# scraed/LanPaint

Measured on AMD Instinct MI355X. Metric: langevin_think_iterations_per_sec, higher is better.
Workload: dtype f32; 1 GPU; c2_sdxl: latent 1x4x128x128 per GPU, 30 sigmas x 5 think iterations, 50% box mask, stub backbone x->(0.9x,0.8x), VE/Karras schedule; rng=torch, graph=auto, mask_format=f32, mask_seen_by_kernels=bits, captured_calls=1, backbone_io=f32, replicas=1, rows_per_gpu=1, global_rows=1, latent_elements_per_gpu=65536

## Files before the change

include/lanpaint_hip.h:

```cpp
#ifndef LANPAINT_HIP_H
#define LANPAINT_HIP_H

#include <stdint.h>

#ifdef __cplusplus
extern "C" {
#endif

#define LP_ABI_VERSION 25

#define LP_API __attribute__((visibility("default")))

#define LP_OK             0
#define LP_E_INVALID     -1
#define LP_E_UNSUPPORTED -2
#define LP_E_LAUNCH      -3
#define LP_E_ALIGN       -4

#define LP_COEF_STRIDE   36
#define LP_C_SCALE        0
#define LP_C_SQRT_ABT     1
#define LP_C_OMA          2
#define LP_C_ABT          3
#define LP_C_RSIGMA       4
#define LP_C_DTX          5
#define LP_C_DTY          6
#define LP_C_AX           7
#define LP_C_AY           8
#define LP_C_DX           9
#define LP_C_DY          10
#define LP_C_VALID       11
#define LP_C_REGION0     12
#define LP_C_REGION1     22
#define LP_R_E_FULL       0
#define LP_R_K_FULL       1
#define LP_R_STD_FULL     2
#define LP_R_E_HALF       3
#define LP_R_K_HALF       4
#define LP_R_STD_HALF     5
#define LP_R_DT           6
#define LP_R_A            7
#define LP_R_CX0          8
#define LP_R_CXT          9
#define LP_C_TMODEL      32
#define LP_C_RSCALE      33

typedef struct lp_hyper {
    float    lambda;
    float    beta;
    float    step_size;
    float    min_step_frac;
    int32_t  is_flow;
    float    one_plus_lambda;
} lp_hyper;

#define LP_PH_REPLACE      (1u << 0)
#define LP_PH_POST_FIRST   (1u << 1)
#define LP_PH_POST_STEADY  (1u << 2)
#define LP_PH_PRE_HALF     (1u << 3)
#define LP_PH_EMIT         (1u << 4)
#define LP_PH_COEFFS       (1u << 5)
#define LP_PH_SIGMA        (1u << 6)

#define LP_FL_FLOW          (1u << 0)
#define LP_FL_MASK_DENOISE  (1u << 1)
#define LP_FL_MASK_U8       (1u << 2)
#define LP_FL_WRITE_X0S     (1u << 3)
#define LP_FL_X0_BF16       (1u << 4)
#define LP_FL_X0_F16        (1u << 5)
#define LP_FL_XIN_BF16      (1u << 6)
#define LP_FL_XIN_F16       (1u << 7)
#define LP_FL_PER_ELEMENT   (1u << 8)
#define LP_FL_CFG_FUSED     (1u << 10)
#define LP_FL_MASK_BITS     (1u << 11)
#define LP_FL_NO_REGION_SKIP (1u << 12)
#define LP_FL_ES            (1u << 13)
#define LP_FL_ES_GATED      (1u << 14)
#define LP_FL_ES_CLOSE      (1u << 15)
#define LP_FL_ES_RING_BITS  (1u << 16)
#define LP_FL_AV            (1u << 17)
#define LP_FL_X0S_GIVEN     (1u << 9)

typedef struct lp_es_state {
    int32_t  stopped;
    int32_t  counter;
    int32_t  n_ran;
    int32_t  cur_slot;
    int32_t  anchor_slot;
    int32_t  write_slot;
    uint32_t reserved0;
    int32_t  enabled;
    int64_t  seq_base;
    int64_t  total_ran;
    double   threshold_eff;
    double   abt_val;
    float*   x0s_buf[3];
} lp_es_state;

#define LP_ES_ACC_SLOTS  64
#define LP_ES_ACC_SETS   3
#define LP_ES_ACC_DOUBLES (LP_ES_ACC_SETS * LP_ES_ACC_SLOTS * 8)
#define LP_ES_SEQ_DONE   0x10000
#define LP_ES_TRACE0     8
#define LP_ES_MAILBOX_DOUBLES(n_steps) (LP_ES_TRACE0 + 8 * (n_steps))

#define LP_RNG_PHILOX 0
#define LP_RNG_TORCH  1

#define LP_REPLACE_KNOWN    0
#define LP_REPLACE_VE       1
#define LP_REPLACE_FLOW     2

typedef struct lp_step_desc {
    int64_t   n_el;
    int64_t   el_per_row;
    int32_t   rows;
    uint32_t  phases;
    uint32_t  flags;
    int32_t   replace_kind;
    float     lambda;
    float     one_plus_lambda;
    float     beta;
    float     step_size;
    float     min_step_frac;
    float     noise_scale;
    float     cfg_scale;
    float     cfg_scale_big;
    const float* coef;
    const float* x;
    const float* known;
    const float* noise;
    const float* y;
    const void*  mask;
    float*       x_t;
    float*       C;
    float*       x0s;
    const void*  x0;
    const void*  x0_big;
    void*        x_in;
    const float* xi_post;
    const float* xi_pre;
    uint64_t     rng_seed;
    uint64_t     rng_offset;
    const uint64_t* rng_offset_ptr;
    const float* abt_el;
    const float* ve_el;
    const float* rsig_el;
    const float* corr_el;
    const float* t_ve;
    const float* t_abt;
    const float* t_rsig;
    const float* t_model;
    float*       coef_out;
    int32_t      t_ve_stride, t_abt_stride, t_rsig_stride, t_model_stride;
    int32_t      rng_kind;
    uint32_t     rng_bg;
    uint32_t     rng_inc;
    uint64_t*    rng_state_out;
    uint64_t     rng_state_val[2];
    uint64_t*    io_table_out;
    uint64_t     io_table_val[2];
    lp_es_state* es;
    float*       es_x0s[3];
    const float* es_ring;
    double*      es_partials;
    double*      es_host;
    double       es_threshold;
    int64_t      es_seq_base;
    int32_t      es_patience_eff;
    int32_t      es_index;
    int32_t      es_n_steps;
    int32_t      es_reset;
    const float* sg_sigma;
    const float* sg_schedule;
    float*       sg_times_out;
    float*       sg_scalars_out;
    int32_t*     sg_seq_out;
    uint64_t*    sg_valid_out;
    double       sg_min_step_frac;
    int32_t      sg_schedule_len, sg_seq, sg_n_steps, sg_early_stop, sg_total_steps, sg_guess;
    double*      clk_out;
    const void*  av_bits;
    float        av_frac;
    uint32_t     reserved2;
    float*       es_xte;
    uint32_t     tune;
    uint32_t     io_valid;
} lp_step_desc;
#define LP_TUNE_VEC1          (1u << 0)
#define LP_TUNE_VEC4          (1u << 1)
#define LP_TUNE_ES_NO_DECIDE  (1u << 2)
#define LP_TUNE_ES_NO_FOLD    (1u << 3)
#define LP_TUNE_ES_NO_ATOMICS (1u << 4)
#define LP_CLK_STAMPS 8

typedef struct lp_final_desc {
    int64_t   n_el;
    uint32_t  flags;
    float     cfg_scale;
    const void*  model_out;
    const void*  uncond;
    const float* y;
    const void*  mask;
    const float* x_src;
    float*       x_dst;
    float*       out;
    uint64_t*    rng_bump_ptr;
    uint64_t     rng_bump;
    const uint64_t* io_table;
} lp_final_desc;

LP_API int lp_abi_version(void);
LP_API const char* lp_strerror(int code);

LP_API int lp_coeffs(const lp_hyper* hyper, const float* ve_sigma, int ve_stride, const float* abt, int abt_stride,
              const float* replace_sigma, int rs_stride, const float* step_override, int step_stride,
              const float* t_model, int t_stride, int rows, float* coef_table, void* stream);

typedef struct lp_call_desc {
    const lp_hyper*      hyper;
    const float*         ve_sigma;      int32_t ve_stride;
    const float*         abt;           int32_t abt_stride;
    const float*         replace_sigma; int32_t rs_stride;
    const float*         t_model;       int32_t t_stride;
    int32_t              rows;
    float*               coef_table;
    const lp_step_desc*  replace;
    void*                graph_exec;
    const lp_final_desc* final;
    const struct lp_graph_binding* replace_binding;
} lp_call_desc;
LP_API int lp_replay_call(const lp_call_desc* call, void* stream);

typedef struct lp_graph_binding {
    void*    node;
    void*    func;
    uint32_t grid[3], block[3];
    uint32_t shared_bytes;
    uint32_t reserved0;
} lp_graph_binding;
LP_API int lp_graph_bind_replace(void* graph, const lp_step_desc* captured_replace, lp_graph_binding* out);
LP_API int lp_graph_clone_tail(void* graph, void** tail_graph_out, void** tail_exec_out);
LP_API int lp_graph_release(void* tail_graph, void* tail_exec);
LP_API int lp_graph_clone_sigma_root(void* graph, const lp_step_desc* with_sigma, void** graph_out, void** exec_out,
                                     lp_graph_binding* binding_out);

LP_API int lp_sigma_times(const float* sigma, int32_t rows, const float* schedule, int32_t schedule_len, int32_t is_flow,
                   float* times_out, float* scalars_out, void* stream);
LP_API int lp_sigma_times_mailbox(const float* sigma, int32_t rows, const float* schedule, int32_t schedule_len, int32_t is_flow,
                           float* times_out, float* scalars_out, int32_t* seq_out, int32_t seq, void* stream);

typedef struct lp_node_call_desc {
    const float*        sigma;
    int32_t             rows;
    int32_t             schedule_len;
    const float*        schedule;
    int32_t             is_flow;
    int32_t             seq;
    float*              times_out;
    float*              scalars_out;
    int32_t*            seq_out;
    const lp_step_desc* replace;
    int32_t             n_steps;
    int32_t             early_stop;
    int32_t             total_steps;
    int32_t             n_counts;
    double              min_step_frac;
    void* const*        exec_by_count;
    int32_t             spin_limit;
    int32_t             guess;
    uint64_t*           valid_word;
    int32_t             fold_sigma;
    int32_t             n_eff;
    int32_t             launched;
    int32_t             speculated;
    int32_t             hit;
    float               step_f, frac;
    void* const*        full_exec_by_count;
    const struct lp_graph_binding* const* full_binding_by_count;
    int32_t             one_launch;
    int32_t             reserved0;
} lp_node_call_desc;
LP_API int lp_node_call(lp_node_call_desc* call, void* stream);
LP_API int32_t lp_effective_inner_steps(int32_t n_steps, double step_f, double frac, int32_t total_steps, int32_t early_stop,
                                 double min_step_frac);

LP_API int lp_step(const lp_step_desc* desc, void* stream);

LP_API int lp_timer_create(void** timer);
LP_API int lp_timer_destroy(void* timer);
LP_API int lp_step_timed(const lp_step_desc* desc, void* stream, void* timer);
LP_API int lp_step_timed_burst(const lp_step_desc* desc, void* stream, void* const* timers, int32_t n);
LP_API int lp_timer_elapsed_ns(void* timer, double* ns);

LP_API int lp_replay_burst(void* const* graph_execs, int32_t n, const lp_step_desc* before, const lp_step_desc* after,
                           int32_t repeats, void* stream);

LP_API int lp_finalize(const lp_final_desc* desc, void* stream);

LP_API int lp_philox_normal(float* out, int64_t n_el, uint64_t seed, uint64_t offset, uint32_t slot, void* stream);
LP_API int lp_torch_normal(float* out, int64_t n_el, uint64_t seed, uint64_t offset, uint32_t bg, void* stream);

LP_API int lp_boundary_ring(const float* mask, float* ring, int64_t planes, int32_t height, int32_t width, void* stream);
LP_API int lp_wmse_pair(const float* a, const float* b, const float* mask, const float* ring, int64_t n_el,
                 double* acc, double* block_scratch, int32_t scratch_blocks, void* stream);

#define LP_MASK_BITS_BYTES(n_el) ((((n_el) + 63) / 64) * 8)

LP_API int lp_pack_mask(const float* mask, int64_t n_el, uint32_t flags, void* bits, int32_t* nonbinary, void* stream);
LP_API int lp_pack_mask_latent(const float* mask, int64_t n_el, uint32_t flags, void* bits, float* latent_out, void* stream);

#define LP_NN_ATEN_SCALAR          0
#define LP_NN_ATEN_CPU_GENERIC_FMA 1
#define LP_NN_ATEN_CPU_GENERIC     2
#define LP_RESHAPE_BINARIZE        1
#define LP_RESHAPE_RULE_SHIFT      8

LP_API int lp_reshape_mask(const float* src, int32_t src_b, int32_t src_c, int32_t src_f, int32_t src_h, int32_t src_w,
                    float* dst, int32_t batch, int32_t channels, int32_t dst_f, int32_t dst_h, int32_t dst_w,
                    int32_t temporal_taps, int32_t flags, void* stream);

typedef struct lp_blend_desc {
    int32_t batch, height, width, channels;
    int32_t k;
    int32_t mask_batch;
    int32_t mask_h, mask_w;
    const float* mask;
    const float* image1;
    const float* image2;
    float*       out;
    float*       smooth_out;
    int32_t nn_rule;
    int32_t reserved0;
} lp_blend_desc;
LP_API int lp_mask_blend(const lp_blend_desc* desc, void* stream);

#define LP_VMASK_MAX_SIDE 16384
#define LP_VMASK_D2_NONE  (-1)
#define LP_VMASK_ZERO     0
#define LP_VMASK_KEY      1
#define LP_VMASK_INNER    2
#define LP_VMASK_OUT_U8   1

typedef struct lp_vmask_edt_desc {
    int32_t n_keys, height, width, reserved0;
    const float* keys;
    int32_t*     d2;
    double*      sdf;
    uint64_t*    csum;
} lp_vmask_edt_desc;
LP_API int lp_vmask_edt(const lp_vmask_edt_desc* desc, void* stream);

typedef struct lp_vmask_frame {
    int32_t kind, key_lo, key_hi, sx1, sy1, sx2, sy2, reserved0;
    double  wf, omw;
} lp_vmask_frame;

typedef struct lp_vmask_morph_desc {
    int32_t n_frames, n_keys, height, width;
    uint32_t flags;
    int32_t  reserved0;
    const lp_vmask_frame* frames;
    const float*  keys;
    const double* sdf;
    void*         out;
} lp_vmask_morph_desc;
LP_API int lp_vmask_morph(const lp_vmask_morph_desc* desc, void* stream);

typedef struct lp_vmask_resize_desc {
    int32_t n_frames, in_h, in_w, out_h, out_w, ksize_x, ksize_y, reserved0;
    const uint8_t* src;
    const int32_t* bounds_x;
    const int32_t* weights_x;
    const int32_t* bounds_y;
    const int32_t* weights_y;
    float*         dst;
} lp_vmask_resize_desc;
LP_API int lp_vmask_resize(const lp_vmask_resize_desc* desc, void* stream);

#define LP_AUDIO_WS_BYTES(mask_len) (12 * ((int64_t)(mask_len) + 1))
typedef struct lp_audio_desc {
    int32_t n;
    int32_t mask_len;
    int32_t batch, channels;
    int32_t cf;
    int32_t nn_rule;
    int64_t orig_sb, orig_sc;
    int64_t inp_sb, inp_sc;
    const float* mask;
    const float* orig;
    const float* inpainted;
    float*       out;
    void*        workspace;
} lp_audio_desc;
// ... 209 lines not shown
```

lanpaint_amd/_cabi.py:

```python
from __future__ import annotations

import ctypes as C
import os

_HERE = os.path.dirname(os.path.abspath(__file__))
LIB_NAME = "liblanpaint_hip.so"
LIB_PATH = os.path.join(_HERE, LIB_NAME)
ABI_VERSION = 25

LP_OK, LP_E_INVALID, LP_E_UNSUPPORTED, LP_E_LAUNCH, LP_E_ALIGN = 0, -1, -2, -3, -4
LP_COEF_STRIDE = 36
(LP_C_SCALE, LP_C_SQRT_ABT, LP_C_OMA, LP_C_ABT, LP_C_RSIGMA, LP_C_DTX, LP_C_DTY, LP_C_AX, LP_C_AY, LP_C_DX, LP_C_DY,
 LP_C_VALID) = range(12)
LP_C_REGION0, LP_C_REGION1, LP_C_TMODEL, LP_C_RSCALE = 12, 22, 32, 33
(LP_R_E_FULL, LP_R_K_FULL, LP_R_STD_FULL, LP_R_E_HALF, LP_R_K_HALF, LP_R_STD_HALF, LP_R_DT, LP_R_A, LP_R_CX0,
 LP_R_CXT) = range(10)

LP_PH_REPLACE, LP_PH_POST_FIRST, LP_PH_POST_STEADY, LP_PH_PRE_HALF, LP_PH_EMIT, LP_PH_COEFFS, LP_PH_SIGMA = 1, 2, 4, 8, 16, 32, 64
LP_FL_FLOW, LP_FL_MASK_DENOISE, LP_FL_MASK_U8, LP_FL_WRITE_X0S = 1, 2, 4, 8
LP_FL_X0_BF16, LP_FL_X0_F16, LP_FL_XIN_BF16, LP_FL_XIN_F16 = 16, 32, 64, 128
LP_FL_PER_ELEMENT, LP_FL_X0S_GIVEN, LP_FL_CFG_FUSED, LP_FL_MASK_BITS, LP_FL_NO_REGION_SKIP = 256, 512, 1024, 2048, 4096
LP_FL_ES, LP_FL_ES_GATED, LP_FL_ES_CLOSE, LP_FL_ES_RING_BITS, LP_FL_AV = 1 << 13, 1 << 14, 1 << 15, 1 << 16, 1 << 17
LP_TUNE_VEC1, LP_TUNE_VEC4, LP_TUNE_ES_NO_DECIDE, LP_TUNE_ES_NO_FOLD, LP_TUNE_ES_NO_ATOMICS = 1, 2, 4, 8, 16


def mask_bits_bytes(n_el: int) -> int:
    return ((int(n_el) + 63) // 64) * 8
LP_REPLACE_KNOWN, LP_REPLACE_VE, LP_REPLACE_FLOW = 0, 1, 2
LP_RNG_PHILOX, LP_RNG_TORCH = 0, 1
LP_NN_ATEN_SCALAR, LP_NN_ATEN_CPU_GENERIC_FMA, LP_NN_ATEN_CPU_GENERIC = 0, 1, 2
LP_RESHAPE_BINARIZE, LP_RESHAPE_RULE_SHIFT = 1, 8


class LpHyper(C.Structure):
    _fields_ = [("lambda_", C.c_float), ("beta", C.c_float), ("step_size", C.c_float), ("min_step_frac", C.c_float),
                ("is_flow", C.c_int32), ("one_plus_lambda", C.c_float)]


class LpStepDesc(C.Structure):
    _fields_ = [
        ("n_el", C.c_int64), ("el_per_row", C.c_int64), ("rows", C.c_int32), ("phases", C.c_uint32),
        ("flags", C.c_uint32), ("replace_kind", C.c_int32),
        ("lambda_", C.c_float), ("one_plus_lambda", C.c_float), ("beta", C.c_float), ("step_size", C.c_float),
        ("min_step_frac", C.c_float), ("noise_scale", C.c_float), ("cfg_scale", C.c_float), ("cfg_scale_big", C.c_float),
        ("coef", C.c_void_p), ("x", C.c_void_p), ("known", C.c_void_p), ("noise", C.c_void_p), ("y", C.c_void_p),
        ("mask", C.c_void_p), ("x_t", C.c_void_p), ("C", C.c_void_p), ("x0s", C.c_void_p), ("x0", C.c_void_p),
        ("x0_big", C.c_void_p), ("x_in", C.c_void_p), ("xi_post", C.c_void_p), ("xi_pre", C.c_void_p),
        ("rng_seed", C.c_uint64), ("rng_offset", C.c_uint64), ("rng_offset_ptr", C.c_void_p),
        ("abt_el", C.c_void_p), ("ve_el", C.c_void_p), ("rsig_el", C.c_void_p), ("corr_el", C.c_void_p),
        ("t_ve", C.c_void_p), ("t_abt", C.c_void_p), ("t_rsig", C.c_void_p), ("t_model", C.c_void_p),
        ("coef_out", C.c_void_p), ("t_ve_stride", C.c_int32), ("t_abt_stride", C.c_int32),
        ("t_rsig_stride", C.c_int32), ("t_model_stride", C.c_int32),
        ("rng_kind", C.c_int32), ("rng_bg", C.c_uint32), ("rng_inc", C.c_uint32),
        ("rng_state_out", C.c_void_p), ("rng_state_val", C.c_uint64 * 2),
        ("io_table_out", C.c_void_p), ("io_table_val", C.c_uint64 * 2),
        ("es", C.c_void_p), ("es_x0s", C.c_void_p * 3), ("es_ring", C.c_void_p), ("es_partials", C.c_void_p), ("es_host", C.c_void_p),
        ("es_threshold", C.c_double), ("es_seq_base", C.c_int64), ("es_patience_eff", C.c_int32), ("es_index", C.c_int32),
        ("es_n_steps", C.c_int32), ("es_reset", C.c_int32),
        ("sg_sigma", C.c_void_p), ("sg_schedule", C.c_void_p), ("sg_times_out", C.c_void_p), ("sg_scalars_out", C.c_void_p),
        ("sg_seq_out", C.c_void_p), ("sg_valid_out", C.c_void_p), ("sg_min_step_frac", C.c_double),
        ("sg_schedule_len", C.c_int32), ("sg_seq", C.c_int32), ("sg_n_steps", C.c_int32), ("sg_early_stop", C.c_int32),
        ("sg_total_steps", C.c_int32), ("sg_guess", C.c_int32), ("clk_out", C.c_void_p), ("av_bits", C.c_void_p), ("av_frac", C.c_float), ("reserved2", C.c_uint32),
        ("es_xte", C.c_void_p),
        ("tune", C.c_uint32), ("io_valid", C.c_uint32),
    ]


class LpEsState(C.Structure):
    _fields_ = [("stopped", C.c_int32), ("counter", C.c_int32), ("n_ran", C.c_int32), ("cur_slot", C.c_int32),
                ("anchor_slot", C.c_int32), ("write_slot", C.c_int32), ("reserved0", C.c_uint32), ("enabled", C.c_int32),
                ("seq_base", C.c_int64), ("total_ran", C.c_int64), ("threshold_eff", C.c_double), ("abt_val", C.c_double), ("x0s_buf", C.c_void_p * 3)]


LP_ES_SEQ_DONE, LP_ES_TRACE0 = 0x10000, 8
LP_ES_ACC_SLOTS, LP_ES_ACC_SETS = 64, 3
LP_ES_ACC_DOUBLES = LP_ES_ACC_SETS * LP_ES_ACC_SLOTS * 8


class LpFinalDesc(C.Structure):
    _fields_ = [
        ("n_el", C.c_int64), ("flags", C.c_uint32), ("cfg_scale", C.c_float),
        ("model_out", C.c_void_p), ("uncond", C.c_void_p), ("y", C.c_void_p), ("mask", C.c_void_p), ("x_src", C.c_void_p),
        ("x_dst", C.c_void_p), ("out", C.c_void_p), ("rng_bump_ptr", C.c_void_p), ("rng_bump", C.c_uint64),
        ("io_table", C.c_void_p),
    ]


class LpGraphBinding(C.Structure):
    _fields_ = [("node", C.c_void_p), ("func", C.c_void_p), ("grid", C.c_uint32 * 3), ("block", C.c_uint32 * 3),
                ("shared_bytes", C.c_uint32), ("reserved0", C.c_uint32)]


class LpCallDesc(C.Structure):
    _fields_ = [
        ("hyper", C.POINTER(LpHyper)),
        ("ve_sigma", C.c_void_p), ("ve_stride", C.c_int32),
        ("abt", C.c_void_p), ("abt_stride", C.c_int32),
        ("replace_sigma", C.c_void_p), ("rs_stride", C.c_int32),
        ("t_model", C.c_void_p), ("t_stride", C.c_int32),
        ("rows", C.c_int32),
        ("coef_table", C.c_void_p),
        ("replace", C.POINTER(LpStepDesc)),
        ("graph_exec", C.c_void_p),
        ("final", C.POINTER(LpFinalDesc)),
        ("replace_binding", C.POINTER(LpGraphBinding)),
    ]


class LpNodeCallDesc(C.Structure):
    _fields_ = [("sigma", C.c_void_p), ("rows", C.c_int32), ("schedule_len", C.c_int32), ("schedule", C.c_void_p),
                ("is_flow", C.c_int32), ("seq", C.c_int32), ("times_out", C.c_void_p), ("scalars_out", C.c_void_p),
                ("seq_out", C.c_void_p), ("replace", C.POINTER(LpStepDesc)), ("n_steps", C.c_int32),
                ("early_stop", C.c_int32), ("total_steps", C.c_int32), ("n_counts", C.c_int32),
                ("min_step_frac", C.c_double), ("exec_by_count", C.POINTER(C.c_void_p)), ("spin_limit", C.c_int32),
                ("guess", C.c_int32), ("valid_word", C.c_void_p), ("fold_sigma", C.c_int32), ("n_eff", C.c_int32), ("launched", C.c_int32),
                ("speculated", C.c_int32), ("hit", C.c_int32), ("step_f", C.c_float), ("frac", C.c_float),
                ("full_exec_by_count", C.POINTER(C.c_void_p)), ("full_binding_by_count", C.POINTER(C.POINTER(LpGraphBinding))),
                ("one_launch", C.c_int32), ("reserved0", C.c_int32)]


class LpBlendDesc(C.Structure):
    _fields_ = [("batch", C.c_int32), ("height", C.c_int32), ("width", C.c_int32), ("channels", C.c_int32),
                ("k", C.c_int32), ("mask_batch", C.c_int32), ("mask_h", C.c_int32), ("mask_w", C.c_int32),
                ("mask", C.c_void_p), ("image1", C.c_void_p), ("image2", C.c_void_p), ("out", C.c_void_p),
                ("smooth_out", C.c_void_p), ("nn_rule", C.c_int32), ("reserved0", C.c_int32)]


LP_VMASK_MAX_SIDE, LP_VMASK_D2_NONE = 16384, -1
LP_VMASK_ZERO, LP_VMASK_KEY, LP_VMASK_INNER, LP_VMASK_OUT_U8 = 0, 1, 2, 1


class LpVmaskEdtDesc(C.Structure):
    _fields_ = [("n_keys", C.c_int32), ("height", C.c_int32), ("width", C.c_int32), ("reserved0", C.c_int32),
                ("keys", C.c_void_p), ("d2", C.c_void_p), ("sdf", C.c_void_p), ("csum", C.c_void_p)]


class LpVmaskFrame(C.Structure):
    _fields_ = [("kind", C.c_int32), ("key_lo", C.c_int32), ("key_hi", C.c_int32), ("sx1", C.c_int32), ("sy1", C.c_int32),
                ("sx2", C.c_int32), ("sy2", C.c_int32), ("reserved0", C.c_int32), ("wf", C.c_double), ("omw", C.c_double)]


class LpVmaskMorphDesc(C.Structure):
    _fields_ = [("n_frames", C.c_int32), ("n_keys", C.c_int32), ("height", C.c_int32), ("width", C.c_int32),
                ("flags", C.c_uint32), ("reserved0", C.c_int32), ("frames", C.c_void_p), ("keys", C.c_void_p),
                ("sdf", C.c_void_p), ("out", C.c_void_p)]


class LpVmaskResizeDesc(C.Structure):
    _fields_ = [("n_frames", C.c_int32), ("in_h", C.c_int32), ("in_w", C.c_int32), ("out_h", C.c_int32),
                ("out_w", C.c_int32), ("ksize_x", C.c_int32), ("ksize_y", C.c_int32), ("reserved0", C.c_int32),
                ("src", C.c_void_p), ("bounds_x", C.c_void_p), ("weights_x", C.c_void_p), ("bounds_y", C.c_void_p),
                ("weights_y", C.c_void_p), ("dst", C.c_void_p)]


class LpAudioDesc(C.Structure):
    _fields_ = [("n", C.c_int32), ("mask_len", C.c_int32), ("batch", C.c_int32), ("channels", C.c_int32), ("cf", C.c_int32),
                ("nn_rule", C.c_int32), ("orig_sb", C.c_int64), ("orig_sc", C.c_int64), ("inp_sb", C.c_int64),
                ("inp_sc", C.c_int64), ("mask", C.c_void_p), ("orig", C.c_void_p), ("inpainted", C.c_void_p),
                ("out", C.c_void_p), ("workspace", C.c_void_p)]


LP_DETAIL_MAX_SIDE, LP_DETAIL_MAX_CHANNELS = 32768, 64


class LpDetailResampleDesc(C.Structure):
    _fields_ = [("batch", C.c_int32), ("src_h", C.c_int32), ("src_w", C.c_int32), ("channels", C.c_int32),
                ("y0", C.c_int32), ("x0", C.c_int32), ("win_h", C.c_int32), ("win_w", C.c_int32),
                ("out_h", C.c_int32), ("out_w", C.c_int32), ("ksize_x", C.c_int32), ("ksize_y", C.c_int32),
                ("src", C.c_void_p), ("bounds_x", C.c_void_p), ("weights_x", C.c_void_p), ("bounds_y", C.c_void_p),
                ("weights_y", C.c_void_p), ("dst", C.c_void_p)]


class LpDetailStitchDesc(C.Structure):
    _fields_ = [("batch", C.c_int32), ("height", C.c_int32), ("width", C.c_int32), ("channels", C.c_int32),
                ("y0", C.c_int32), ("x0", C.c_int32), ("win_h", C.c_int32), ("win_w", C.c_int32),
                ("k", C.c_int32), ("mask_batch", C.c_int32),
                ("mask", C.c_void_p), ("original", C.c_void_p), ("detail", C.c_void_p), ("out", C.c_void_p)]


LP_DETAIL_MAX_COMPONENTS, LP_DETAIL_MAX_REGIONS = 4096, 64


class LpDetailResampleRegionsDesc(C.Structure):
    _fields_ = [("batch", C.c_int32), ("src_h", C.c_int32), ("src_w", C.c_int32), ("channels", C.c_int32),
                ("regions", C.c_int32), ("win_h", C.c_int32), ("win_w", C.c_int32), ("owner_len", C.c_int32),
                ("out_h", C.c_int32), ("out_w", C.c_int32), ("ksize_x", C.c_int32), ("ksize_y", C.c_int32),
                ("origins", C.c_void_p), ("src", C.c_void_p), ("bounds_x", C.c_void_p), ("weights_x", C.c_void_p),
                ("bounds_y", C.c_void_p), ("weights_y", C.c_void_p), ("dst", C.c_void_p), ("labels", C.c_void_p),
                ("owner", C.c_void_p), ("scratch", C.c_void_p)]


class LpDetailStitchRegionsDesc(C.Structure):
    _fields_ = [("batch", C.c_int32), ("height", C.c_int32), ("width", C.c_int32), ("channels", C.c_int32),
                ("regions", C.c_int32), ("win_h", C.c_int32), ("win_w", C.c_int32), ("k", C.c_int32),
                ("mask_batch", C.c_int32), ("owner_len", C.c_int32),
                ("origins", C.c_void_p), ("mask", C.c_void_p), ("original", C.c_void_p), ("detail", C.c_void_p),
                ("out", C.c_void_p), ("labels", C.c_void_p), ("owner", C.c_void_p)]


class LpDetailResampleTrackDesc(C.Structure):
    _fields_ = [("batch", C.c_int32), ("src_h", C.c_int32), ("src_w", C.c_int32), ("channels", C.c_int32),
                ("win_h", C.c_int32), ("win_w", C.c_int32), ("out_h", C.c_int32), ("out_w", C.c_int32),
                ("ksize_x", C.c_int32), ("ksize_y", C.c_int32),
                ("origins", C.c_void_p), ("src", C.c_void_p), ("bounds_x", C.c_void_p), ("weights_x", C.c_void_p),
                ("bounds_y", C.c_void_p), ("weights_y", C.c_void_p), ("dst", C.c_void_p)]


class LpDetailStitchTrackDesc(C.Structure):
    _fields_ = [("batch", C.c_int32), ("height", C.c_int32), ("width", C.c_int32), ("channels", C.c_int32),
                ("win_h", C.c_int32), ("win_w", C.c_int32), ("k", C.c_int32), ("mask_batch", C.c_int32),
                ("origins", C.c_void_p), ("mask", C.c_void_p), ("original", C.c_void_p), ("detail", C.c_void_p),
                ("out", C.c_void_p)]


class LpDetailResampleSubjectsDesc(C.Structure):
    _fields_ = [("batch", C.c_int32), ("src_h", C.c_int32), ("src_w", C.c_int32), ("channels", C.c_int32),
                ("subjects", C.c_int32), ("win_h", C.c_int32), ("win_w", C.c_int32), ("owner_len", C.c_int32),
                ("out_h", C.c_int32), ("out_w", C.c_int32), ("ksize_x", C.c_int32), ("ksize_y", C.c_int32),
                ("origins", C.c_void_p), ("src", C.c_void_p), ("bounds_x", C.c_void_p), ("weights_x", C.c_void_p),
                ("bounds_y", C.c_void_p), ("weights_y", C.c_void_p), ("dst", C.c_void_p), ("labels", C.c_void_p),
                ("owner", C.c_void_p), ("scratch", C.c_void_p)]


class LpDetailStitchSubjectsDesc(C.Structure):
    _fields_ = [("batch", C.c_int32), ("height", C.c_int32), ("width", C.c_int32), ("channels", C.c_int32),
                ("subjects", C.c_int32), ("win_h", C.c_int32), ("win_w", C.c_int32), ("k", C.c_int32),
                ("owner_len", C.c_int32), ("reserved0", C.c_int32),
                ("origins", C.c_void_p), ("mask", C.c_void_p), ("original", C.c_void_p), ("detail", C.c_void_p),
                ("out", C.c_void_p), ("labels", C.c_void_p), ("owner", C.c_void_p)]


LP_COLOR_MIN_COUNT, LP_COLOR_MAX_MARGIN, LP_COLOR_TILE_H, LP_COLOR_TILE_W = 64, 25, 32, 128
LP_COLOR_METHOD_MEAN, LP_COLOR_METHOD_MEAN_STD = 0, 1


class LpColorStatsDesc(C.Structure):
    _fields_ = [("batch", C.c_int32), ("height", C.c_int32), ("width", C.c_int32), ("channels", C.c_int32),
                ("mask_batch", C.c_int32), ("margin", C.c_int32),
                ("detail", C.c_void_p), ("reference", C.c_void_p), ("mask", C.c_void_p), ("stats", C.c_void_p),
                ("workspace", C.c_void_p), ("workspace_bytes", C.c_int64)]


class LpColorFitDesc(C.Structure):
    _fields_ = [("batch", C.c_int32), ("channels", C.c_int32), ("clip_frames", C.c_int32), ("smooth", C.c_int32),
                ("method", C.c_int32), ("reserved0", C.c_int32), ("strength", C.c_double),
                ("stats", C.c_void_p), ("coef", C.c_void_p)]


class LpColorApplyDesc(C.Structure):
    _fields_ = [("batch", C.c_int32), ("height", C.c_int32), ("width", C.c_int32), ("channels", C.c_int32),
                ("detail", C.c_void_p), ("coef", C.c_void_p), ("out", C.c_void_p)]


def lp_color_ws_bytes(batch, height, width, channels):
    tiles = ((int(height) + LP_COLOR_TILE_H - 1) // LP_COLOR_TILE_H) * ((int(width) + LP_COLOR_TILE_W - 1) // LP_COLOR_TILE_W)
    return int(batch) * tiles * (1 + 4 * int(channels)) * 8


LP_FILL_TILE, LP_FILL_SPAN = 32, 5


class LpFillDesc(C.Structure):
    _fields_ = [("batch", C.c_int32), ("height", C.c_int32), ("width", C.c_int32), ("channels", C.c_int32),
                ("mask_batch", C.c_int32), ("reserved0", C.c_int32),
                ("image", C.c_void_p), ("mask", C.c_void_p), ("out", C.c_void_p), ("ws", C.c_void_p), ("ws_bytes", C.c_int64)]


class LpOutpaintDesc(C.Structure):
    _fields_ = [("batch", C.c_int32), ("height", C.c_int32), ("width", C.c_int32), ("channels", C.c_int32),
                ("mask_batch", C.c_int32), ("left", C.c_int32), ("top", C.c_int32), ("right", C.c_int32),
                ("bottom", C.c_int32), ("overlap", C.c_int32), ("reserved0", C.c_int32),
                ("image", C.c_void_p), ("mask", C.c_void_p), ("image_out", C.c_void_p), ("mask_out", C.c_void_p)]


def fill_levels(height, width):
    levels = [(int(height), int(width))]
    while levels[-1] != (1, 1):
        h, w = levels[-1]
        levels.append(((h + 1) // 2, (w + 1) // 2))
    return levels


def fill_ws_bytes(batch, height, width, channels):
    pix = sum(h * w for h, w in fill_levels(height, width)[1:])
    return max(16, (int(batch) * pix * (4 * int(channels) + 1) + 15) // 16 * 16)


def lp_components_ws_bytes(height, width):
    return ((int(height) * int(width) + 1023) // 1024) * 4100


def lp_components_frames_ws_bytes(frames, height, width):
    return ((int(frames) * int(height) * int(width) + 1023) // 1024) * 4100


def lp_audio_ws_bytes(mask_len):
    return 12 * (int(mask_len) + 1)


EXPORTS = {
    "lp_abi_version": (C.c_int, []),
    "lp_strerror": (C.c_char_p, [C.c_int]),
    "lp_coeffs": (C.c_int, [C.POINTER(LpHyper), C.c_void_p, C.c_int, C.c_void_p, C.c_int, C.c_void_p, C.c_int,
                            C.c_void_p, C.c_int, C.c_void_p, C.c_int, C.c_int, C.c_void_p, C.c_void_p]),
    "lp_sigma_times": (C.c_int, [C.c_void_p, C.c_int32, C.c_void_p, C.c_int32, C.c_int32, C.c_void_p, C.c_void_p, C.c_void_p]),
    "lp_sigma_times_mailbox": (C.c_int, [C.c_void_p, C.c_int32, C.c_void_p, C.c_int32, C.c_int32, C.c_void_p, C.c_void_p,
                                         C.c_void_p, C.c_int32, C.c_void_p]),
    "lp_step": (C.c_int, [C.POINTER(LpStepDesc), C.c_void_p]),
    "lp_finalize": (C.c_int, [C.POINTER(LpFinalDesc), C.c_void_p]),
    "lp_mask_blend": (C.c_int, [C.POINTER(LpBlendDesc), C.c_void_p]),
    "lp_timer_create": (C.c_int, [C.POINTER(C.c_void_p)]),
    "lp_timer_destroy": (C.c_int, [C.c_void_p]),
    "lp_step_timed": (C.c_int, [C.POINTER(LpStepDesc), C.c_void_p, C.c_void_p]),
    "lp_step_timed_burst": (C.c_int, [C.POINTER(LpStepDesc), C.c_void_p, C.POINTER(C.c_void_p), C.c_int32]),
    "lp_timer_elapsed_ns": (C.c_int, [C.c_void_p, C.POINTER(C.c_double)]),
    "lp_replay_burst": (C.c_int, [C.POINTER(C.c_void_p), C.c_int32, C.POINTER(LpStepDesc), C.POINTER(LpStepDesc), C.c_int32, C.c_void_p]),
    "lp_torch_normal": (C.c_int, [C.c_void_p, C.c_int64, C.c_uint64, C.c_uint64, C.c_uint32, C.c_void_p]),
    "lp_philox_normal": (C.c_int, [C.c_void_p, C.c_int64, C.c_uint64, C.c_uint64, C.c_uint32, C.c_void_p]),
    "lp_boundary_ring": (C.c_int, [C.c_void_p, C.c_void_p, C.c_int64, C.c_int32, C.c_int32, C.c_void_p]),
    "lp_wmse_pair": (C.c_int, [C.c_void_p, C.c_void_p, C.c_void_p, C.c_void_p, C.c_int64, C.c_void_p, C.c_void_p,
                               C.c_int32, C.c_void_p]),
    "lp_replay_call": (C.c_int, [C.POINTER(LpCallDesc), C.c_void_p]),
    "lp_graph_bind_replace": (C.c_int, [C.c_void_p, C.POINTER(LpStepDesc), C.POINTER(LpGraphBinding)]),
    "lp_graph_clone_tail": (C.c_int, [C.c_void_p, C.POINTER(C.c_void_p), C.POINTER(C.c_void_p)]),
    "lp_graph_release": (C.c_int, [C.c_void_p, C.c_void_p]),
    "lp_graph_clone_sigma_root": (C.c_int, [C.c_void_p, C.POINTER(LpStepDesc), C.POINTER(C.c_void_p), C.POINTER(C.c_void_p),
                                            C.POINTER(LpGraphBinding)]),
    "lp_node_call": (C.c_int, [C.POINTER(LpNodeCallDesc), C.c_void_p]),
    "lp_effective_inner_steps": (C.c_int32, [C.c_int32, C.c_double, C.c_double, C.c_int32, C.c_int32, C.c_double]),
    "lp_pack_mask": (C.c_int, [C.c_void_p, C.c_int64, C.c_uint32, C.c_void_p, C.c_void_p, C.c_void_p]),
    "lp_pack_mask_latent": (C.c_int, [C.c_void_p, C.c_int64, C.c_uint32, C.c_void_p, C.c_void_p, C.c_void_p]),
    "lp_reshape_mask": (C.c_int, [C.c_void_p] + [C.c_int32] * 5 + [C.c_void_p] + [C.c_int32] * 7 + [C.c_void_p]),
    "lp_vmask_edt": (C.c_int, [C.POINTER(LpVmaskEdtDesc), C.c_void_p]),
    "lp_vmask_morph": (C.c_int, [C.POINTER(LpVmaskMorphDesc), C.c_void_p]),
    "lp_vmask_resize": (C.c_int, [C.POINTER(LpVmaskResizeDesc), C.c_void_p]),
    "lp_audio_merge": (C.c_int, [C.POINTER(LpAudioDesc), C.c_void_p]),
    "lp_mask_bbox": (C.c_int, [C.c_void_p, C.c_int32, C.c_int32, C.c_int32, C.c_void_p, C.c_void_p]),
    "lp_detail_resample": (C.c_int, [C.POINTER(LpDetailResampleDesc), C.c_void_p]),
    "lp_detail_stitch": (C.c_int, [C.POINTER(LpDetailStitchDesc), C.c_void_p]),
    "lp_mask_components": (C.c_int, [C.c_void_p, C.c_int32, C.c_int32, C.c_int32, C.c_void_p, C.c_void_p, C.c_void_p, C.c_int64,
                                     C.c_void_p]),
    "lp_detail_resample_regions": (C.c_int, [C.POINTER(LpDetailResampleRegionsDesc), C.c_void_p]),
    "lp_detail_stitch_regions": (C.c_int, [C.POINTER(LpDetailStitchRegionsDesc), C.c_void_p]),
    "lp_mask_bbox_frames": (C.c_int, [C.c_void_p, C.c_int32, C.c_int32, C.c_int32, C.c_void_p, C.c_void_p]),
    "lp_detail_resample_track": (C.c_int, [C.POINTER(LpDetailResampleTrackDesc), C.c_void_p]),
    "lp_detail_stitch_track": (C.c_int, [C.POINTER(LpDetailStitchTrackDesc), C.c_void_p]),
    "lp_mask_components_frames": (C.c_int, [C.c_void_p, C.c_int32, C.c_int32, C.c_int32, C.c_void_p, C.c_void_p, C.c_void_p,
                                            C.c_int64, C.c_void_p]),
    "lp_subject_boxes": (C.c_int, [C.c_void_p, C.c_int32, C.c_int32, C.c_int32, C.c_void_p, C.c_int32, C.c_int32, C.c_void_p,
                                   C.c_void_p]),
    "lp_detail_resample_subjects": (C.c_int, [C.POINTER(LpDetailResampleSubjectsDesc), C.c_void_p]),
    "lp_detail_stitch_subjects": (C.c_int, [C.POINTER(LpDetailStitchSubjectsDesc), C.c_void_p]),
    "lp_color_stats": (C.c_int, [C.POINTER(LpColorStatsDesc), C.c_void_p]),
    "lp_color_fit": (C.c_int, [C.POINTER(LpColorFitDesc), C.c_void_p]),
    "lp_color_apply": (C.c_int, [C.POINTER(LpColorApplyDesc), C.c_void_p]),
    "lp_mask_fill": (C.c_int, [C.POINTER(LpFillDesc), C.c_void_p]),
    "lp_fill_ws_bytes": (C.c_int64, [C.c_int32, C.c_int32, C.c_int32, C.c_int32]),
    "lp_outpaint_pad": (C.c_int, [C.POINTER(LpOutpaintDesc), C.c_void_p]),
}


class LanPaintHipError(RuntimeError):
    """A C-ABI call returned a negative status (the reference raises Python
    exceptions only; C codes are mapped to RuntimeError here)."""


_lib = None


def load(path: str | None = None):
    global _lib
    if _lib is not None and path is None:
        return _lib
    p = path or os.environ.get("LANPAINT_AMD_LIB", LIB_PATH)
    if not os.path.exists(p):
        raise ImportError(
            f"{p} not found: the HIP extension is not built. Run `python -c 'import __graft_entry__ as g; g.build()'` "
            "(or `python -m lanpaint_amd.build`). lanpaint_amd has no CPU / PyTorch fallback for the Langevin path.")
    lib = C.CDLL(p)
    for name, (res, args) in EXPORTS.items():
        fn = getattr(lib, name)
        fn.restype, fn.argtypes = res, args
    v = lib.lp_abi_version()
    if v != ABI_VERSION:
        raise ImportError(f"{p}: ABI version {v}, expected {ABI_VERSION}; rebuild the extension")
    if path is None:
        _lib = lib
    return lib


def check(code: int, what: str = "lanpaint_hip"):
    if code != LP_OK:
        msg = load().lp_strerror(code)
        raise LanPaintHipError(f"{what}: {msg.decode() if msg else code} (code {code})")
```

lanpaint_amd/buffers.py:

```python
from __future__ import annotations

import weakref

import torch

from . import _cabi
from ._util import tensor_version

class _Workspace:

    def __init__(self, like: torch.Tensor, static_io: bool = False, model_dtype=None):
        self.shape, self.device = tuple(like.shape), like.device
        self.x_t = torch.empty_like(like)
        self.C = torch.empty_like(like)
        self.coef = torch.empty((like.shape[0], _cabi.LP_COEF_STRIDE), dtype=torch.float32, device=like.device)
        self.coef_av = None
        self.av_times = None
        self.x0s = []
        self.static_io = static_io
        if static_io:
            self.x_final = torch.empty_like(like)
            self.x_in = self.x_final if model_dtype is None else torch.empty_like(like, dtype=model_dtype)

    def matches(self, like):
        return self.shape == tuple(like.shape) and self.device == like.device


class _DeviceStop:

    def __init__(self, like: torch.Tensor, n_steps: int):
        dev = like.device
        self.shape, self.device, self.n_cap = tuple(like.shape), dev, max(8, int(n_steps))
        self.x0s = [torch.empty_like(like) for _ in range(3)]
        self.x_te = torch.empty_like(like)
        init = _cabi.LpEsState()
        init.cur_slot = init.anchor_slot = -1
        for k in range(3):
            init.x0s_buf[k] = self.x0s[k].data_ptr()
        raw = torch.frombuffer(bytearray(bytes(init) * 2), dtype=torch.uint8)
        self.state = torch.empty(raw.numel(), dtype=torch.uint8, device=dev)
        self.state.copy_(raw)
        self.partials = torch.zeros(_cabi.LP_ES_ACC_DOUBLES, dtype=torch.float64, device=dev)
        self.mailbox = torch.zeros(_cabi.LP_ES_TRACE0 + 8 * self.n_cap, dtype=torch.float64).pin_memory()
        self.f64 = self.mailbox.numpy()
        self.i64 = self.mailbox.view(torch.int64).numpy()
        self.seq_base = 0
        self.seen_total = 0
        self.ring = None

    def matches(self, like, n_steps):
        return self.shape == tuple(like.shape) and self.device == like.device and n_steps <= self.n_cap

    def next_seq(self):
        self.seq_base += 2 * _cabi.LP_ES_SEQ_DONE
        return self.seq_base

    def ring_for(self, key, mask):
        c = self.ring
        ver = (tensor_version(key), key.data_ptr())
        if c is None or c[0]() is not key or c[1] != ver or ver[0] == -1:
            ring = None
            if mask.dim() == 4:
                old = c[2] if c is not None else None
                ring = old if (old is not None and old.shape == mask.shape and old.device == mask.device) else torch.empty_like(mask)
                b, ch, h, w = mask.shape
                with torch.cuda.device(mask.device):
                    _cabi.check(_cabi.load().lp_boundary_ring(mask.data_ptr(), ring.data_ptr(), b * ch, h, w,
                                                              torch.cuda.current_stream(mask.device).cuda_stream),
                                "lp_boundary_ring")
            bits = None
            if ring is not None:
                old_bits = c[3] if c is not None else None
                n_bytes = _cabi.mask_bits_bytes(ring.numel())
                bits = old_bits if (old_bits is not None and old_bits.numel() == n_bytes and old_bits.device == ring.device) \
                    else torch.empty(n_bytes, dtype=torch.uint8, device=ring.device)
                with torch.cuda.device(mask.device):
                    _cabi.check(_cabi.load().lp_pack_mask(ring.data_ptr(), ring.numel(), 0, bits.data_ptr(), None,
                                                          torch.cuda.current_stream(mask.device).cuda_stream), "lp_pack_mask")
            self.ring = c = (weakref.ref(key), ver, ring, bits)
        return c[2]

    def ring_bits(self):
        return self.ring[3] if self.ring is not None else None

    def wait(self, seq, device):
        i64 = self.i64
        for _ in range(20000):
            if i64[0] >= seq:
                return
        torch.cuda.current_stream(device).synchronize()
        if i64[0] < seq:
            raise RuntimeError("early-stop mailbox was not written (expected sequence %d, found %d)" % (seq, int(i64[0])))


class _CallState:
    __slots__ = ("input_x", "xc", "shape", "n_el", "rows", "flow", "ws", "stream", "sigma", "y", "m", "m_c", "m_flag", "abt",
                 "current_times", "base_flags", "keep", "t_model", "sigma_model", "compat", "n_steps", "x_final", "x_in",
                 "xin_flag", "k0_desc", "replace_kind_static", "out", "es")


class _CapturedCall:

    def __init__(self, counter):
        self.graph = torch.cuda.CUDAGraph()
        self.counter = counter
        self.ws = None
        self.final = None
        self.ran = 0
        self.launches = 0
        self.keep = None
        self.fast = False
        self.rows, self.flow, self.hyper, self.k0_desc, self.f_desc = 0, False, None, None, None
        self.call = None
        self.raw_exec = None
        self.ident = None
        self.final_in_graph = False
        self.es = None
        self.n_steps = 0
        self.key = None
        self.tail = None
        self.model_options = None
        self.alive = True
        self.siblings = {}
        self.times_seen = ()
        self.node_table = None
        self.binding = None
        self.tail_handles = None
        self.sigma_root = None

    def __del__(self):
        sr, self.sigma_root = self.sigma_root, None
        if sr:
            try:
                _cabi.load().lp_graph_release(sr[0], sr[1])
            except Exception:
                pass
        h, self.tail_handles = self.tail_handles, None
        if h is not None:
            try:
                _cabi.load().lp_graph_release(h[0], h[1])
            except Exception:
                pass
```

lanpaint_amd/capture.py:

```python
from __future__ import annotations

import ctypes
import os
import weakref

import torch

from . import _cabi
from ._util import _gc_hold, _gc_release
from .buffers import _CapturedCall, _Workspace
from .masks import _compact_mask


class GraphReplay:

    MAX_GRAPHS = 16
    AUTO_MAX_BACKBONE_HOST_US = 100.0

    def begin_call(self, x, latent_image, noise, sigma, latent_mask, current_times, model_options, seed):
        cap = self._last_cap
        if cap is None or cap.tail is None or self.model_dtype is not None or not x.is_cuda:
            return None
        self.img_dim_size = len(x.shape)
        self.latent_image, self.noise = latent_image, noise
# ... 167 lines not shown
                and i[17] == self._hyper_key() and (x.data_ptr() & 15) == 0 and (nz.data_ptr() & 15) == 0
                and not (isinstance(model_options, dict) and "lanpaint_semantic_stop" in model_options))

    @staticmethod
    def _times_ok(cap, current_times):
        i, f32 = cap.ident, torch.float32
        ve, abt, ft = current_times
        for seen in cap.times_seen:
            if seen[0] is ve and seen[1] is abt and seen[2] is ft:
                return True
        ok = (i[13] == ve.numel() and i[14] == abt.numel() and i[15] == ft.numel() and ve.dtype == f32 and abt.dtype == f32
              and ft.dtype == f32 and ve.is_contiguous() and abt.is_contiguous() and ft.is_contiguous())
        if ok:
            cap.times_seen = (cap.times_seen + ((ve, abt, ft),))[-2:]
        return ok

    def _hyper_key(self):
        return (self.chara_lamb, self.chara_beta, self.step_size, self.min_step_frac)

    def _override_state(self):
        d, t, o = self.__dict__, type(self), self._OWN_METHODS
        return ("langevin_dynamics" in d or t.langevin_dynamics is not o[0], "score_model" in d or t.score_model is not o[1],
                "prepare_step_size" in d or t.prepare_step_size is not o[2], self.IS_FLUX, self.IS_FLOW, self.model_dtype)

    def _graph_eligible(self, x, model_options, sigma, current_times):
        if not self.graph or self._graph_blocked or callable(self.rng) or self._noise_regenerated:
            return False
        rows = x.shape[0] if x.ndim else 1
        if any(t.numel() not in (1, rows) for t in (sigma, *current_times)):
            return False
        if self.audio_indicator is not None or self.audio_correction is not None:
            if (self.audio_indicator is None or self.current_times_audio is None
                    or any(t.numel() not in (1, rows) for t in self.current_times_audio)
                    or os.environ.get("LANPAINT_AMD_AV_TABLE", "1") == "0"):
                return False
            packed = self._indicator_pack(self.audio_indicator, x.shape)
            if packed is None or (self._es_opts is not None and not packed[2]):
                return False
        if self._es_opts is not None and (not self._es_opts["device"] or self.rng not in ("torch", "philox")):
            return False
        if self._overridden("langevin_dynamics") or self._overridden("score_model") or \
                self._overridden("prepare_step_size"):
            return False
        return x.dtype == torch.float32 and x.numel() > 0

    def _auto_ready(self, x, latent_mask, model_options):
        a = self._auto
        if a is not None and a[0][0]() is self.latent_image and a[0][1]() is latent_mask and a[0][2] == id(model_options) \
                and a[0][3] == x.shape and a[0][4] == x.device:
            if self._es_opts is not None:
                return False
            return a[1] >= 1 and 1e6 * a[2] < self.AUTO_MAX_BACKBONE_HOST_US
        self._auto = [(weakref.ref(self.latent_image), weakref.ref(latent_mask), id(model_options), x.shape, x.device), 0,
                      float("inf")]
        return False

    def _auto_capture(self, key, x, sigma, latent_mask, current_times, n_steps, model_options, seed, IS_FLUX, IS_FLOW):
        import warnings
        dev = x.device
        saved = (self._iterations_run, torch.cuda.get_rng_state(dev), self._es_opts, self._torch_consumed, self._philox_offset)

        def give_up(why):
            self._capturing = None
            try:
                torch.cuda.synchronize(dev)
            except Exception:
                pass
            self._iterations_run, _, self._es_opts, self._torch_consumed, self._philox_offset = saved
            torch.cuda.set_rng_state(saved[1], dev)
            self._graph_blocked = True
            cap = self._graphs.pop(key, None)
            if cap is not None:
                cap.alive = False
            self._last_cap = None
            warnings.warn("lanpaint_amd: graph='auto' stays with eager launches for this engine: " + why)
            return None

        try:
            cap = self._capture(key, x, sigma, latent_mask, current_times, n_steps, model_options, seed, IS_FLUX, IS_FLOW)
        except Exception as e:
            return give_up("the backbone could not be captured (%s: %s)" % (type(e).__name__, str(e).splitlines()[0] if str(e) else ""))
        if cap is None or self.rng != "torch":
            return cap
        try:
            xa, xb = x.clone(), x.clone()
            out_a = self._run_capture(cap, xa, sigma, latent_mask, current_times, n_steps, model_options, seed, IS_FLUX, IS_FLOW)
            torch.cuda.set_rng_state(saved[1], dev)
            self._last_cap = None
            out_b = self.LanPaint(xb, sigma, latent_mask, current_times, n_steps, model_options, seed, IS_FLUX, IS_FLOW)
            same = bool(torch.equal(out_a, out_b)) and bool(torch.equal(xa, xb))
        except Exception as e:
            return give_up("checking the capture against eager launches failed (%s)" % type(e).__name__)
        if not same:
            return give_up("a replayed sigma call does not reproduce the eager one (the backbone keeps state the graph does not see)")
        self._iterations_run, _, _, self._torch_consumed, self._philox_offset = saved
        torch.cuda.set_rng_state(saved[1], dev)
        return cap

    def _call_graphed(self, x, sigma, latent_mask, current_times, n_steps, model_options, seed, IS_FLUX, IS_FLOW):
        m_c, _ = _compact_mask(latent_mask, x.shape, x.device)
        key = (tuple(x.shape), x.device.index, int(n_steps), bool(IS_FLUX), bool(IS_FLOW), self.latent_image.data_ptr(),
               latent_mask.data_ptr(), m_c.data_ptr() if m_c is not None else 0, int(sigma.numel()),
               tuple(int(t.numel()) for t in current_times), id(model_options), seed, self.rng, self._hyper_key(),
               self.model_dtype, None if self._es_opts is None else (self._es_opts["threshold"], self._es_opts["patience_eff"],
                                                                      self._es_opts["trace"] is not None),
               None if self.audio_indicator is None else (self._indicator_pack(self.audio_indicator, x.shape)[0].data_ptr(),
                                                          self.audio_correction is not None))
        cap = self._graphs.get(key)
        if cap is not None and cap.model_options is not model_options:
            del self._graphs[key]
            cap.alive = False
            cap = None
        if cap is None:
            capture = self._auto_capture if self.graph == "auto" else self._capture
            cap = capture(key, x, sigma, latent_mask, current_times, n_steps, model_options, seed, IS_FLUX, IS_FLOW)
            if cap is None:
                return self.LanPaint(x, sigma, latent_mask, current_times, n_steps, model_options, seed, IS_FLUX, IS_FLOW)
            while len(self._graphs) > self.MAX_GRAPHS:
                self._graphs.popitem(last=False)[1].alive = False
        else:
            self._graphs.move_to_end(key)
        return self._run_capture(cap, x, sigma, latent_mask, current_times, n_steps, model_options, seed, IS_FLUX, IS_FLOW)

    def _run_capture(self, cap, x, sigma, latent_mask, current_times, n_steps, model_options, seed, IS_FLUX, IS_FLOW):
        srcs = (x, sigma, current_times[0], current_times[1], current_times[2], self.noise)
        fast = cap.fast and all(t.dtype == torch.float32 and t.is_contiguous() for t in srcs) and self.noise.shape == x.shape \
            and (x.data_ptr() & 15) == 0 and (self.noise.data_ptr() & 15) == 0
        if not fast and cap.binding is not None:
            self._last_cap = None
            return self.LanPaint(x, sigma, latent_mask, current_times, n_steps, model_options, seed, IS_FLUX, IS_FLOW)
        self._iterations_run += cap.ran
        self.last_inner_steps = cap.ran
        if fast:
            if not isinstance(model_options, dict) or "lanpaint_semantic_stop" not in model_options:
                cap.ident = (self.latent_image, latent_mask, model_options, x.shape, n_steps, seed, self.rng,
                             self.latent_image.data_ptr(), latent_mask.data_ptr(), getattr(latent_mask, "_lp_bits", None),
                             getattr(latent_mask, "_lp_u8", None), x.device, sigma.numel(), current_times[0].numel(),
                             current_times[1].numel(), current_times[2].numel(), self._override_state(), self._hyper_key())
                self._last_cap = cap
            return self._replay_fast(cap, x, sigma, current_times)
        self._last_cap = None
        st = self._prologue(x, sigma, latent_mask, current_times, n_steps, model_options, seed, IS_FLUX, IS_FLOW, ws=cap.ws,
                            ds=cap.es["ds"] if cap.es is not None else None)
        cap.graph.replay()
        if self.rng == "torch":
            gen = self._generator(x.device)
            gen.set_offset(gen.get_offset() + cap.launches)
            self._torch_consumed += cap.launches
        out = self._epilogue(st, cap.final, rng_bump=(cap.counter, cap.launches) if self.rng == "philox" else None,
                             in_graph=cap.final_in_graph)
        if cap.es is not None and st.es is not None:
            self._es_after_replay(cap, st.es["seq"], x.device)
        return out

    def _replay_fast(self, cap, x, sigma, current_times):
        lib, stream = self._lib, self._stream(x.device)
        ve, abt = current_times[0], current_times[1]
        t_src = current_times[2] if cap.flow else ve
        out = torch.empty_like(x)
        k0, f = cap.k0_desc, cap.f_desc
        k0.x, k0.noise = x.data_ptr(), self.noise.data_ptr()
        k0.t_ve, k0.t_abt, k0.t_rsig, k0.t_model = ve.data_ptr(), abt.data_ptr(), sigma.data_ptr(), t_src.data_ptr()
        if cap.final_in_graph:
            k0.io_table_val[0], k0.io_table_val[1] = k0.x, out.data_ptr()
        else:
            f.x_dst, f.out = k0.x, out.data_ptr()
        if self.rng == "torch":
            gen = self._generator(x.device)
            off = gen.get_offset()
            k0.rng_state_val[0], k0.rng_state_val[1] = off, gen.initial_seed()
            gen.set_offset(off + cap.launches)
            self._torch_consumed += cap.launches
        seq = 0
        if cap.es is not None:
            seq = k0.es_seq_base = cap.es["ds"].next_seq()
        if cap.raw_exec is not None:
            _cabi.check(lib.lp_replay_call(ctypes.byref(cap.call), stream), "lp_replay_call")
        else:
            _cabi.check(lib.lp_step(ctypes.byref(k0), stream), "lp_step")
            cap.graph.replay()
            if not cap.final_in_graph:
                _cabi.check(lib.lp_finalize(ctypes.byref(f), stream), "lp_finalize")
        if cap.es is not None:
            self._es_after_replay(cap, seq, x.device)
        return out

    def _es_after_replay(self, cap, seq, dev):
        es = dict(cap.es, trace=self._es_opts["trace"] if self._es_opts is not None else None,
                  tags=self._es_opts["tags"] if self._es_opts is not None else (None, None, None))
        inc = self._randn_policy(dev, cap.ws.x_t.numel())[1] if self.rng == "torch" else 0
        self._es_pending = (cap.es["ds"], seq, cap.n_steps, es, dev, inc)
        if inc or es["trace"] is not None:
            self._es_resolve()

    def _rng_state(self, dev):
        state = self._rng_counters.get(dev)
        if state is None:
            state = self._rng_counters[dev] = torch.zeros(8, dtype=torch.int64, device=dev)
            state[4] = 1
        return state

    _capture_sentinels = {}
    _capture_warned = set()

    @classmethod
    def _warm_capture_state(cls, dev):
        if cls._capture_sentinels.get(dev.index) is not None:
            return
        try:
            with torch.inference_mode(False), torch.no_grad():
                g = torch.cuda.CUDAGraph()
                s = torch.cuda.Stream(device=dev)
                s.wait_stream(torch.cuda.current_stream(dev))
                with torch.cuda.graph(g, stream=s, capture_error_mode="thread_local"):
                    torch.zeros(1, device=dev)
                torch.cuda.current_stream(dev).wait_stream(s)
                cls._capture_sentinels[dev.index] = g
        except Exception as e:
            if dev.index not in cls._capture_warned:
                cls._capture_warned.add(dev.index)
                import warnings
                warnings.warn("lanpaint_amd: the capture warm-up on %s failed (%s: %s); it is retried before the next capture"
                              % (dev, type(e).__name__, str(e).splitlines()[0] if str(e) else ""))

    def _capture(self, key, x, sigma, latent_mask, current_times, n_steps, model_options, seed, IS_FLUX, IS_FLOW,
                 replace_in_graph=None):
        dev = x.device
        self._warm_capture_state(dev)
        if replace_in_graph is None:
            replace_in_graph = os.environ.get("LANPAINT_AMD_REPLACE_IN_GRAPH", "1") != "0"
        raw_ok = self.rng in ("philox", "torch") and os.environ.get("LANPAINT_AMD_RAW_GRAPH", "1") != "0"
        replace_in_graph = bool(replace_in_graph and raw_ok)
        counter = self._rng_state(dev)
        cap = _CapturedCall(counter)
        if replace_in_graph:
            try:
                cap.graph = torch.cuda.CUDAGraph(keep_graph=True)
            except (TypeError, RuntimeError):
                replace_in_graph = False
        ws_key = (tuple(x.shape), dev.index, self.model_dtype)
        cap.ws = self._static_ws.get(ws_key)
        if cap.ws is None:
            if len(self._static_ws) >= self.MAX_GRAPHS:
                self._static_ws.pop(next(iter(self._static_ws)))
            cap.ws = self._static_ws[ws_key] = _Workspace(x.detach().to(torch.float32).contiguous(), static_io=True,
                                                          model_dtype=self.model_dtype)
        side = torch.cuda.Stream(device=dev)
        side.wait_stream(torch.cuda.current_stream(dev))
        it0 = self._iterations_run
        rng_state = torch.cuda.get_rng_state(dev)
        gen = self._generator(dev)
        off0, own0 = gen.get_offset(), self._torch_consumed
        es_user = self._es_opts
        if es_user is not None:
            self._es_opts = dict(es_user, trace=None)
            self._es_close = es_user["trace"] is None
        with torch.cuda.stream(side):
            xw = x.detach().clone()
            st = self._prologue(xw, sigma, latent_mask, current_times, n_steps, model_options, seed, IS_FLUX, IS_FLOW,
                                ws=cap.ws)
            self._epilogue(st, self._think_and_final_model(st, model_options, seed))
            st = self._prologue(xw, sigma, latent_mask, current_times, n_steps, model_options, seed, IS_FLUX, IS_FLOW,
                                ws=cap.ws, defer_launch=replace_in_graph)
            if replace_in_graph and not (st.k0_desc is not None and st.replace_kind_static and st.xc is st.input_x
                                         and (st.xc.data_ptr() & 15) == 0 and (self.noise.data_ptr() & 15) == 0):
                replace_in_graph = False
                self._launch_step_desc(st.k0_desc, st.stream)
        torch.cuda.current_stream(dev).wait_stream(side)
        torch.cuda.synchronize(dev)
        torch_rng_used = (gen.get_offset() - off0) != (self._torch_consumed - own0)
        if torch_rng_used and self.rng == "torch":
            torch.cuda.set_rng_state(rng_state, dev)
            self._iterations_run = it0
            self._graph_blocked = True
            self._es_opts = es_user
            return None
        if torch_rng_used and replace_in_graph:
            torch.cuda.set_rng_state(rng_state, dev)
            self._iterations_run = it0
            self._es_opts = es_user
            return self._capture(key, x, sigma, latent_mask, current_times, n_steps, model_options, seed, IS_FLUX, IS_FLOW,
                                 replace_in_graph=False)
        self._iterations_run = it0
        self._capturing, self._cap_offset = counter, 0
        _gc_hold()
        try:
            f = _cabi.LpFinalDesc()
            with torch.cuda.graph(cap.graph, stream=side, capture_error_mode="thread_local"):
                if replace_in_graph:
                    self._launch_step_desc(st.k0_desc, self._stream(dev))
                cap.final = self._think_and_final_model(st, model_options, seed)
                dense_ok = self._fill_final_desc(f, st, cap.final, st.out)
                if self.rng == "philox":
                    f.rng_bump_ptr, f.rng_bump = counter.data_ptr(), self._cap_offset
                if dense_ok and st.out is not None:
                    f.io_table = counter.data_ptr() + 16
                    _cabi.check(self._lib.lp_finalize(ctypes.byref(f), self._stream(dev)), "lp_finalize")
                    cap.final_in_graph = True
        finally:
            self._capturing = None
            _gc_release()
        cap.launches = self._cap_offset
        self._es_opts = es_user
        torch.cuda.set_rng_state(rng_state, dev)
        cap.ran = self._iterations_run - it0
        self._iterations_run = it0
        cap.keep = st
        cap.rows, cap.flow = st.rows, st.flow
        cap.hyper = _cabi.LpHyper.from_buffer_copy(self._hyper)
        cap.k0_desc = st.k0_desc
        cap.f_desc = f
        cap.model_options = model_options
        cap.es, cap.n_steps = st.es, st.n_steps
        cap.fast = bool(dense_ok and st.k0_desc is not None and st.replace_kind_static and st.xc is st.input_x)
        if replace_in_graph:
            ok = cap.fast and cap.final_in_graph
            if ok:
                try:
                    cap.graph.instantiate()
                    raw_graph = int(cap.graph.raw_cuda_graph())
                    cap.raw_exec = int(cap.graph.raw_cuda_graph_exec()) or None
                    b = _cabi.LpGraphBinding()
                    ok = cap.raw_exec is not None and self._lib.lp_graph_bind_replace(
                        raw_graph, ctypes.byref(cap.k0_desc), ctypes.byref(b)) == _cabi.LP_OK
                    if ok:
                        cap.binding = b
                        tg, te = ctypes.c_void_p(), ctypes.c_void_p()
                        if self._lib.lp_graph_clone_tail(raw_graph, ctypes.byref(tg), ctypes.byref(te)) == _cabi.LP_OK:
                            cap.tail_handles = (tg.value, te.value)
                except Exception:
                    ok = False
            if not ok:
                return self._capture(key, x, sigma, latent_mask, current_times, n_steps, model_options, seed, IS_FLUX,
                                     IS_FLOW, replace_in_graph=False)
        if cap.fast:
            if cap.binding is None and raw_ok and not torch_rng_used:
                try:
                    cap.raw_exec = int(cap.graph.raw_cuda_graph_exec()) or None
                except Exception:
                    cap.raw_exec = None
            c = cap.call = _cabi.LpCallDesc()
            c.replace = ctypes.pointer(cap.k0_desc)
            c.final = None if cap.final_in_graph else ctypes.pointer(f)
            c.rows, c.coef_table, c.graph_exec = st.rows, cap.ws.coef.data_ptr(), cap.raw_exec
            if cap.binding is not None:
                c.replace_binding = ctypes.pointer(cap.binding)
                if cap.tail_handles is not None:
                    t = cap.tail = _cabi.LpCallDesc()
                    t.rows, t.coef_table, t.graph_exec = st.rows, cap.ws.coef.data_ptr(), cap.tail_handles[1]
            elif cap.raw_exec is not None and cap.final_in_graph:
                t = cap.tail = _cabi.LpCallDesc()
                t.rows, t.coef_table, t.graph_exec = st.rows, cap.ws.coef.data_ptr(), cap.raw_exec
        cap.key = key
        self._graphs[key] = cap
        return cap
```

lanpaint_amd/csrc/cabi.hip:

```cpp
#include <cmath>

#include "lp_common.h"

namespace lp {
int step_dispatch(const lp_step_desc* d, hipStream_t stream, void* timer);
int replace_node_update(const lp_step_desc* d, hipGraphExec_t exec, const lp_graph_binding* b);
int timer_create(void** out);
int timer_destroy(void* h);
int timer_elapsed_ns(void* h, double* ns);
int coeffs_dispatch(const lp_hyper* h, const float* ve, int ve_stride, const float* abt, int abt_stride,
                    const float* rs, int rs_stride, const float* step_ov, int step_stride, const float* t_model,
                    int t_stride, int rows, float* table, hipStream_t stream);
int finalize_dispatch(const lp_final_desc* d, hipStream_t stream);
int sigma_times_dispatch(const float* sigma, int rows, const float* schedule, int schedule_len, int is_flow, float* times,
                         float* scalars, int32_t* seq_out, int32_t seq, hipStream_t stream);
int sigma_times_rule_dispatch(const float* sigma, int rows, const float* schedule, int schedule_len, int is_flow,
                              float* times, float* scalars, int32_t* seq_out, int32_t seq, int32_t n_steps, int32_t early_stop,
                              int32_t total_steps, double min_step_frac, int32_t guess, uint64_t* valid_out, hipStream_t stream);
int blend_dispatch(const lp_blend_desc* d, hipStream_t stream);
int philox_dispatch(float* out, int64_t n_el, uint64_t seed, uint64_t offset, uint32_t slot, hipStream_t stream);
int ring_dispatch(const float* mask, float* ring, int64_t planes, int height, int width, hipStream_t stream);
int wmse_dispatch(const float* a, const float* b, const float* mask, const float* ring, int64_t n_el, double* acc,
                  double* scratch, int scratch_blocks, hipStream_t stream);
int torch_normal_dispatch(float* out, int64_t n, uint64_t seed, uint64_t offset, uint32_t bg, hipStream_t stream);
int pack_mask_dispatch(const float* mask, int64_t n_el, uint32_t flags, void* bits, int32_t* nonbinary, float* latent_out,
                       hipStream_t stream);
int vmask_edt_dispatch(const lp_vmask_edt_desc* d, hipStream_t stream);
int vmask_morph_dispatch(const lp_vmask_morph_desc* d, hipStream_t stream);
int vmask_resize_dispatch(const lp_vmask_resize_desc* d, hipStream_t stream);
int audio_merge_dispatch(const lp_audio_desc* d, hipStream_t stream);
int mask_bbox_dispatch(const float* mask, int planes, int H, int W, int32_t* boxes, bool per_plane, hipStream_t stream);
int detail_resample_dispatch(const lp_detail_resample_desc* d, hipStream_t stream);
int detail_stitch_dispatch(const lp_detail_stitch_desc* d, hipStream_t stream);
int mask_components_dispatch(const float* mask, int planes, int H, int W, int32_t* labels, int32_t* table, void* workspace,
                             int64_t workspace_bytes, hipStream_t stream);
int detail_resample_regions_dispatch(const lp_detail_resample_regions_desc* d, hipStream_t stream);
int detail_stitch_regions_dispatch(const lp_detail_stitch_regions_desc* d, hipStream_t stream);
int detail_resample_track_dispatch(const lp_detail_resample_track_desc* d, hipStream_t stream);
int detail_stitch_track_dispatch(const lp_detail_stitch_track_desc* d, hipStream_t stream);
int mask_components_frames_dispatch(const float* mask, int F, int H, int W, int32_t* labels, int32_t* table, void* workspace,
                                    int64_t workspace_bytes, hipStream_t stream);
int subject_boxes_dispatch(const int32_t* labels, int frames, int H, int W, const int32_t* owner, int owner_len, int subjects,
                           int32_t* boxes, hipStream_t stream);
int detail_resample_subjects_dispatch(const lp_detail_resample_subjects_desc* d, hipStream_t stream);
int detail_stitch_subjects_dispatch(const lp_detail_stitch_subjects_desc* d, hipStream_t stream);
int color_stats_dispatch(const lp_color_stats_desc* d, hipStream_t stream);
int color_fit_dispatch(const lp_color_fit_desc* d, hipStream_t stream);
int color_apply_dispatch(const lp_color_apply_desc* d, hipStream_t stream);
int mask_fill_dispatch(const lp_fill_desc* d, hipStream_t stream);
int64_t fill_ws_bytes(int batch, int height, int width, int channels);
int outpaint_pad_dispatch(const lp_outpaint_desc* d, hipStream_t stream);
int reshape_mask_dispatch(const float* src, int sb, int sc, int sf, int sh, int sw, float* dst, int db, int dc, int df,
                          int dh, int dw, int taps, int flags, hipStream_t stream);
}

static inline hipStream_t as_stream(void* s) { return static_cast<hipStream_t>(s); }

extern "C" {

int lp_abi_version(void) { return LP_ABI_VERSION; }

const char* lp_strerror(int code) {
    switch (code) {
        case LP_OK: return "ok";
        case LP_E_INVALID: return "invalid argument (null pointer or inconsistent sizes/phases)";
        case LP_E_UNSUPPORTED: return "unsupported layout or flag combination";
        case LP_E_LAUNCH: return "HIP kernel launch failed";
        case LP_E_ALIGN: return "pointer not aligned for the requested layout";
        default: return "unknown lanpaint_hip error code";
    }
}

int lp_coeffs(const lp_hyper* hyper, const float* ve_sigma, int ve_stride, const float* abt, int abt_stride,
              const float* replace_sigma, int rs_stride, const float* step_override, int step_stride,
              const float* t_model, int t_stride, int rows, float* coef_table, void* stream) {
    return lp::coeffs_dispatch(hyper, ve_sigma, ve_stride, abt, abt_stride, replace_sigma, rs_stride, step_override,
                               step_stride, t_model, t_stride, rows, coef_table, as_stream(stream));
}

int lp_sigma_times(const float* sigma, int32_t rows, const float* schedule, int32_t schedule_len, int32_t is_flow,
                   float* times_out, float* scalars_out, void* stream) {
    return lp::sigma_times_dispatch(sigma, rows, schedule, schedule_len, is_flow, times_out, scalars_out, nullptr, 0,
                                    as_stream(stream));
}

int lp_sigma_times_mailbox(const float* sigma, int32_t rows, const float* schedule, int32_t schedule_len, int32_t is_flow,
                           float* times_out, float* scalars_out, int32_t* seq_out, int32_t seq, void* stream) {
    if (!seq_out) return LP_E_INVALID;
    return lp::sigma_times_dispatch(sigma, rows, schedule, schedule_len, is_flow, times_out, scalars_out, seq_out, seq,
                                    as_stream(stream));
}

int lp_step(const lp_step_desc* desc, void* stream) { return lp::step_dispatch(desc, as_stream(stream), nullptr); }

int lp_timer_create(void** timer) { return lp::timer_create(timer); }
int lp_timer_destroy(void* timer) { return lp::timer_destroy(timer); }
int lp_step_timed(const lp_step_desc* desc, void* stream, void* timer) {
    if (!timer) return LP_E_INVALID;
    return lp::step_dispatch(desc, as_stream(stream), timer);
}
int lp_timer_elapsed_ns(void* timer, double* ns) { return lp::timer_elapsed_ns(timer, ns); }

int lp_mask_blend(const lp_blend_desc* desc, void* stream) { return lp::blend_dispatch(desc, as_stream(stream)); }

int lp_vmask_edt(const lp_vmask_edt_desc* desc, void* stream) { return lp::vmask_edt_dispatch(desc, as_stream(stream)); }

int lp_vmask_morph(const lp_vmask_morph_desc* desc, void* stream) { return lp::vmask_morph_dispatch(desc, as_stream(stream)); }

int lp_vmask_resize(const lp_vmask_resize_desc* desc, void* stream) { return lp::vmask_resize_dispatch(desc, as_stream(stream)); }

int lp_audio_merge(const lp_audio_desc* desc, void* stream) { return lp::audio_merge_dispatch(desc, as_stream(stream)); }

int lp_mask_bbox(const float* mask, int32_t planes, int32_t height, int32_t width, int32_t* bbox, void* stream) {
    return lp::mask_bbox_dispatch(mask, planes, height, width, bbox, false, as_stream(stream));
}

int lp_detail_resample(const lp_detail_resample_desc* desc, void* stream) { return lp::detail_resample_dispatch(desc, as_stream(stream)); }

int lp_detail_stitch(const lp_detail_stitch_desc* desc, void* stream) { return lp::detail_stitch_dispatch(desc, as_stream(stream)); }

int lp_mask_components(const float* mask, int32_t planes, int32_t height, int32_t width, int32_t* labels, int32_t* table,
                       void* workspace, int64_t workspace_bytes, void* stream) {
    return lp::mask_components_dispatch(mask, planes, height, width, labels, table, workspace, workspace_bytes, as_stream(stream));
}

int lp_detail_resample_regions(const lp_detail_resample_regions_desc* desc, void* stream) {
    return lp::detail_resample_regions_dispatch(desc, as_stream(stream));
}

int lp_detail_stitch_regions(const lp_detail_stitch_regions_desc* desc, void* stream) {
    return lp::detail_stitch_regions_dispatch(desc, as_stream(stream));
}

int lp_mask_bbox_frames(const float* mask, int32_t planes, int32_t height, int32_t width, int32_t* boxes, void* stream) {
    return lp::mask_bbox_dispatch(mask, planes, height, width, boxes, true, as_stream(stream));
}

int lp_detail_resample_track(const lp_detail_resample_track_desc* desc, void* stream) {
    return lp::detail_resample_track_dispatch(desc, as_stream(stream));
}

int lp_detail_stitch_track(const lp_detail_stitch_track_desc* desc, void* stream) {
    return lp::detail_stitch_track_dispatch(desc, as_stream(stream));
}

int lp_mask_components_frames(const float* mask, int32_t frames, int32_t height, int32_t width, int32_t* labels, int32_t* table,
                              void* workspace, int64_t workspace_bytes, void* stream) {
    return lp::mask_components_frames_dispatch(mask, frames, height, width, labels, table, workspace, workspace_bytes,
                                               as_stream(stream));
}

int lp_subject_boxes(const int32_t* labels, int32_t frames, int32_t height, int32_t width, const int32_t* owner, int32_t owner_len,
                     int32_t subjects, int32_t* boxes, void* stream) {
    return lp::subject_boxes_dispatch(labels, frames, height, width, owner, owner_len, subjects, boxes, as_stream(stream));
}

int lp_detail_resample_subjects(const lp_detail_resample_subjects_desc* desc, void* stream) {
    return lp::detail_resample_subjects_dispatch(desc, as_stream(stream));
}

int lp_detail_stitch_subjects(const lp_detail_stitch_subjects_desc* desc, void* stream) {
    return lp::detail_stitch_subjects_dispatch(desc, as_stream(stream));
}

int lp_color_stats(const lp_color_stats_desc* desc, void* stream) { return lp::color_stats_dispatch(desc, as_stream(stream)); }

int lp_color_fit(const lp_color_fit_desc* desc, void* stream) { return lp::color_fit_dispatch(desc, as_stream(stream)); }

int lp_color_apply(const lp_color_apply_desc* desc, void* stream) { return lp::color_apply_dispatch(desc, as_stream(stream)); }

int lp_mask_fill(const lp_fill_desc* desc, void* stream) { return lp::mask_fill_dispatch(desc, as_stream(stream)); }

int64_t lp_fill_ws_bytes(int32_t batch, int32_t height, int32_t width, int32_t channels) {
    return lp::fill_ws_bytes(batch, height, width, channels);
}

int lp_outpaint_pad(const lp_outpaint_desc* desc, void* stream) { return lp::outpaint_pad_dispatch(desc, as_stream(stream)); }

int lp_finalize(const lp_final_desc* desc, void* stream) { return lp::finalize_dispatch(desc, as_stream(stream)); }

int lp_philox_normal(float* out, int64_t n_el, uint64_t seed, uint64_t offset, uint32_t slot, void* stream) {
    return lp::philox_dispatch(out, n_el, seed, offset, slot, as_stream(stream));
}

int lp_boundary_ring(const float* mask, float* ring, int64_t planes, int32_t height, int32_t width, void* stream) {
    return lp::ring_dispatch(mask, ring, planes, height, width, as_stream(stream));
}

int lp_wmse_pair(const float* a, const float* b, const float* mask, const float* ring, int64_t n_el, double* acc,
                 double* block_scratch, int32_t scratch_blocks, void* stream) {
    return lp::wmse_dispatch(a, b, mask, ring, n_el, acc, block_scratch, scratch_blocks, as_stream(stream));
}

int lp_replay_call(const lp_call_desc* c, void* stream) {
    if (!c || (!c->replace && !c->graph_exec && !c->final)) return LP_E_INVALID;
    hipStream_t s = as_stream(stream);
    int rc = LP_OK;
    if (c->hyper)
        rc = lp::coeffs_dispatch(c->hyper, c->ve_sigma, c->ve_stride, c->abt, c->abt_stride, c->replace_sigma,
                                 c->rs_stride, nullptr, 0, c->t_model, c->t_stride, c->rows, c->coef_table, s);
    if (rc != LP_OK) return rc;
    if (c->replace && c->replace_binding) {
        if (!c->graph_exec) return LP_E_INVALID;
        rc = lp::replace_node_update(c->replace, static_cast<hipGraphExec_t>(c->graph_exec), c->replace_binding);
    } else if (c->replace) {
        rc = lp::step_dispatch(c->replace, s, nullptr);
    }
    if (rc != LP_OK) return rc;
    if (c->graph_exec && hipGraphLaunch(static_cast<hipGraphExec_t>(c->graph_exec), s) != hipSuccess) return LP_E_LAUNCH;
    return c->final ? lp::finalize_dispatch(c->final, s) : LP_OK;
}

int lp_graph_bind_replace(void* graph, const lp_step_desc* captured, lp_graph_binding* out) {
    if (!graph || !captured || !out) return LP_E_INVALID;
    hipGraph_t g = static_cast<hipGraph_t>(graph);
    size_t n_root = 0;
    if (hipGraphGetRootNodes(g, nullptr, &n_root) != hipSuccess || n_root != 1) return LP_E_UNSUPPORTED;
    hipGraphNode_t root = nullptr;
    if (hipGraphGetRootNodes(g, &root, &n_root) != hipSuccess || !root) return LP_E_UNSUPPORTED;
    hipGraphNodeType ty;
    if (hipGraphNodeGetType(root, &ty) != hipSuccess || ty != hipGraphNodeTypeKernel) return LP_E_UNSUPPORTED;
    hipKernelNodeParams p{};
    if (hipGraphKernelNodeGetParams(root, &p) != hipSuccess || !p.func || !p.kernelParams) return LP_E_UNSUPPORTED;
    void* const* kp = p.kernelParams;
    const lp_step_desc* dn = static_cast<const lp_step_desc*>(kp[8]);
    if (*static_cast<void* const*>(kp[0]) != captured->x_t || *static_cast<const void* const*>(kp[2]) != captured->x ||
        !dn || dn->phases != captured->phases || !(dn->phases & LP_PH_REPLACE) || dn->n_el != captured->n_el)
        return LP_E_UNSUPPORTED;
    lp::StepPlan plan;
    const int rc = lp::plan_step(*captured, &plan);
    if (rc != LP_OK) return rc;
    if (!lp::plan_is_node(plan, p.func, p.gridDim, p.blockDim)) return LP_E_UNSUPPORTED;
    out->node = root; out->func = p.func;
    out->grid[0] = p.gridDim.x; out->grid[1] = p.gridDim.y; out->grid[2] = p.gridDim.z;
    out->block[0] = p.blockDim.x; out->block[1] = p.blockDim.y; out->block[2] = p.blockDim.z;
    out->shared_bytes = p.sharedMemBytes; out->reserved0 = 0;
    return LP_OK;
}

int lp_graph_clone_tail(void* graph, void** tail_graph_out, void** tail_exec_out) {
    if (!graph || !tail_graph_out || !tail_exec_out) return LP_E_INVALID;
    hipGraph_t clone = nullptr;
    if (hipGraphClone(&clone, static_cast<hipGraph_t>(graph)) != hipSuccess) return LP_E_LAUNCH;
    size_t n_root = 0;
    hipGraphNode_t root = nullptr;
    hipGraphExec_t exec = nullptr;
    if (hipGraphGetRootNodes(clone, nullptr, &n_root) == hipSuccess && n_root == 1 &&
        hipGraphGetRootNodes(clone, &root, &n_root) == hipSuccess && root && hipGraphDestroyNode(root) == hipSuccess &&
        hipGraphInstantiate(&exec, clone, nullptr, nullptr, 0) == hipSuccess) {
        *tail_graph_out = clone; *tail_exec_out = exec;
        return LP_OK;
    }
    (void)hipGraphDestroy(clone);
    return LP_E_UNSUPPORTED;
}

int lp_graph_clone_sigma_root(void* graph, const lp_step_desc* with_sigma, void** graph_out, void** exec_out,
                              lp_graph_binding* binding_out) {
    if (!graph || !with_sigma || !graph_out || !exec_out || !binding_out) return LP_E_INVALID;
    if (with_sigma->phases != (LP_PH_REPLACE | LP_PH_EMIT | LP_PH_COEFFS | LP_PH_SIGMA)) return LP_E_INVALID;
    lp::StepPlan sig, plain;
    int rc = lp::plan_step(*with_sigma, &sig);
    if (rc != LP_OK) return rc;
    lp_step_desc without = *with_sigma;
    without.phases &= ~LP_PH_SIGMA;
    rc = lp::plan_step(without, &plain);
    if (rc != LP_OK) return rc;
    rc = LP_E_UNSUPPORTED;
    hipGraph_t clone = nullptr;
    hipGraphExec_t exec = nullptr;
    do {
        if (hipGraphClone(&clone, static_cast<hipGraph_t>(graph)) != hipSuccess) { clone = nullptr; break; }
        hipGraphNode_t root = nullptr;
        size_t n_root = 0;
        if (hipGraphGetRootNodes(clone, nullptr, &n_root) != hipSuccess || n_root != 1 ||
            hipGraphGetRootNodes(clone, &root, &n_root) != hipSuccess || !root) break;
        hipGraphNodeType ty;
        if (hipGraphNodeGetType(root, &ty) != hipSuccess || ty != hipGraphNodeTypeKernel) break;
        hipKernelNodeParams p{};
        if (hipGraphKernelNodeGetParams(root, &p) != hipSuccess || !lp::plan_is_node(plain, p.func, p.gridDim, p.blockDim)) break;
        lp::StepArgs a;
        lp::pack_step_args(sig, *with_sigma, &a);
        p.func = const_cast<void*>(sig.kernel);
        p.gridDim = sig.grid;
        p.kernelParams = a.ptr;
        p.extra = nullptr;
        if (hipGraphKernelNodeSetParams(root, &p) != hipSuccess) break;
        if (hipGraphInstantiate(&exec, clone, nullptr, nullptr, 0) != hipSuccess) { exec = nullptr; break; }
        binding_out->node = root; binding_out->func = p.func;
        binding_out->grid[0] = p.gridDim.x; binding_out->grid[1] = p.gridDim.y; binding_out->grid[2] = p.gridDim.z;
        binding_out->block[0] = p.blockDim.x; binding_out->block[1] = p.blockDim.y; binding_out->block[2] = p.blockDim.z;
        binding_out->shared_bytes = p.sharedMemBytes; binding_out->reserved0 = 0;
        *graph_out = clone; *exec_out = exec;
        rc = LP_OK;
    } while (false);
    if (rc != LP_OK) {
        if (exec) (void)hipGraphExecDestroy(exec);
        if (clone) (void)hipGraphDestroy(clone);
    }
    return rc;
}

int lp_graph_release(void* tail_graph, void* tail_exec) {
    if (tail_exec) (void)hipGraphExecDestroy(static_cast<hipGraphExec_t>(tail_exec));
    if (tail_graph) (void)hipGraphDestroy(static_cast<hipGraph_t>(tail_graph));
    return LP_OK;
}

int32_t lp_effective_inner_steps(int32_t n_steps, double step_f, double frac, int32_t total_steps, int32_t early_stop,
                                 double min_step_frac) {
    return lp::effective_inner_steps(n_steps, step_f, frac, total_steps, early_stop, min_step_frac);
}

static int node_wait(const lp_node_call_desc* c, int32_t want, hipStream_t s) {
    for (int32_t k = 0; k < c->spin_limit; ++k)
        if (__atomic_load_n(c->seq_out, __ATOMIC_ACQUIRE) == want) return LP_OK;
    if (hipStreamSynchronize(s) != hipSuccess) return LP_E_LAUNCH;
    return __atomic_load_n(c->seq_out, __ATOMIC_ACQUIRE) == want ? LP_OK : LP_E_LAUNCH;
}

static int node_call_body(lp_node_call_desc* c, hipStream_t s, bool* queued_spec) {
    const auto exec_for = [&](int32_t n) -> hipGraphExec_t {
        return (c->exec_by_count && n >= 0 && n < c->n_counts) ? static_cast<hipGraphExec_t>(c->exec_by_count[n]) : nullptr;
    };
    const bool speculate = c->guess >= 0 && c->valid_word && exec_for(c->guess) != nullptr && c->replace && !c->replace->es_reset;
    c->speculated = speculate ? 1 : 0;
    c->hit = 0;
    c->launched = 0;
    int rc = LP_OK;
    lp_step_desc rep;
    if (c->replace) {
        rep = *c->replace;
        rep.io_valid = 0;
    }
    lp_step_desc d;
    bool fold_sigma = speculate && c->fold_sigma && c->is_flow == ((c->replace->flags & LP_FL_FLOW) ? 1 : 0) &&
                      c->rows == c->replace->rows;
    if (fold_sigma) {
        d = rep;
        d.phases |= LP_PH_SIGMA;
        d.sg_sigma = c->sigma; d.sg_schedule = c->schedule; d.sg_schedule_len = c->schedule_len; d.sg_times_out = c->times_out;
        d.sg_scalars_out = c->scalars_out; d.sg_seq_out = c->seq_out; d.sg_seq = c->seq; d.sg_valid_out = c->valid_word;
        d.sg_n_steps = c->n_steps; d.sg_early_stop = c->early_stop; d.sg_total_steps = c->total_steps; d.sg_guess = c->guess;
        d.sg_min_step_frac = c->min_step_frac;
        lp::StepPlan plan;
        fold_sigma = lp::plan_step(d, &plan) == LP_OK;
    }
    c->one_launch = 0;
    if (fold_sigma) {
        hipGraphExec_t full = (c->full_exec_by_count && c->full_binding_by_count && c->guess < c->n_counts)
                                  ? static_cast<hipGraphExec_t>(c->full_exec_by_count[c->guess]) : nullptr;
        const lp_graph_binding* fb = full ? c->full_binding_by_count[c->guess] : nullptr;
        if (full && fb) {
            rc = lp::replace_node_update(&d, full, fb);
            if (rc != LP_OK) return rc;
            if (hipGraphLaunch(full, s) != hipSuccess) return LP_E_LAUNCH;
            *queued_spec = true;
            c->one_launch = 1;
        } else {
            rc = lp::step_dispatch(&d, s, nullptr);
            if (rc != LP_OK) return rc;
            *queued_spec = true;
        }
    } else {
        rc = lp::sigma_times_rule_dispatch(c->sigma, c->rows, c->schedule, c->schedule_len, c->is_flow, c->times_out,
                                           c->scalars_out, c->seq_out, c->seq, c->n_steps, c->early_stop, c->total_steps,
                                           c->min_step_frac, speculate ? c->guess : -1, c->valid_word, s);
        if (rc != LP_OK) return rc;
        *queued_spec = speculate;
        if (c->replace) {
            rc = lp::step_dispatch(&rep, s, nullptr);
            if (rc != LP_OK) return rc;
        }
    }
    if (speculate && !c->one_launch && hipGraphLaunch(exec_for(c->guess), s) != hipSuccess) return LP_E_LAUNCH;
    rc = node_wait(c, c->seq, s);
    if (rc != LP_OK) return rc;
    c->step_f = c->scalars_out[0];
    c->frac = c->scalars_out[1];
    c->n_eff = lp::effective_inner_steps(c->n_steps, static_cast<double>(c->step_f), static_cast<double>(c->frac),
                                         c->total_steps, c->early_stop, c->min_step_frac);
    if (c->valid_word && static_cast<int32_t>(c->scalars_out[3]) != c->n_eff) return LP_E_UNSUPPORTED;
    if (speculate) {
        if (c->n_eff == c->guess) {
            c->hit = 1;
            c->launched = 1;
            *queued_spec = false;
            return LP_OK;
        }
        rc = lp::sigma_times_rule_dispatch(c->sigma, c->rows, c->schedule, c->schedule_len, c->is_flow, c->times_out,
                                           c->scalars_out, c->seq_out, c->seq ^ 0x40000000, c->n_steps, c->early_stop,
                                           c->total_steps, c->min_step_frac, -1, c->valid_word, s);
        if (rc != LP_OK) return rc;
        *queued_spec = false;
        rc = lp::step_dispatch(&rep, s, nullptr);
        if (rc != LP_OK) return rc;
    }
    if (hipGraphExec_t e = exec_for(c->n_eff)) {
        if (hipGraphLaunch(e, s) != hipSuccess) return LP_E_LAUNCH;
        c->launched = 1;
    }
    return LP_OK;
}

int lp_node_call(lp_node_call_desc* c, void* stream) {
    if (!c || !c->sigma || !c->schedule || !c->times_out || !c->scalars_out || !c->seq_out || c->rows <= 0) return LP_E_INVALID;
    hipStream_t s = as_stream(stream);
    bool queued_spec = false;
    const int rc = node_call_body(c, s, &queued_spec);
    if (rc != LP_OK && queued_spec && c->valid_word) {
        (void)lp::sigma_times_rule_dispatch(c->sigma, c->rows, c->schedule, c->schedule_len, c->is_flow, c->times_out,
                                            c->scalars_out, c->seq_out, c->seq ^ 0x20000000, c->n_steps, c->early_stop,
                                            c->total_steps, c->min_step_frac, -1, c->valid_word, s);
    }
    return rc;
}

int lp_step_timed_burst(const lp_step_desc* desc, void* stream, void* const* timers, int32_t n) {
    if (!desc || !timers || n <= 0) return LP_E_INVALID;
    lp_step_desc d = *desc;
    for (int32_t i = 0; i < n; ++i) {
        d.rng_offset = desc->rng_offset + static_cast<uint64_t>(i);
        const int rc = lp::step_dispatch(&d, as_stream(stream), timers[i]);
        if (rc != LP_OK) return rc;
    }
    return LP_OK;
}

int lp_replay_burst(void* const* graph_execs, int32_t n, const lp_step_desc* before, const lp_step_desc* after,
                    int32_t repeats, void* stream) {
    if (!graph_execs || n <= 0 || repeats <= 0) return LP_E_INVALID;
    hipStream_t s = as_stream(stream);
    for (int32_t r = 0; r < repeats; ++r) {
        for (int32_t i = 0; i < n; ++i) {
            if (before) {
                const int rc = lp::step_dispatch(before, s, nullptr);
                if (rc != LP_OK) return rc;
            }
            if (graph_execs[i] && hipGraphLaunch(static_cast<hipGraphExec_t>(graph_execs[i]), s) != hipSuccess) return LP_E_LAUNCH;
            if (after) {
                const int rc = lp::step_dispatch(after, s, nullptr);
                if (rc != LP_OK) return rc;
            }
        }
    }
    return LP_OK;
}

int lp_torch_normal(float* out, int64_t n_el, uint64_t seed, uint64_t offset, uint32_t bg, void* stream) {
    return lp::torch_normal_dispatch(out, n_el, seed, offset, bg, as_stream(stream));
}

int lp_pack_mask(const float* mask, int64_t n_el, uint32_t flags, void* bits, int32_t* nonbinary, void* stream) {
    return lp::pack_mask_dispatch(mask, n_el, flags, bits, nonbinary, nullptr, as_stream(stream));
}

int lp_pack_mask_latent(const float* mask, int64_t n_el, uint32_t flags, void* bits, float* latent_out, void* stream) {
    if (!latent_out) return LP_E_INVALID;
    return lp::pack_mask_dispatch(mask, n_el, flags, bits, nullptr, latent_out, as_stream(stream));
}

int lp_reshape_mask(const float* src, int32_t src_b, int32_t src_c, int32_t src_f, int32_t src_h, int32_t src_w,
                    float* dst, int32_t batch, int32_t channels, int32_t dst_f, int32_t dst_h, int32_t dst_w,
                    int32_t temporal_taps, int32_t flags, void* stream) {
    return lp::reshape_mask_dispatch(src, src_b, src_c, src_f, src_h, src_w, dst, batch, channels, dst_f, dst_h, dst_w,
                                     temporal_taps, flags, as_stream(stream));
}

}
```

lanpaint_amd/csrc/step_kernel.hip:

```cpp
#include <cstddef>

#include "lp_common.h"

#pragma clang fp contract(off)

namespace lp {

struct RegionCoef {
    float e_full, k_full, std_full, e_half, k_half, std_half, dt, a, cx0, cxt;
};

struct RowCoef {
    float scale, sqrt_abt, oma, abt, rsigma, dtx, dty, ax, ay, dx, dy, valid;
    RegionCoef reg[2];
    float rscale;
};

__device__ __forceinline__ RowCoef load_row(const float* __restrict__ coef, int row) {
    const float* c = coef + static_cast<int64_t>(row) * LP_COEF_STRIDE;
    RowCoef r;
    r.scale = c[LP_C_SCALE]; r.sqrt_abt = c[LP_C_SQRT_ABT]; r.oma = c[LP_C_OMA]; r.abt = c[LP_C_ABT];
    r.rsigma = c[LP_C_RSIGMA]; r.dtx = c[LP_C_DTX]; r.dty = c[LP_C_DTY]; r.ax = c[LP_C_AX]; r.ay = c[LP_C_AY];
    r.dx = c[LP_C_DX]; r.dy = c[LP_C_DY]; r.valid = c[LP_C_VALID];
    r.rscale = c[LP_C_RSCALE];
// ... 73 lines not shown
__device__ __forceinline__ float ou_general(float x, float tau, float a, float c, float d, float xi) {
    const float adt = a * tau;
    const float e = expf(-adt);
    float k, k2;
    if (fabsf(a) < 1e-8f) {
        k = tau;
        k2 = tau;
    } else {
        k = (-expm1f(-adt)) / a;
        k2 = (-expm1f(-2.0f * adt)) / (2.0f * a);
    }
    const float mean = e * x + k * c;
    const float var = (d * d) * k2;
    return mean + xi * sqrtf(fmaxf(var, 0.0f));
}

constexpr int kEsSums = 6;

constexpr int kEsSlots = LP_ES_ACC_SLOTS, kEsSets = LP_ES_ACC_SETS;
static_assert(kEsSlots == kWave, "one accumulator slot per lane of the reducing wave");

__device__ __forceinline__ double* es_acc_set(const lp_step_desc& d, int iteration) {
    return d.es_partials + static_cast<size_t>(((iteration % kEsSets) + kEsSets) % kEsSets) * kEsSlots * 8;
}

__device__ __forceinline__ void es_slot_total(const double (&v)[kEsSums], float (&tot)[kEsSums]) {
    float f[kEsSums];
#pragma unroll
    for (int k = 0; k < kEsSums; ++k) f[k] = static_cast<float>(v[k]);
    wave_sum_dpp(f);
#pragma unroll
    for (int k = 0; k < kEsSums; ++k)
        tot[k] = __builtin_bit_cast(float, __builtin_amdgcn_readlane(__builtin_bit_cast(int, f[k]), kWave - 1));
}

__device__ __forceinline__ double clamp01(double v) { return v <= 0.0 ? 0.0 : (v >= 1.0 ? 1.0 : v); }

__device__ __forceinline__ void es_reset_state(const lp_step_desc& d, bool fold) {
    lp_es_state* es = d.es;
    const int n = fold ? (d.t_abt_stride ? d.rows : 1) : d.rows;
    const bool av = (d.flags & LP_FL_AV) != 0;
    float sum = 0.0f;
    for (int r = 0; r < n; ++r) {
        if (av) {
            const float v = d.coef[static_cast<int64_t>(2 * r) * LP_COEF_STRIDE + LP_C_ABT];
            const float a = d.coef[static_cast<int64_t>(2 * r + 1) * LP_COEF_STRIDE + LP_C_ABT];
            sum = sum + (v * (1.0f - d.av_frac) + a * d.av_frac);
        } else {
            sum = sum + (fold ? d.t_abt[static_cast<int64_t>(r) * d.t_abt_stride]
                              : d.coef[static_cast<int64_t>(r) * LP_COEF_STRIDE + LP_C_ABT]);
        }
    }
    const double abt_val = static_cast<double>(sum / static_cast<float>(n));
    const double a = clamp01(abt_val);
    const double thr_eff = d.es_threshold * clamp01(4.0 * a * (1.0 - a));
    const int64_t total = es[0].total_ran > es[1].total_ran ? es[0].total_ran : es[1].total_ran;
    es->total_ran = total;
    es->stopped = 0; es->counter = 0; es->n_ran = 0;
    es->cur_slot = -1; es->anchor_slot = -1; es->write_slot = 0;
    es->enabled = thr_eff > 0.0 ? 1 : 0;
    es->seq_base = d.es_seq_base;
    es->threshold_eff = thr_eff;
    es->abt_val = abt_val;
    es[1] = es[0];
}

__device__ __forceinline__ void es_post_seq(double* host, int64_t seq) {
    __threadfence_system();
    __hip_atomic_store(reinterpret_cast<int64_t*>(host), seq, __ATOMIC_RELEASE, __HIP_MEMORY_SCOPE_SYSTEM);
}

__device__ __forceinline__ void es_decide(const lp_step_desc& d, lp_es_state& st, const float (&sf)[kEsSums], bool have_prev,
                                          bool have_anchor, int i, bool post) {
    double* host = post ? d.es_host : nullptr;
    const bool has_ring = d.es_ring != nullptr;
    const float* s = sf;
    const double nan = __builtin_nan("");
    double dist_in = static_cast<double>(s[0] / (s[1] + 1e-12f)), dist_ring = nan, dist_drift = nan;
    double dist = dist_in;
    if (have_prev && has_ring) {
        dist_ring = static_cast<double>(s[2] / (s[3] + 1e-12f));
        dist = dist_in > dist_ring ? dist_in : dist_ring;
    }
    const bool enabled = st.enabled != 0 && s[1] >= 1e-6f;
    int counter = st.counter, anchor = st.anchor_slot, stopped = 0;
    const int cur = st.write_slot;
    if (enabled) {
        const double thr = st.threshold_eff;
        if (dist <= thr) {
            if (anchor < 0) {
                anchor = cur;
            } else if (have_anchor) {
                const double di = static_cast<double>(s[4] / (s[1] + 1e-12f));
                const double dr = has_ring ? static_cast<double>(s[5] / (s[3] + 1e-12f)) : nan;
                dist_drift = has_ring ? (di > dr ? di : dr) : di;
                dist = dist > dist_drift ? dist : dist_drift;
            }
        } else {
            anchor = -1;
        }
        if (dist <= thr) {
            counter += 1;
        } else {
            counter = 0;
            anchor = -1;
        }
        stopped = counter >= d.es_patience_eff ? 1 : 0;
    }
    st.counter = counter;
    st.anchor_slot = anchor;
    st.cur_slot = cur;
    int w = 0;
    while (w == cur || w == anchor) ++w;
    st.write_slot = w;
    st.n_ran = i + 1;
    st.total_ran += 1;
    st.stopped = stopped;
    if (host) {
        double* rec = host + LP_ES_TRACE0 + 8 * i;
        rec[0] = dist; rec[1] = dist_in; rec[2] = dist_ring; rec[3] = dist_drift;
        rec[4] = static_cast<double>(counter); rec[5] = static_cast<double>(stopped); rec[6] = 0.0; rec[7] = 0.0;
        host[1] = static_cast<double>(i + 1); host[2] = static_cast<double>(stopped);
        host[3] = enabled ? 1.0 : 0.0; host[4] = st.threshold_eff; host[5] = st.abt_val;
        host[6] = static_cast<double>(st.total_ran);
        const bool gated = (d.flags & LP_FL_ES_GATED) != 0;
        if (!gated) es_post_seq(host, st.seq_base + i + 1);
        else if (i + 1 == d.es_n_steps) es_post_seq(host, st.seq_base + LP_ES_SEQ_DONE);
    }
}

__device__ __forceinline__ void es_store_dynamic(lp_es_state* dst, const lp_es_state& st) {
    dst->stopped = st.stopped; dst->counter = st.counter; dst->n_ran = st.n_ran; dst->cur_slot = st.cur_slot;
    dst->anchor_slot = st.anchor_slot; dst->write_slot = st.write_slot; dst->total_ran = st.total_ran;
}

#ifdef LP_SHADER_CLOCK
__device__ __forceinline__ uint64_t clk_now() {
    uint64_t t;
    asm volatile("s_memtime %0\n s_waitcnt lgkmcnt(0)" : "=s"(t)::"memory");
    return t;
}
__device__ __forceinline__ uint64_t clk_after_loads() {
    uint64_t t;
    asm volatile("s_waitcnt vmcnt(0)\n s_memtime %0\n s_waitcnt lgkmcnt(0)" : "=s"(t)::"memory");
    return t;
}
__device__ __forceinline__ uint64_t clk_real() {
    uint64_t t;
    asm volatile("s_memrealtime %0\n s_waitcnt lgkmcnt(0)" : "=s"(t)::"memory");
    return t;
}
#define LP_CLK_DECL                                                                                                  \
    uint64_t clk_t[LP_CLK_STAMPS] = {}, clk_r0 = 0;                                                                  \
    const bool clk_on = d_arg.clk_out && threadIdx.x == 0 && blockIdx.y == 0 && (blockIdx.x == 0 || blockIdx.x == gridDim.x - 1); \
    if (clk_on) { clk_t[0] = clk_now(); clk_r0 = clk_real(); }
#define LP_CLK(k) if (clk_on) clk_t[k] = clk_now();
#define LP_CLK_LOADS(k) if (clk_on) clk_t[k] = clk_after_loads();
#define LP_CLK_FLUSH                                                                                                 \
    if (clk_on) {                                                                                                    \
        double* clk_o = d_arg.clk_out + (blockIdx.x == 0 ? 0 : 16);                                                  \
        for (int k = 0; k < LP_CLK_STAMPS; ++k) clk_o[k] = clk_t[k] ? static_cast<double>(clk_t[k] - clk_t[0]) : 0.0; \
        clk_o[15] = static_cast<double>(clk_real() - clk_r0);                                                        \
        clk_o[14] = static_cast<double>(clk_r0 & 0xffffffffffffull);       \
    }
#else
#define LP_CLK_DECL
#define LP_CLK(k)
#define LP_CLK_LOADS(k)
#define LP_CLK_FLUSH
#endif

constexpr int kBlock = 256;

constexpr uint32_t kPost = LP_PH_POST_FIRST | LP_PH_POST_STEADY;
constexpr uint32_t kTouchXt = LP_PH_REPLACE | kPost | LP_PH_PRE_HALF;

enum : int { MODE_ROW = 0, MODE_PER_EL = 1, MODE_HARD = 2 };

template <int VEC, int MODE, uint32_t PH, int X0W, int RNG, bool ST = false, int ES = 0>
__global__ __launch_bounds__(256) __attribute__((amdgpu_waves_per_eu((ES == 2 && VEC == 4 && PH != 0) ? 8 : 1))) void lp_step_kernel(void* a0, void* a1, const void* a2, const void* a3, const void* a4,
                                                       const void* a5, int32_t a_el_per_row, uint32_t a_flags,
                                                       const lp_step_desc d_arg) {
    constexpr bool PER_EL = MODE == MODE_PER_EL;
    constexpr bool HARD = MODE == MODE_HARD;
    constexpr bool SMALL = VEC == 1;
    constexpr bool PAIR = X0W == 2 && VEC == 4 && !ST;
    static_assert(!PAIR || ES == 0, "pair accesses: every lane that has not left the kernel is active");
    constexpr bool TBL = (PH & LP_PH_COEFFS) != 0 && VEC == 1;
    const unsigned el_bx = blockIdx.x - (TBL ? 1u : 0u);
    static_assert(!TBL || (!ST && !ES && (PH & LP_PH_REPLACE) != 0), "table block: the fused replace launches only");
    LP_CLK_DECL
    lp_step_desc d = d_arg;
    d.x_t = static_cast<float*>(a0); d.C = static_cast<float*>(a1);
    if constexpr ((PH & LP_PH_REPLACE) != 0) {
        d.x = static_cast<const float*>(a2);
        d.known = d.noise = static_cast<const float*>(a3);
        d.y = static_cast<const float*>(a4); d.mask = a5;
    } else {
        d.x0 = a2; d.x0_big = a3;
        if constexpr (SMALL) {
            d.coef = static_cast<const float*>(a4); d.rng_offset_ptr = static_cast<const uint64_t*>(a5);
        } else {
            d.y = static_cast<const float*>(a4); d.mask = a5;
        }
    }
    d.el_per_row = a_el_per_row; d.flags = a_flags;
    static_assert(!ES || (!ST && !PER_EL && (PH & LP_PH_REPLACE) == 0), "early stop: think-step launches of the row-table modes");
    constexpr bool es_fold = ES == 2;
    int row = blockIdx.y;
    int64_t st_base = 0, st_lo = 0, st_hi = 0;
    uint32_t st_round = 0;
    if constexpr (ST) {
        const int64_t span = 4 * static_cast<int64_t>(d.rng_bg), epr = d.el_per_row;
        const uint32_t rounds = d.rng_inc >> 2, per_round = gridDim.y / rounds;
        st_round = blockIdx.y / per_round;
        st_base = static_cast<int64_t>(st_round) * span;
        row = static_cast<int>(st_base / epr) + static_cast<int>(blockIdx.y - st_round * per_round);
        const int64_t row_lo = static_cast<int64_t>(row) * epr, row_hi = row_lo + epr;
        st_lo = row_lo > st_base ? row_lo : st_base;
        st_hi = row_hi < st_base + span ? row_hi : st_base + span;
        if (row >= d.rows || st_lo >= st_hi) return;
        const int64_t i0 = st_base + static_cast<int64_t>(blockIdx.x) * kBlock, i1 = i0 + kBlock;
        bool any = false;
#pragma unroll
        for (int k = 0; k < 4; ++k) {
            const int64_t s0 = i0 + k * static_cast<int64_t>(d.rng_bg), s1 = i1 + k * static_cast<int64_t>(d.rng_bg);
            any = any || (s0 < st_hi && s1 > st_lo);
        }
        if (!any) return;
    }
    const uint32_t fl = d.flags;
    bool es_gated = false, es_idle = false;
    int es_prev = -1, es_anchor = -1, es_write = 0;
    bool es_keeper = false;
    lp_es_state es_lite;
    uint2 es_words[8];
    double es_fv[kEsSums];
    if constexpr (ES) {
        es_gated = (fl & LP_FL_ES_GATED) != 0;
        if constexpr (es_fold) {
            const int rd = (d.es_index + 1) & 1;
            const lp_es_state* sp = d.es + rd;
            if constexpr (VEC == 4) {
                const uint2* sv = reinterpret_cast<const uint2*>(sp);
#pragma unroll
                for (int k = 0; k < 8; ++k) es_words[k] = sv[k];
            } else {
                uint32_t lane_zero;
                asm volatile("v_mov_b32 %0, 0" : "=v"(lane_zero));
                const uint2* sv = reinterpret_cast<const uint2*>(sp) + lane_zero;
#pragma unroll
                for (int k = 0; k < 8; ++k) es_words[k] = sv[k];
            }
            es_keeper = blockIdx.x == 0 && blockIdx.y == 0 && threadIdx.x == 0;
            if constexpr (VEC != 4) {
                if (threadIdx.x < kWave) {
                    const double* src = es_acc_set(d, d.es_index - 1) + static_cast<size_t>(threadIdx.x) * 8;
#pragma unroll
                    for (int k = 0; k < kEsSums; ++k) es_fv[k] = src[k];
                }
            }
        } else {
            es_prev = d.es->cur_slot; es_anchor = d.es->anchor_slot; es_write = d.es->write_slot;
            if (es_gated && d.es->stopped != 0) {
                const int64_t g = static_cast<int64_t>(blockIdx.x) * kBlock + threadIdx.x;
                if (g >= d.el_per_row / VEC) return;
                const int64_t i = static_cast<int64_t>(row) * d.el_per_row + g * VEC;
                float xt[VEC], xo[VEC];
                load_f32<VEC>(d.x_t, i, xt);
                if constexpr (PH == 0 && MODE == MODE_ROW && !ST) {
                    if (fl & LP_FL_AV) {
                        const uint32_t word = static_cast<const uint32_t*>(d.av_bits)[i >> 5];
                        const uint32_t nib = word >> (static_cast<uint32_t>(i) & 31u);
#pragma unroll
                        for (int k = 0; k < VEC; ++k) {
                            const float sc = d.coef[static_cast<int64_t>(2 * row + static_cast<int>((nib >> k) & 1u)) * LP_COEF_STRIDE + LP_C_SCALE];
                            xo[k] = (fl & LP_FL_FLOW) ? xt[k] / sc : xt[k] * sc;
                        }
                        store_any<VEC>(d.x_in, xin_dtype(fl), i, xo);
                        return;
                    }
                }
                const float sc = load_row(d.coef, row).scale;
#pragma unroll
                for (int k = 0; k < VEC; ++k) xo[k] = (fl & LP_FL_FLOW) ? xt[k] / sc : xt[k] * sc;
                store_any<VEC>(d.x_in, xin_dtype(fl), i, xo);
                return;
            }
        }
    }
    const uint32_t ph = PH ? PH : d.phases;
    const bool flow = fl & LP_FL_FLOW;
    const bool post = ph & kPost;
    constexpr bool HOT = PH != 0 && ES == 0 && RNG == 0;
    const bool given = HOT ? false : (fl & LP_FL_X0S_GIVEN) != 0;
    const int x0dt = X0W == 4 ? static_cast<int>(DT_F32) : x0_dtype(fl), xindt = xin_dtype(fl);
    const int64_t groups = ST ? static_cast<int64_t>(d.rng_bg) : d.el_per_row / VEC;
    const int64_t row_base = static_cast<int64_t>(row) * d.el_per_row;
    const float lam = d.lambda, opl = d.one_plus_lambda;

    RowCoef rc;
    bool av_mixed = false;
    uint32_t av_nib = 0u;
    const bool fold_coeffs = (ph & LP_PH_COEFFS) != 0;
    constexpr bool fold_sigma = (PH & LP_PH_SIGMA) != 0;
    static_assert(!fold_sigma || PH != 0, "LP_PH_SIGMA: the phase-specialised kernels only");
    auto row_times = [&](float& abt_f, float& ve_f, float& rs_f, float& tm_f) __attribute__((always_inline)) {
        if constexpr (fold_sigma) {
            float ft;
            rs_f = d.sg_sigma[row];
            sigma_to_times(rs_f, flow, ve_f, abt_f, ft);
            tm_f = flow ? ft : ve_f;
        } else {
            abt_f = d.t_abt[static_cast<int64_t>(row) * d.t_abt_stride];
            ve_f = d.t_ve ? d.t_ve[static_cast<int64_t>(row) * d.t_ve_stride] : 0.0f;
            rs_f = d.t_rsig ? d.t_rsig[static_cast<int64_t>(row) * d.t_rsig_stride] : 0.0f;
            tm_f = 0.0f;
        }
    };
    if (fold_coeffs) {
        auto build_table = [&](float abt_f, float ve_f, float rs_f, float tm_sig) __attribute__((always_inline)) {
            if (threadIdx.x < 4) {
                lp_hyper h;
                h.lambda = d.lambda; h.beta = d.beta; h.step_size = d.step_size; h.min_step_frac = d.min_step_frac;
                h.is_flow = flow ? 1 : 0; h.one_plus_lambda = d.one_plus_lambda;
                const float tm_f = fold_sigma ? tm_sig : (d.t_model ? d.t_model[static_cast<int64_t>(row) * d.t_model_stride] : 0.0f);
                const float step = d.step_size * fmaxf(1.0f - abt_f, d.min_step_frac);
                coeffs_lane(h, abt_f, ve_f, rs_f, tm_f, step, (threadIdx.x >> 1) & 1, threadIdx.x & 1,
                            d.coef_out + static_cast<int64_t>(row) * LP_COEF_STRIDE);
                if (row == 0 && threadIdx.x == 0 && d.rng_state_out) {
                    d.rng_state_out[0] = d.rng_state_val[0];
                    d.rng_state_out[1] = d.rng_state_val[1];
                }
            }
        };
        auto sigma_rule = [&]() __attribute__((always_inline)) {
            const SigmaRule rule{d.sg_n_steps, d.sg_early_stop, d.sg_total_steps, d.sg_guess, d.sg_min_step_frac, d.sg_valid_out};
            sigma_rows_and_rule(d.sg_sigma, d.rows, d.sg_schedule, d.sg_schedule_len, flow, d.sg_times_out,
                                d.sg_scalars_out, d.sg_seq_out, d.sg_seq, rule);
        };
        if constexpr (TBL) {
            if (blockIdx.x == 0) {
                if (threadIdx.x < kWave) {
                    float abt_f, ve_f, rs_f, tm_f;
                    row_times(abt_f, ve_f, rs_f, tm_f);
                    build_table(abt_f, ve_f, rs_f, tm_f);
                    LP_CLK(5)
                } else if (fold_sigma && blockIdx.y == 0 && threadIdx.x < 2 * kWave) {
                    sigma_rule();
                }
                LP_CLK(6)
                LP_CLK_FLUSH
                return;
            }
        } else {
            float abt_f, ve_f, rs_f, tm_f;
            row_times(abt_f, ve_f, rs_f, tm_f);
            if constexpr (fold_sigma) {
                if (blockIdx.x == 0 && blockIdx.y == 0 && threadIdx.x < kWave) sigma_rule();
            }
            if (blockIdx.x == 0) build_table(abt_f, ve_f, rs_f, tm_f);
            rc.scale = row_scale(flow, abt_f, ve_f);
            rc.rscale = 1.0f / rc.scale;
            rc.rsigma = rs_f;
        }
    } else {
        if constexpr (PH == 0) {
            if ((ph & LP_PH_REPLACE) && d.rng_state_out && blockIdx.x == 0 && blockIdx.y == 0 && threadIdx.x == 0) {
                d.rng_state_out[0] = d.rng_state_val[0];
                d.rng_state_out[1] = d.rng_state_val[1];
            }
        }
        if constexpr (!PER_EL) {
            if constexpr (SMALL && PH != 0) {
                static_assert(VEC == 1, "load_row_early leaves rc.rscale poisoned: the div_shared paths (VEC == 4) must use load_row");
                rc = load_row_early(d.coef, row);
            } else {
                int crow = row;
                if constexpr (PH == 0 && MODE == MODE_ROW && !ST) {
                    if (fl & LP_FL_AV) {
                        const int64_t g0 = static_cast<int64_t>(blockIdx.x) * kBlock + threadIdx.x;
                        const bool in_row = g0 < groups;
                        const int64_t i0 = row_base + (in_row ? g0 : groups - 1) * VEC;
                        const uint32_t word = static_cast<const uint32_t*>(d.av_bits)[i0 >> 5];
                        av_nib = (word >> (static_cast<uint32_t>(i0) & 31u)) & ((1u << VEC) - 1u);
                        const bool any_audio = __ballot(in_row && av_nib != 0u) != 0ull;
                        const bool any_video = __ballot(in_row && av_nib != ((1u << VEC) - 1u)) != 0ull;
                        av_mixed = any_audio && any_video;
                        crow = 2 * row + ((any_audio && !any_video) ? 1 : 0);
                    }
                }
                rc = load_row(d.coef, crow);
            }
        }
    }

    uint64_t rng_w0 = 0, rng_w1 = 0;
    bool rng_have = false;
    if constexpr (SMALL) {
        if (d.rng_offset_ptr) {
            rng_w0 = d.rng_offset_ptr[0];
            rng_w1 = d.rng_offset_ptr[1];
            rng_have = true;
        }
    }

    const int64_t g_raw = static_cast<int64_t>(el_bx) * kBlock + threadIdx.x;
    int64_t st_i = 0;
    if constexpr (ST) st_i = st_base + static_cast<int64_t>(threadIdx.x >> 6) * static_cast<int64_t>(d.rng_bg) +
                             static_cast<int64_t>(blockIdx.x) * kBlock + static_cast<int64_t>(threadIdx.x & 63) * VEC;
    const bool active = ST ? (st_i >= st_lo && st_i < st_hi) : (g_raw < groups);
    if constexpr (!ES && !ST) {
        if (!active) return;
    }
    const int64_t g = active ? g_raw : groups - 1;
    float es_p[kEsSums] = {0.f, 0.f, 0.f, 0.f, 0.f, 0.f};
    bool es_zero_wave = false;
    {
        const int64_t i = ST ? (active ? st_i : st_lo) : row_base + g * VEC;

        constexpr bool AVK = PH == 0 && MODE == MODE_ROW && !ST;
        auto av_row = [&](int k) __attribute__((always_inline)) -> const float* {
            return d.coef + static_cast<int64_t>(2 * row + static_cast<int>((av_nib >> k) & 1u)) * LP_COEF_STRIDE;
        };
        auto av_ld = [&](const float* c, int f) __attribute__((always_inline)) -> float {
            return __hip_atomic_load(c + f, __ATOMIC_RELAXED, __HIP_MEMORY_SCOPE_WAVEFRONT);
        };
        auto row_scale_of = [&](int k) __attribute__((always_inline)) -> float {
            if constexpr (AVK) {
                if (av_mixed) return av_ld(av_row(k), LP_C_SCALE);
            }
            return rc.scale;
        };
        auto row_rsigma_of = [&](int k) __attribute__((always_inline)) -> float {
            if constexpr (AVK) {
                if (av_mixed) return av_ld(av_row(k), LP_C_RSIGMA);
            }
            return rc.rsigma;
        };
        auto elem_of = [&](int k, float mk) __attribute__((always_inline)) -> ElemCoef {
            float ax = rc.ax, ay = rc.ay, dx = rc.dx, dy = rc.dy, dtx = rc.dtx, dty = rc.dty, sq = rc.sqrt_abt, oma = rc.oma,
                  sc = rc.scale, valid = rc.valid;
            if constexpr (AVK) {
                if (av_mixed) {
                    const float* c = av_row(k);
                    ax = av_ld(c, LP_C_AX); ay = av_ld(c, LP_C_AY); dx = av_ld(c, LP_C_DX); dy = av_ld(c, LP_C_DY);
                    dtx = av_ld(c, LP_C_DTX); dty = av_ld(c, LP_C_DTY); sq = av_ld(c, LP_C_SQRT_ABT); oma = av_ld(c, LP_C_OMA);
                    sc = av_ld(c, LP_C_SCALE); valid = av_ld(c, LP_C_VALID);
                }
            }
            const float om = 1.0f - mk;
            ElemCoef e;
            e.a = ax * om + ay * mk;
            e.d = dx * om + dy * mk;
            e.dt = dtx * om + dty * mk;
            e.sqrt_abt = sq;
            e.oma = oma;
            e.scale = sc;
            e.valid = valid != 0.0f;
            return e;
        };

        auto form_verdict = [&]() __attribute__((always_inline)) {
                const int it = d.es_index;
                {
                    const auto u = [&](int w) { return __builtin_amdgcn_readfirstlane(static_cast<int>((w & 1) ? es_words[w >> 1].y : es_words[w >> 1].x)); };
                    const auto u64 = [&](int w) { return (static_cast<uint64_t>(static_cast<uint32_t>(u(w + 1))) << 32) | static_cast<uint32_t>(u(w)); };
                    static_assert(offsetof(lp_es_state, enabled) == 28 && offsetof(lp_es_state, seq_base) == 32 &&
                                  offsetof(lp_es_state, abt_val) == 56, "lp_es_state layout");
                    es_lite.stopped = u(0); es_lite.counter = u(1); es_lite.n_ran = u(2); es_lite.cur_slot = u(3);
                    es_lite.anchor_slot = u(4); es_lite.write_slot = u(5); es_lite.enabled = u(7);
                    es_lite.seq_base = static_cast<int64_t>(u64(8)); es_lite.total_ran = static_cast<int64_t>(u64(10));
                    es_lite.threshold_eff = __longlong_as_double(static_cast<long long>(u64(12)));
                    es_lite.abt_val = __longlong_as_double(static_cast<long long>(u64(14)));
                }
                int v_stopped = 0, v_cur = -1, v_anchor = -1, v_write = 0;
                bool v_have = false;
                if (it > 0 && es_lite.stopped == 0) {
                    __shared__ int fold_out[4];
                    if (threadIdx.x < kWave) {
                        float tot[kEsSums];
                        if constexpr (VEC == 4) {
                            const double* src = es_acc_set(d, d.es_index - 1) + static_cast<size_t>(threadIdx.x) * 8;
#pragma unroll
                            for (int k = 0; k < kEsSums; ++k) es_fv[k] = src[k];
                        }
                        if constexpr (VEC != 4) {
#pragma unroll
                            for (int k = 0; k < kEsSums; ++k) asm volatile("" : "+v"(es_fv[k]));
                        }
                        es_slot_total(es_fv, tot);
                        const bool hp = es_lite.cur_slot >= 0, ha = es_lite.anchor_slot >= 0;
                        es_decide(d, es_lite, tot, hp, ha, it - 1, es_keeper);
                        if (threadIdx.x == 0) {
                            fold_out[0] = es_lite.stopped; fold_out[1] = es_lite.cur_slot;
                            fold_out[2] = es_lite.anchor_slot; fold_out[3] = es_lite.write_slot;
                        }
                    }
                    __syncthreads();
                    v_stopped = fold_out[0]; v_cur = fold_out[1]; v_anchor = fold_out[2]; v_write = fold_out[3];
                    v_have = true;
                }
                if ((fl & LP_FL_ES_CLOSE) && it + 1 == d.es_n_steps) {
                    if (es_lite.stopped == 0) {
                        es_lite.n_ran = it + 1;
                        es_lite.total_ran += 1;
                    }
                    if (es_keeper) {
                        es_store_dynamic(d.es + (it & 1), es_lite);
                        if (double* host = d.es_host) {
                            host[1] = static_cast<double>(es_lite.n_ran); host[2] = static_cast<double>(es_lite.stopped);
                            host[3] = es_lite.enabled ? 1.0 : 0.0; host[4] = es_lite.threshold_eff; host[5] = es_lite.abt_val;
                            host[6] = static_cast<double>(es_lite.total_ran);
                            es_post_seq(host, es_lite.seq_base + LP_ES_SEQ_DONE);
                        }
                    }
                } else if (es_keeper) {
                    es_store_dynamic(d.es + (it & 1), es_lite);
                }
                es_prev = v_have ? v_cur : es_lite.cur_slot; es_anchor = v_have ? v_anchor : es_lite.anchor_slot;
                es_write = v_have ? v_write : es_lite.write_slot;
                es_idle = (v_have ? v_stopped : es_lite.stopped) != 0;
        };
        if constexpr (ES == 2 && VEC == 4) form_verdict();
        float m[VEC], xt[VEC], yv[VEC], cv[VEC], x0[VEC], x0b[VEC], xi_a[VEC], xi_b[VEC], corr[VEC];
        float xv[VEC], kn[VEC], nv[VEC], rs[VEC], abt_e[VEC], ve_e[VEC];
        Raw<VEC> m_raw, x0_raw, x0b_raw;
        const uint32_t mfl = HARD ? static_cast<uint32_t>(LP_FL_MASK_BITS) : (PH != 0 ? (fl & ~LP_FL_MASK_U8) : fl);
        if constexpr (!SMALL) load_mask_raw<VEC>(d.mask, mfl, i, m_raw);
        constexpr bool RA = HARD && VEC == 4 && (PH & kPost) != 0;
        constexpr bool UNI = HARD && VEC == 4 && (PH & (kPost | LP_PH_PRE_HALF)) != 0 && (PH & LP_PH_REPLACE) == 0;
        constexpr bool MIXSEL = UNI && ES == 0;
        int uni = -1;
        bool need_x0 = true, need_known = true;
        bool lane_x0 = true, lane_known = true;
        bool pair_x0 = true, pair_known = true;
        if constexpr (PER_EL) {
            load_f32<VEC>(d.abt_el, i, abt_e);
            if (!flow) load_f32<VEC>(d.ve_el, i, ve_e);
        }
        if (ph & LP_PH_REPLACE) {
            load_f32<VEC>(d.x, i, xv);
            bool need_kn = true;
            if constexpr (HARD && VEC == 4 && (PH & LP_PH_REPLACE) != 0) {
                if (!(fl & LP_FL_NO_REGION_SKIP)) {
                    const uint32_t nib = (m_raw.w[0] >> (static_cast<uint32_t>(i) & 31u)) & 0xFu;
                    need_kn = __ballot(nib != 0u) != 0ull;
                }
            }
            if (!need_kn) {
#pragma unroll
                for (int k = 0; k < VEC; ++k) kn[k] = 0.0f, nv[k] = 0.0f, yv[k] = 0.0f;
            } else if (d.replace_kind == LP_REPLACE_KNOWN) {
                load_f32<VEC>(d.known, i, kn);
            } else {
                load_f32<VEC>(d.noise, i, nv);
                load_f32<VEC>(d.y, i, yv);
                if constexpr (PER_EL) load_f32<VEC>(d.rsig_el, i, rs);
            }
        } else {
            load_f32<VEC>((ES && es_gated && (ph & LP_PH_POST_STEADY)) ? d.es_xte : d.x_t, i, xt);
        }
        if ((ph & LP_PH_POST_STEADY) || ((ph & LP_PH_PRE_HALF) && !post)) load_f32<VEC>(d.C, i, cv);
        if constexpr (UNI) {
            const uint32_t nib = (m_raw.w[0] >> (static_cast<uint32_t>(i) & 31u)) & 0xFu;
            const bool any_known = __ballot(nib != 0u) != 0ull, any_inpaint = __ballot(nib != 0xFu) != 0ull;
            uni = !any_known ? 0 : (!any_inpaint ? 1 : -1);
        }
        if constexpr (RA) {
            if (!given && d.x0_big != d.x0 && !(fl & (LP_FL_CFG_FUSED | LP_FL_NO_REGION_SKIP))) {
                const uint32_t nib = (m_raw.w[0] >> (static_cast<uint32_t>(i) & 31u)) & 0xFu;
                need_known = uni != 0;
                need_x0 = uni != 1;
                lane_known = nib != 0u;
                lane_x0 = nib != 0xFu;
                if constexpr (PAIR) {
                    const uint32_t nib8 = (m_raw.w[0] >> (static_cast<uint32_t>(i) & 24u)) & 0xFFu;
                    pair_known = nib8 != 0u;
                    pair_x0 = nib8 != 0xFFu;
                }
            }
        }
        const int64_t i_x0 = i, i_kn = i;
        if (post) {
            if constexpr (PAIR) {
                if (need_x0) load_raw_pair(d.x0, i, pair_x0, x0_raw);
                if (!(d.x0_big == d.x0 || given) && need_known) load_raw_pair(d.x0_big, i, pair_known, x0b_raw);
            } else {
                if (need_x0 && lane_x0) load_raw_w<VEC, X0W>(d.x0, x0dt, i_x0, x0_raw);
                if (!(d.x0_big == d.x0 || given) && need_known && lane_known) load_raw_w<VEC, X0W>(d.x0_big, x0dt, i_kn, x0b_raw);
            }
        }
        if constexpr (SMALL) load_mask_raw<VEC>(d.mask, mfl, i, m_raw);
        const bool has_corr = d.corr_el != nullptr && !given;
        const bool host_post = HOT ? false : d.xi_post != nullptr, host_pre = HOT ? false : d.xi_pre != nullptr;
        const bool need_rng = (post && !host_post) || ((ph & LP_PH_PRE_HALF) && !host_pre);
        if (post) {
            if (!given && need_known && lane_known) load_f32<VEC>(d.y, i_kn, yv);
            if (host_post) load_f32<VEC>(d.xi_post, i, xi_a);
            if (has_corr) load_f32<VEC>(d.corr_el, i, corr);
        }
        if ((ph & LP_PH_PRE_HALF) && host_pre) load_f32<VEC>(d.xi_pre, i, xi_b);
        float x0p[VEC], anc[VEC], rg[VEC], es_b0[VEC], es_b1[VEC], es_b2[VEC];
        constexpr bool RING_BITS_ONLY = ES != 0 && HARD && PH != 0;
        const bool ring_bits = RING_BITS_ONLY || (fl & LP_FL_ES_RING_BITS) != 0;
        uint32_t rg_raw = 0u;
        auto load_ring = [&]() __attribute__((always_inline)) {
            if (!d.es_ring) return;
            if (ring_bits) {
                if constexpr (!ST) rg_raw = reinterpret_cast<const uint32_t*>(d.es_ring)[i >> 5];
            } else {
                if constexpr (!RING_BITS_ONLY) load_f32<VEC>(d.es_ring, i, rg);
            }
        };
        auto ring_weight = [&](int k) __attribute__((always_inline)) -> float {
            if (!d.es_ring) return 0.0f;
            if (ring_bits) {
                if constexpr (!ST) return static_cast<float>((rg_raw >> ((static_cast<uint32_t>(i) & 31u) + k)) & 1u);
                else return 0.0f;
            }
            if constexpr (!RING_BITS_ONLY) return rg[k];
            else return 0.0f;
        };
        if constexpr (ES) {
            if (post) {
                if constexpr (es_fold && VEC == 4) {
                } else if constexpr (es_fold) {
                    load_f32<VEC>(d.es_x0s[0], i, es_b0);
                    load_f32<VEC>(d.es_x0s[1], i, es_b1);
                    load_f32<VEC>(d.es_x0s[2], i, es_b2);
                } else {
                    if (es_prev >= 0) load_f32<VEC>(es_prev == 0 ? d.es_x0s[0] : es_prev == 1 ? d.es_x0s[1] : d.es_x0s[2], i, x0p);
                    if (es_anchor >= 0) load_f32<VEC>(es_anchor == 0 ? d.es_x0s[0] : es_anchor == 1 ? d.es_x0s[1] : d.es_x0s[2], i, anc);
                }
                if constexpr (!(es_fold && VEC == 4)) {
                    load_ring();
                }
            }
        }

        if constexpr (!SMALL) {
            if (need_rng && d.rng_offset_ptr) {
                rng_w0 = d.rng_offset_ptr[0];
                rng_w1 = d.rng_offset_ptr[1];
                rng_have = true;
            }
        }
        if (d.io_table_out && el_bx == 0 && blockIdx.y == 0 && threadIdx.x == 0) {
            d.io_table_out[0] = d.io_table_val[0];
            d.io_table_out[1] = d.io_table_val[1];
            if (d.io_valid) d.io_table_out[2] = 1ull;
        }
        if constexpr (PH == 0 || (PH & LP_PH_REPLACE) != 0) {
            if (d.es_reset && d.es && el_bx == 0 && blockIdx.y == 0) {
                if (d.es_partials) {
                    for (int k = threadIdx.x; k < kEsSets * kEsSlots * 8; k += kBlock) d.es_partials[k] = 0.0;
                }
                if (threadIdx.x == 0) es_reset_state(d, fold_coeffs);
            }
        }
        if constexpr (TBL) {
            float abt_f, ve_f, rs_f, tm_f;
            row_times(abt_f, ve_f, rs_f, tm_f);
            rc.scale = row_scale(flow, abt_f, ve_f);
            rc.rscale = 1.0f / rc.scale;
            rc.rsigma = rs_f;
        }

        LP_CLK(1)
        if (need_rng) {
            const bool torch_kind = RNG == 2 ? (d.rng_kind == LP_RNG_TORCH) : (RNG == 1);
            uint64_t seq = d.rng_offset, seed = d.rng_seed;
            if (rng_have) {
                seq += rng_w0;
                if (torch_kind) seed = rng_w1;
            }
            if (torch_kind) {
                const bool draw_post = post && !host_post, draw_pre = (ph & LP_PH_PRE_HALF) && !host_pre;
                const uint64_t off_pre = seq + (draw_post ? d.rng_inc : 0u);
                if constexpr (ST) {
                    static_assert(!ST || VEC == 4, "the ATen layout is four elements per lane");
                    __shared__ __attribute__((aligned(16))) float st_xi[2][4][kBlock];
                    const uint32_t aten_thread = static_cast<uint32_t>(g_raw);
                    if (draw_post) {
                        float z[4];
                        torch_normal4(aten_thread, seed, seq + 4ull * st_round, z);
#pragma unroll
                        for (int k = 0; k < 4; ++k) st_xi[0][k][threadIdx.x] = z[k];
                    }
                    if (draw_pre) {
                        float z[4];
                        torch_normal4(aten_thread, seed, off_pre + 4ull * st_round, z);
#pragma unroll
                        for (int k = 0; k < 4; ++k) st_xi[1][k][threadIdx.x] = z[k];
                    }
                    __syncthreads();
                    const int w = threadIdx.x >> 6, l4 = (threadIdx.x & 63) * 4;
                    if (draw_post) {
                        const float4 q = *reinterpret_cast<const float4*>(&st_xi[0][w][l4]);
                        xi_a[0] = q.x; xi_a[1] = q.y; xi_a[2] = q.z; xi_a[3] = q.w;
                    }
                    if (draw_pre) {
                        const float4 q = *reinterpret_cast<const float4*>(&st_xi[1][w][l4]);
                        xi_b[0] = q.x; xi_b[1] = q.y; xi_b[2] = q.z; xi_b[3] = q.w;
                    }
                } else {
                    const bool small = d.n_el <= static_cast<int64_t>(d.rng_bg);
#pragma unroll
                    for (int k = 0; k < VEC; ++k) {
                        const uint64_t li = static_cast<uint64_t>(elem_index(i, k));
                        if (draw_post) xi_a[k] = torch_normal<PH != 0>(li, seed, seq, d.rng_bg, small);
                        if (draw_pre) xi_b[k] = torch_normal<PH != 0>(li, seed, off_pre, d.rng_bg, small);
                    }
                }
            } else {
                const bool key_uniform = !SMALL && d.n_el <= 0xffffffffll;
                const uint32_t key0 = philox_key(seed, seq, 0);
                if constexpr (VEC == 4 && HOT) {
                    if (key_uniform) {
                        uint32_t e4[4];
#pragma unroll
                        for (int k = 0; k < 4; ++k) e4[k] = static_cast<uint32_t>(elem_index(i, k));
                        normal_pairs4_key<true>(e4, static_cast<uint32_t>(seq), key0, xi_a, xi_b);
                    } else {
#pragma unroll
                        for (int k = 0; k < VEC; ++k) normal_pair(static_cast<uint64_t>(elem_index(i, k)), seq, seed, xi_a[k], xi_b[k]);
                    }
                } else {
#pragma unroll
                for (int k = 0; k < VEC; ++k) {
                    float za, zb;
                    const uint64_t e = static_cast<uint64_t>(elem_index(i, k));
                    if (key_uniform) normal_pair_key<PH != 0>(static_cast<uint32_t>(e), static_cast<uint32_t>(seq), key0, za, zb);
                    else normal_pair(e, seq, seed, za, zb);
                    if (!host_post) xi_a[k] = za;
                    if (!host_pre) xi_b[k] = zb;
                }
                }
            }
        }

        if constexpr (ES == 2 && VEC == 4) {
            if (post) {
                if (es_prev >= 0) load_f32<VEC>(es_prev == 0 ? d.es_x0s[0] : es_prev == 1 ? d.es_x0s[1] : d.es_x0s[2], i, x0p);
                load_ring();
            }
        }
        LP_CLK(2)
        LP_CLK_LOADS(3)
        if constexpr (ES) {
            if constexpr (es_fold) {
                if constexpr (VEC != 4) form_verdict();
                if constexpr (VEC != 4) {
                    if (post) {
#pragma unroll
                        for (int k = 0; k < VEC; ++k) {
                            x0p[k] = es_prev == 0 ? es_b0[k] : es_prev == 1 ? es_b1[k] : es_b2[k];
                            anc[k] = es_anchor == 0 ? es_b0[k] : es_anchor == 1 ? es_b1[k] : es_b2[k];
                        }
                    }
                }
            }
        }
        LP_CLK(4)
        const bool live = active && !es_idle;

        if (UNI && uni >= 0) {
#pragma unroll
            for (int k = 0; k < VEC; ++k) m[k] = static_cast<float>(uni);
        } else {
            cvt_mask<VEC>(mfl, i, m_raw, m);
        }
        if (post) {
            if constexpr (PAIR) {
                cvt_raw_pair(x0dt, x0_raw, x0);
                if (!(d.x0_big == d.x0 || given)) cvt_raw_pair(x0dt, x0b_raw, x0b);
            } else {
                cvt_raw<VEC>(x0dt, x0_raw, x0, i);
                if (!(d.x0_big == d.x0 || given)) cvt_raw<VEC>(x0dt, x0b_raw, x0b, i);
            }
        }

        if (ph & LP_PH_REPLACE) {
            if (d.replace_kind != LP_REPLACE_KNOWN) {
#pragma unroll
                for (int k = 0; k < VEC; ++k) {
                    const float r = PER_EL ? rs[k] : row_rsigma_of(k);
                    kn[k] = (d.replace_kind == LP_REPLACE_VE) ? fmaf(nv[k], r, yv[k])
                                                              : (r * (d.noise_scale * nv[k]) + (1.0f - r) * yv[k]);
                }
            }
#pragma unroll
            for (int k = 0; k < VEC; ++k) {
                const float xr = fmaf(kn[k], m[k], xv[k] * (1.0f - m[k]));
                float sc;
                if constexpr (PER_EL) {
                    sc = flow ? (sqrtf(abt_e[k]) + sqrtf(1.0f - abt_e[k])) : sqrtf(1.0f + ve_e[k] * ve_e[k]);
                } else {
                    sc = row_scale_of(k);
                }
                if constexpr (VEC == 4 && !PER_EL && PH != 0) {
                    xt[k] = flow ? xr * sc : div_shared(xr, sc, rc.rscale);
                } else {
                    xt[k] = flow ? xr * sc : xr / sc;
                }
            }
        }

        auto half_valid = [&](float x, float c, float xi, const RegionCoef& q) __attribute__((always_inline)) -> float {
            return fmaf(q.e_half, x, fmaf(q.k_half, c, q.std_half * xi));
        };
        auto half_table = [&](float x, float c, float xi, const RegionCoef& q) __attribute__((always_inline)) -> float {
            return rc.valid != 0.0f ? half_valid(x, c, xi, q) : x;
        };
        auto half_step = [&](float x, float c, float xi, int k) __attribute__((always_inline)) -> float {
            const float mk = m[k];
            const bool table = HARD || (!PER_EL && !av_mixed && ((mk == 0.0f) || (mk == 1.0f)));
            if (table) {
                if constexpr (SMALL) return half_table(x, c, xi, rc.reg[mk == 1.0f ? 1 : 0]);
                if (mk == 1.0f) return half_table(x, c, xi, rc.reg[1]);
                return half_table(x, c, xi, rc.reg[0]);
            }
            if constexpr (!HARD) {
                ElemCoef e;
                if constexpr (PER_EL) {
                    e = elem_from_times(abt_e[k], flow ? 0.0f : ve_e[k], mk, flow, opl, d.beta, d.step_size, d.min_step_frac);
                } else {
                    e = elem_of(k, mk);
                }
                if (e.valid) return ou_general(x, e.dt / 2.0f, e.a, c, e.d, xi);
            }
            return x;
        };

        float x0s[VEC], xb[VEC];
        if constexpr (ES) {
            if (ph & LP_PH_POST_FIRST) {
#pragma unroll
                for (int k = 0; k < VEC; ++k) xb[k] = xt[k];
            }
        }

        if (post) {
            if (d.x0_big == d.x0 || given) {
#pragma unroll
                for (int k = 0; k < VEC; ++k) x0b[k] = x0[k];
            } else if (fl & LP_FL_CFG_FUSED) {
#pragma unroll
                for (int k = 0; k < VEC; ++k) {
                    const float c = x0[k], u = x0b[k], diff = c - u;
                    x0[k] = fmaf(diff, d.cfg_scale, u);
                    x0b[k] = fmaf(diff, d.cfg_scale_big, u);
                }
            }
            if (given) {
#pragma unroll
                for (int k = 0; k < VEC; ++k) yv[k] = 0.0f;
            }
            if constexpr (!HARD) {
                if (has_corr) {
#pragma unroll
                    for (int k = 0; k < VEC; ++k) {
                        float sc;
                        if constexpr (PER_EL) sc = flow ? (sqrtf(abt_e[k]) + sqrtf(1.0f - abt_e[k])) : sqrtf(1.0f + ve_e[k] * ve_e[k]);
                        else sc = row_scale_of(k);
                        const float xm = flow ? xt[k] / sc : xt[k] * sc;
                        x0[k] = xm + corr[k] * (x0[k] - xm);
                        x0b[k] = xm + corr[k] * (x0b[k] - xm);
                    }
                }
            }
            auto post_vals = [&](int k, const RegionCoef& q, bool known_el, float& s0, float& cn, float& xn) __attribute__((always_inline)) {
                s0 = (given || !known_el) ? x0[k] : fmaf(-lam, x0b[k], opl * yv[k]);
                cn = fmaf(q.cx0, s0, q.cxt * xt[k]);
                if (ph & LP_PH_POST_FIRST) {
                    xn = fmaf(q.e_full, xt[k], fmaf(q.k_full, cn, q.std_full * xi_a[k]));
                } else {
                    const float xd = fmaf(cn - cv[k], q.dt, xt[k]);
                    xn = fmaf(q.e_half, xd, fmaf(q.k_half, cv[k], q.std_half * xi_a[k]));
                }
            };
            auto post_valid = [&](int k, const RegionCoef& q, bool known_el) __attribute__((always_inline)) {
                float s0, cn, xn;
                post_vals(k, q, known_el, s0, cn, xn);
                x0s[k] = s0;
                xt[k] = xn;
                cv[k] = cn;
            };
            auto post_skipped = [&](int k) __attribute__((always_inline)) {
                x0s[k] = x0[k];
                if (ph & LP_PH_POST_FIRST) cv[k] = 0.0f;
            };
            auto post_table = [&](int k, const RegionCoef& q, bool known_el) __attribute__((always_inline)) {
                if (rc.valid != 0.0f) post_valid(k, q, known_el);
// ... 64 lines not shown
                    }
                }
            }
            }
            if ((fl & LP_FL_WRITE_X0S) && live) store_f32<VEC>(d.x0s, i, x0s);
            if constexpr (ES) {
                if (live) {
                    store_f32<VEC>(es_write == 0 ? d.es_x0s[0] : es_write == 1 ? d.es_x0s[1] : d.es_x0s[2], i, x0s);
                    if constexpr (ES == 2 && VEC == 4) {
                        if (es_anchor >= 0 && !(UNI && uni == 1))
                            load_f32<VEC>(es_anchor == 0 ? d.es_x0s[0] : es_anchor == 1 ? d.es_x0s[1] : d.es_x0s[2], i, anc);
                    }
                    if (UNI && uni == 1) {
                        es_zero_wave = true;
                    } else if (UNI && uni == 0 && !d.es_ring) {
#pragma unroll
                        for (int k = 0; k < VEC; ++k) {
                            const float da = es_prev >= 0 ? x0s[k] - x0p[k] : xt[k] - xb[k];
                            es_p[0] += da * da;
                            es_p[1] += 1.0f;
                            if (es_anchor >= 0) {
                                const float db = x0s[k] - anc[k];
                                es_p[4] += db * db;
                            }
                        }
                    } else {
#pragma unroll
                        for (int k = 0; k < VEC; ++k) {
                            const float w1 = 1.0f - m[k];
                            const float w2 = ring_weight(k);
                            const float da = es_prev >= 0 ? x0s[k] - x0p[k] : xt[k] - xb[k];
                            const float da2 = da * da;
                            es_p[0] += da2 * w1;
                            es_p[1] += w1;
                            es_p[2] += da2 * w2;
                            es_p[3] += w2;
                            if (es_anchor >= 0) {
                                const float db = x0s[k] - anc[k];
                                const float db2 = db * db;
                                es_p[4] += db2 * w1;
                                es_p[5] += db2 * w2;
                            }
                        }
                    }
                }
            }
        }

        float xe[VEC];
#pragma unroll
        for (int k = 0; k < VEC; ++k) xe[k] = xt[k];
        if (ph & LP_PH_PRE_HALF) {
            if (UNI && uni >= 0 && rc.valid == 0.0f) {
            } else if (UNI && uni == 0) {
#pragma unroll
                for (int k = 0; k < VEC; ++k) xe[k] = half_valid(xt[k], cv[k], xi_b[k], rc.reg[0]);
            } else if (UNI && uni == 1) {
#pragma unroll
                for (int k = 0; k < VEC; ++k) xe[k] = half_valid(xt[k], cv[k], xi_b[k], rc.reg[1]);
            } else if (MIXSEL && rc.valid != 0.0f) {
#pragma unroll
                for (int k = 0; k < VEC; ++k) {
                    const float ha = half_valid(xt[k], cv[k], xi_b[k], rc.reg[0]), hb = half_valid(xt[k], cv[k], xi_b[k], rc.reg[1]);
                    xe[k] = m[k] == 1.0f ? hb : ha;
                }
            } else {
#pragma unroll
                for (int k = 0; k < VEC; ++k) xe[k] = half_step(xt[k], cv[k], xi_b[k], k);
            }
            if (!(ES && es_gated)) {
#pragma unroll
                for (int k = 0; k < VEC; ++k) xt[k] = xe[k];
            }
        }

        LP_CLK(5)
        if (post && live) store_f32<VEC>(d.C, i, cv);
        if ((ph & kTouchXt) && live) store_f32<VEC>(d.x_t, i, xt);
        if constexpr (ES) {
            if (es_gated && (ph & LP_PH_PRE_HALF) && live) store_f32<VEC>(d.es_xte, i, xe);
            if (es_fold && es_idle) load_f32<VEC>(d.x_t, i, xe);
        }

        if (ph & LP_PH_EMIT) {
            float xo[VEC];
            if constexpr (VEC == 4 && !PER_EL && PH != 0) {
                const float sc = rc.scale;
                if (flow) {
                    float y;
                    if constexpr (ES != 0 || (RNG == 1 && !ST)) {
                        y = 1.0f / sc;
                        asm volatile("" : "+v"(y));
                    } else {
                        y = rc.rscale;
                    }
#pragma unroll
                    for (int k = 0; k < VEC; ++k) xo[k] = div_shared(xe[k], sc, y);
                } else {
#pragma unroll
                    for (int k = 0; k < VEC; ++k) xo[k] = xe[k] * sc;
                }
            } else {
#pragma unroll
                for (int k = 0; k < VEC; ++k) {
                    float sc;
                    if constexpr (PER_EL) {
                        sc = flow ? (sqrtf(abt_e[k]) + sqrtf(1.0f - abt_e[k])) : sqrtf(1.0f + ve_e[k] * ve_e[k]);
                    } else {
                        sc = row_scale_of(k);
                    }
                    xo[k] = flow ? xe[k] / sc : xe[k] * sc;
                }
            }
            if constexpr (PAIR) {
                if (xindt != DT_F32) store_half_pair(d.x_in, xindt, i, xo);
                else store_any<VEC>(d.x_in, xindt, i, xo);
            } else {
                if (active) store_any<VEC>(d.x_in, xindt, i, xo);
            }
        }
    }

    LP_CLK(6)
    if constexpr (!ES) {
        LP_CLK_FLUSH
    }
    if constexpr (ES) {
        if (es_idle || !post) return;
        __shared__ float es_part[4][kEsSums];
        const int lane = threadIdx.x & (kWave - 1), wave = threadIdx.x / kWave;
        if (!es_zero_wave) wave_sum_dpp(es_p);
        if (lane == kWave - 1) {
#pragma unroll
            for (int k = 0; k < kEsSums; ++k) es_part[wave][k] = es_p[k];
        }
        __syncthreads();
        const unsigned blk = blockIdx.y * gridDim.x + blockIdx.x;
        if (threadIdx.x < kEsSums && !(d.tune & LP_TUNE_ES_NO_ATOMICS)) {
            const float p0 = es_part[0][threadIdx.x], p1 = es_part[1][threadIdx.x], p2 = es_part[2][threadIdx.x],
                        p3 = es_part[3][threadIdx.x];
            const float v = ((p0 + p1) + p2) + p3;
            double* acc = es_acc_set(d, d.es_index) + static_cast<size_t>(blk % kEsSlots) * 8 + threadIdx.x;
            (void)unsafeAtomicAdd(acc, static_cast<double>(v));
        }
        if (blk == 0 && threadIdx.x >= kWave) {
            double* nxt = es_acc_set(d, d.es_index + 1);
            for (int k = threadIdx.x - kWave; k < kEsSlots * 8; k += kBlock - kWave) nxt[k] = 0.0;
        }
        LP_CLK(7)
        LP_CLK_FLUSH
    }
}

__global__ __launch_bounds__(64) void lp_es_decide_kernel(const lp_step_desc d, int slot) {
    const double* src = es_acc_set(d, d.es_index) + static_cast<size_t>(threadIdx.x) * 8;
    double v[kEsSums];
#pragma unroll
    for (int k = 0; k < kEsSums; ++k) v[k] = __builtin_nontemporal_load(src + k);
    lp_es_state st;
    if (threadIdx.x == 0) st = d.es[slot];
    const bool gated = (d.flags & LP_FL_ES_GATED) != 0;
    float tot[kEsSums];
    es_slot_total(v, tot);
    if (threadIdx.x != 0) return;
    if (gated && st.stopped != 0) {
        if (d.es_index + 1 == d.es_n_steps) {
            d.es[0] = st;
            d.es[1] = st;
            if (d.es_host) es_post_seq(d.es_host, st.seq_base + LP_ES_SEQ_DONE);
        }
        return;
    }
    es_decide(d, st, tot, st.cur_slot >= 0, st.anchor_slot >= 0, d.es_index, true);
    d.es[0] = st;
    d.es[1] = st;
}

struct Timer {
    hipEvent_t start, stop;
};

static unsigned st_segments(const lp_step_desc& d) {
    const int64_t span = 4 * static_cast<int64_t>(d.rng_bg);
    const int64_t rounds = (d.n_el + span - 1) / span;
    int64_t per_round = (span + d.el_per_row - 1) / d.el_per_row + 1;
    if (per_round > d.rows) per_round = d.rows;
    const int64_t gy = rounds * per_round;
    return (gy > 0 && gy <= 65535 && static_cast<int64_t>(d.rng_inc) == 4 * rounds) ? static_cast<unsigned>(gy) : 0u;
}


template <int VEC, int MODE, uint32_t PH, int X0W = 0, int RNG = 2, bool ST = false, int ES = 0>
static void plan_kernel(const lp_step_desc& d, StepPlan* p) {
    const int64_t groups = ST ? static_cast<int64_t>(d.rng_bg) : d.el_per_row / VEC;
    int64_t bx = (groups + kBlock - 1) / kBlock;
    if (bx < 1) bx = 1;
    if constexpr ((PH & LP_PH_COEFFS) != 0 && VEC == 1) bx += 1;
    const unsigned gy = ST ? st_segments(d) : static_cast<unsigned>(d.rows);
    *p = StepPlan{reinterpret_cast<const void*>(&lp_step_kernel<VEC, MODE, PH, X0W, RNG, ST, ES>), dim3(static_cast<unsigned>(bx), gy),
                  PH, VEC, false, 0, MODE, X0W, RNG, ES, ST};
}

template <int VEC, int MODE, uint32_t PH, int X0W = 0, int RNG = 2>
static void plan_es(const lp_step_desc& d, StepPlan* p) {
    const bool fold = (d.flags & LP_FL_ES_GATED) && !(d.tune & LP_TUNE_ES_NO_FOLD);
    if constexpr (PH != 0) {
        if (!fold) return plan_es<VEC, MODE, 0>(d, p);
        plan_kernel<VEC, MODE, PH, X0W, RNG, false, 2>(d, p);
    } else {
        if (fold) plan_kernel<VEC, MODE, PH, X0W, RNG, false, 2>(d, p);
        else plan_kernel<VEC, MODE, PH, X0W, RNG, false, 1>(d, p);
    }
    const bool close = fold && (d.flags & LP_FL_ES_CLOSE) && d.es_index + 1 == d.es_n_steps;
    p->decide = (d.phases & kPost) && !(d.tune & LP_TUNE_ES_NO_DECIDE) && !close && (!fold || d.es_index + 1 == d.es_n_steps);
    p->decide_slot = fold ? (d.es_index & 1) : 0;
}

template <int VEC, int MODE, uint32_t PH>
static void plan_hot(const lp_step_desc& d, bool strided, bool x0_half, bool rng_torch, StepPlan* p) {
    if (strided) return x0_half ? plan_kernel<4, MODE, PH, 2, 1, true>(d, p) : plan_kernel<4, MODE, PH, 4, 1, true>(d, p);
    if (x0_half) return rng_torch ? plan_kernel<VEC, MODE, PH, 2, 1>(d, p) : plan_kernel<VEC, MODE, PH, 2, 0>(d, p);
    return rng_torch ? plan_kernel<VEC, MODE, PH, 4, 1>(d, p) : plan_kernel<VEC, MODE, PH, 4, 0>(d, p);
}

static bool aligned(const void* p, size_t a) { return p == nullptr || (reinterpret_cast<uintptr_t>(p) % a) == 0; }

template <int VEC>
static void plan_phase(const lp_step_desc& d, StepPlan* p) {
    if (d.flags & LP_FL_PER_ELEMENT) return plan_kernel<VEC, MODE_PER_EL, 0>(d, p);
    constexpr uint32_t R = LP_PH_REPLACE, F = LP_PH_POST_FIRST, S = LP_PH_POST_STEADY, P = LP_PH_PRE_HALF,
                       E = LP_PH_EMIT;
    const bool hard = (d.flags & LP_FL_MASK_BITS) && d.corr_el == nullptr;
    if (d.flags & LP_FL_AV)
        return (d.flags & LP_FL_ES) ? plan_es<VEC, MODE_ROW, 0>(d, p) : plan_kernel<VEC, MODE_ROW, 0>(d, p);
    const bool rare = (d.flags & LP_FL_X0S_GIVEN) || d.xi_post || d.xi_pre;
    const bool x0_half = x0_dtype(d.flags) != DT_F32;
    const bool pair_ok = VEC != 4 || !x0_half ||
                         (aligned(d.x0, 16) && aligned(d.x0_big, 16) && (xin_dtype(d.flags) == DT_F32 || aligned(d.x_in, 16)) &&
                          d.el_per_row % 8 == 0);
    if (d.flags & LP_FL_ES) {
        if (hard && !x0_half && !rare && (!d.es_ring || (d.flags & LP_FL_ES_RING_BITS))) {
            const bool rt = d.rng_kind == LP_RNG_TORCH;
            if (d.phases == (S | P | E))
                return rt ? plan_es<VEC, MODE_HARD, S | P | E, 4, 1>(d, p) : plan_es<VEC, MODE_HARD, S | P | E, 4, 0>(d, p);
            if (d.phases == (F | P | E))
                return rt ? plan_es<VEC, MODE_HARD, F | P | E, 4, 1>(d, p) : plan_es<VEC, MODE_HARD, F | P | E, 4, 0>(d, p);
        }
        return hard ? plan_es<VEC, MODE_HARD, 0>(d, p) : plan_es<VEC, MODE_ROW, 0>(d, p);
    }
    if (d.flags & LP_FL_MASK_U8) return plan_kernel<VEC, MODE_ROW, 0>(d, p);
    if (d.phases == (R | E | LP_PH_COEFFS))
        return hard ? plan_kernel<VEC, MODE_HARD, R | E | LP_PH_COEFFS>(d, p) : plan_kernel<VEC, MODE_ROW, R | E | LP_PH_COEFFS>(d, p);
    if (d.phases == (R | E | LP_PH_COEFFS | LP_PH_SIGMA))
        return plan_kernel<VEC, MODE_HARD, R | E | LP_PH_COEFFS | LP_PH_SIGMA>(d, p);
    const bool rng_torch = d.rng_kind == LP_RNG_TORCH;
    const bool strided = VEC == 4 && rng_torch && !d.xi_post && !d.xi_pre && d.n_el > static_cast<int64_t>(d.rng_bg) &&
                         (d.rng_bg % kBlock) == 0 &&
                         (d.rows == 1 || d.el_per_row >= 2 * static_cast<int64_t>(d.rng_bg)) && st_segments(d) != 0;
    if (!pair_ok || rare) return hard ? plan_kernel<VEC, MODE_HARD, 0>(d, p) : plan_kernel<VEC, MODE_ROW, 0>(d, p);
    if (hard) {
        switch (d.phases) {
            case S | P | E: return plan_hot<VEC, MODE_HARD, S | P | E>(d, strided, x0_half, rng_torch, p);
            case F | P | E: return plan_hot<VEC, MODE_HARD, F | P | E>(d, strided, x0_half, rng_torch, p);
            case S | E: return plan_hot<VEC, MODE_HARD, S | E>(d, strided, x0_half, rng_torch, p);
            default: return plan_kernel<VEC, MODE_HARD, 0>(d, p);
        }
    }
    switch (d.phases) {
        case S | P | E: return plan_hot<VEC, MODE_ROW, S | P | E>(d, strided, x0_half, rng_torch, p);
        case F | P | E: return plan_hot<VEC, MODE_ROW, F | P | E>(d, strided, x0_half, rng_torch, p);
        case S | E: return plan_hot<VEC, MODE_ROW, S | E>(d, strided, x0_half, rng_torch, p);
        default: return plan_kernel<VEC, MODE_ROW, 0>(d, p);
    }
}

int plan_step(const lp_step_desc& d, StepPlan* out, bool timed) {
    if (d.n_el <= 0 || d.rows <= 0 || d.el_per_row <= 0 || d.n_el != d.el_per_row * d.rows) return LP_E_INVALID;
    if (d.rows > 65535 || d.el_per_row > 0x7fffffff) return LP_E_UNSUPPORTED;
    if (!d.mask || !d.x_t) return LP_E_INVALID;
    if ((d.flags & LP_FL_MASK_BITS) && ((d.flags & (LP_FL_MASK_U8 | LP_FL_MASK_DENOISE)) || !aligned(d.mask, 4)))
        return LP_E_INVALID;
    const uint32_t ph = d.phases;
    if (ph == 0 || (ph & ~0x7fu)) return LP_E_INVALID;
    if (ph & LP_PH_SIGMA) {
        if (ph != (LP_PH_REPLACE | LP_PH_EMIT | LP_PH_COEFFS | LP_PH_SIGMA) || !(d.flags & LP_FL_MASK_BITS) || d.corr_el ||
            d.replace_kind == LP_REPLACE_KNOWN)
            return LP_E_INVALID;
        if (!d.sg_sigma || !d.sg_schedule || d.sg_schedule_len <= 0 || !d.sg_scalars_out) return LP_E_INVALID;
        if (d.es_reset) return LP_E_UNSUPPORTED;
    }
    if (d.flags & LP_FL_AV) {
        if (!d.av_bits || !aligned(d.av_bits, 4) || !d.coef || (d.flags & LP_FL_PER_ELEMENT) || (ph & (LP_PH_COEFFS | LP_PH_SIGMA)) ||
            !(d.av_frac >= 0.0f && d.av_frac <= 1.0f))
            return LP_E_INVALID;
    }
    if (d.rng_kind != LP_RNG_PHILOX && d.rng_kind != LP_RNG_TORCH) return LP_E_INVALID;
    if (d.rng_kind == LP_RNG_TORCH && (d.rng_bg == 0 || (d.rng_inc & 3u) || d.rng_inc == 0)) return LP_E_INVALID;
    if (ph & LP_PH_COEFFS) {
        if ((ph & ~LP_PH_SIGMA) != (LP_PH_REPLACE | LP_PH_EMIT | LP_PH_COEFFS) || (d.flags & LP_FL_PER_ELEMENT)) return LP_E_INVALID;
        if (!d.coef_out) return LP_E_INVALID;
        if (!(ph & LP_PH_SIGMA)) {
            if (!d.t_abt || (!(d.flags & LP_FL_FLOW) && !d.t_ve)) return LP_E_INVALID;
            if (d.replace_kind != LP_REPLACE_KNOWN && !d.t_rsig) return LP_E_INVALID;
        }
    }
    if ((ph & LP_PH_POST_FIRST) && (ph & LP_PH_POST_STEADY)) return LP_E_INVALID;
    if ((ph & LP_PH_REPLACE) && (ph & (kPost | LP_PH_PRE_HALF))) return LP_E_INVALID;
    const bool per_el = d.flags & LP_FL_PER_ELEMENT;
    if (!per_el && !d.coef && !(ph & LP_PH_COEFFS)) return LP_E_INVALID;
    if (per_el && (!d.abt_el || (!(d.flags & LP_FL_FLOW) && !d.ve_el))) return LP_E_INVALID;
    if (ph & LP_PH_REPLACE) {
        if (!d.x) return LP_E_INVALID;
        if (d.replace_kind == LP_REPLACE_KNOWN) {
            if (!d.known) return LP_E_INVALID;
        } else if (d.replace_kind == LP_REPLACE_VE || d.replace_kind == LP_REPLACE_FLOW) {
            if (!d.noise || !d.y) return LP_E_INVALID;
            if (per_el && !d.rsig_el) return LP_E_INVALID;
        } else {
            return LP_E_INVALID;
        }
    }
    if (ph & kPost) {
        const bool given = d.flags & LP_FL_X0S_GIVEN;
        if (!d.x0 || !d.C || (!given && (!d.x0_big || !d.y))) return LP_E_INVALID;
        if ((d.flags & LP_FL_WRITE_X0S) && !d.x0s) return LP_E_INVALID;
    }
    if ((ph & LP_PH_PRE_HALF) && !d.C) return LP_E_INVALID;
    if ((ph & LP_PH_EMIT) && !d.x_in) return LP_E_INVALID;
    if (d.es_reset && !d.es) return LP_E_INVALID;
    if (d.flags & LP_FL_ES) {
        if (timed) return LP_E_UNSUPPORTED;
        if (per_el || !d.es || !d.es_partials || d.es_index < 0 || d.es_n_steps <= d.es_index) return LP_E_INVALID;
        if (!d.es_x0s[0] || !d.es_x0s[1] || !d.es_x0s[2]) return LP_E_INVALID;
        if ((d.flags & LP_FL_ES_GATED) && !d.es_xte) return LP_E_INVALID;
        if ((d.flags & LP_FL_ES_CLOSE) && !(d.flags & LP_FL_ES_GATED)) return LP_E_INVALID;
        if ((d.flags & LP_FL_ES_RING_BITS) && (!(d.flags & LP_FL_MASK_BITS) || !aligned(d.es_ring, 4))) return LP_E_INVALID;
    } else if (d.flags & (LP_FL_ES_GATED | LP_FL_ES_CLOSE | LP_FL_ES_RING_BITS)) {
        return LP_E_INVALID;
    }

    const size_t half_al = 8, f_al = 16;
    const bool x0_half = x0_dtype(d.flags) != DT_F32, xin_half = xin_dtype(d.flags) != DT_F32;
    const bool can_vec4 = (d.el_per_row % 4 == 0) && aligned(d.x, f_al) && aligned(d.known, f_al) &&
                          aligned(d.noise, f_al) && aligned(d.y, f_al) &&
                          aligned(d.mask, (d.flags & (LP_FL_MASK_U8 | LP_FL_MASK_BITS)) ? 4 : f_al) && aligned(d.x_t, f_al) &&
                          aligned(d.C, f_al) && aligned(d.x0s, f_al) && aligned(d.x0, x0_half ? half_al : f_al) &&
                          aligned(d.x0_big, x0_half ? half_al : f_al) && aligned(d.x_in, xin_half ? half_al : f_al) &&
                          aligned(d.xi_post, f_al) && aligned(d.xi_pre, f_al) && aligned(d.abt_el, f_al) &&
                          aligned(d.ve_el, f_al) && aligned(d.rsig_el, f_al) && aligned(d.corr_el, f_al);
    bool vec4 = can_vec4 && d.n_el > 512 * 1024;
    if (d.tune & LP_TUNE_VEC4) vec4 = can_vec4;
    if (d.tune & LP_TUNE_VEC1) vec4 = false;
    if (vec4) plan_phase<4>(d, out);
    else plan_phase<1>(d, out);
    return LP_OK;
}

void pack_step_args(const StepPlan& p, const lp_step_desc& d, StepArgs* a) {
    const bool rep = (p.ph_ct & LP_PH_REPLACE) != 0, lead_y = rep || p.vec != 1;
    a->x_t = d.x_t;
    a->C = d.C;
    a->a2 = rep ? static_cast<const void*>(d.x) : d.x0;
    a->a3 = rep ? static_cast<const void*>(d.replace_kind == LP_REPLACE_KNOWN ? d.known : d.noise) : d.x0_big;
    a->a4 = lead_y ? static_cast<const void*>(d.y) : static_cast<const void*>(d.coef);
    a->a5 = lead_y ? d.mask : static_cast<const void*>(d.rng_offset_ptr);
    a->el_per_row = static_cast<int32_t>(d.el_per_row);
    a->flags = d.flags;
    void* const ptr[9] = {&a->x_t, &a->C, &a->a2, &a->a3, &a->a4, &a->a5, &a->el_per_row, &a->flags, const_cast<lp_step_desc*>(&d)};
    for (int k = 0; k < 9; ++k) a->ptr[k] = ptr[k];
}

bool plan_is_node(const StepPlan& p, const void* func, const dim3& grid, const dim3& block) {
    return !p.decide && func == p.kernel && grid.x == p.grid.x && grid.y == p.grid.y && grid.z == p.grid.z &&
           block.x == static_cast<unsigned>(kBlock) && block.y == 1 && block.z == 1;
}

#ifdef LP_TRACE_INSTANTIATIONS
}
#include <cstdio>
#include <cstdlib>
#include <mutex>
#include <set>
#include <string>
namespace lp {
struct TraceSet {
    std::mutex mu;
    std::set<std::string> seen;
    ~TraceSet() {
        const char* path = std::getenv("LANPAINT_AMD_TRACE_FILE");
        if (!path || seen.empty()) return;
        if (FILE* f = std::fopen(path, "a")) {
            for (const auto& s : seen) std::fprintf(f, "%s\n", s.c_str());
            std::fclose(f);
        }
    }
};
static TraceSet& trace_set() {
    static TraceSet t;
    return t;
}
static void trace_note(const StepPlan& p) {
    char buf[96];
    std::snprintf(buf, sizeof buf, "%d, %d, %uu, %d, %d, %s, %d", p.vec, p.mode, p.ph_ct, p.x0w, p.rng, p.st ? "true" : "false", p.es);
    TraceSet& t = trace_set();
    std::lock_guard<std::mutex> lock(t.mu);
    t.seen.insert(buf);
}
#define LP_TRACE(p) trace_note(p)
#else
#define LP_TRACE(p)
#endif

static int enqueue(const StepPlan& p, const lp_step_desc& d, hipStream_t stream, Timer* timer) {
    LP_TRACE(p);
    StepArgs a;
    pack_step_args(p, d, &a);
    if (timer) (void)hipExtLaunchKernel(p.kernel, p.grid, dim3(kBlock), a.ptr, 0, stream, timer->start, timer->stop, 0);
    else (void)hipLaunchKernel(p.kernel, p.grid, dim3(kBlock), a.ptr, 0, stream);
    if (hipGetLastError() != hipSuccess) return LP_E_LAUNCH;
    if (p.decide) {
        hipLaunchKernelGGL(lp_es_decide_kernel, dim3(1), dim3(kWave), 0, stream, d, p.decide_slot);
        if (hipGetLastError() != hipSuccess) return LP_E_LAUNCH;
    }
    return LP_OK;
}

int step_dispatch(const lp_step_desc* dp, hipStream_t stream, void* timer_handle) {
    if (!dp) return LP_E_INVALID;
    Timer* timer = static_cast<Timer*>(timer_handle);
    StepPlan p;
    const int rc = plan_step(*dp, &p, timer != nullptr);
    return rc == LP_OK ? enqueue(p, *dp, stream, timer) : rc;
}

int replace_node_update(const lp_step_desc* dp, hipGraphExec_t exec, const lp_graph_binding* b) {
    if (!dp || !exec || !b || !b->node || !b->func) return LP_E_INVALID;
    const lp_step_desc& d = *dp;
    if (!(d.phases & LP_PH_REPLACE) || d.xi_post || d.xi_pre || (d.flags & LP_FL_X0S_GIVEN)) return LP_E_INVALID;
    StepPlan p;
    const int rc = plan_step(d, &p);
    if (rc != LP_OK) return rc;
    if (!plan_is_node(p, b->func, dim3(b->grid[0], b->grid[1], b->grid[2]), dim3(b->block[0], b->block[1], b->block[2])))
        return LP_E_INVALID;
    StepArgs a;
    pack_step_args(p, d, &a);
    hipKernelNodeParams np{};
    np.func = const_cast<void*>(p.kernel);
    np.gridDim = p.grid;
    np.blockDim = dim3(kBlock);
    np.sharedMemBytes = b->shared_bytes;
    np.kernelParams = a.ptr;
    np.extra = nullptr;
    return hipGraphExecKernelNodeSetParams(exec, static_cast<hipGraphNode_t>(b->node), &np) == hipSuccess ? LP_OK : LP_E_LAUNCH;
}

int timer_create(void** out) {
    if (!out) return LP_E_INVALID;
    Timer* t = new Timer();
    if (hipEventCreate(&t->start) != hipSuccess || hipEventCreate(&t->stop) != hipSuccess) {
        delete t;
        return LP_E_LAUNCH;
    }
    *out = t;
    return LP_OK;
}

int timer_destroy(void* h) {
    if (!h) return LP_E_INVALID;
    Timer* t = static_cast<Timer*>(h);
    (void)hipEventDestroy(t->start);
    (void)hipEventDestroy(t->stop);
    delete t;
    return LP_OK;
}

int timer_elapsed_ns(void* h, double* ns) {
    if (!h || !ns) return LP_E_INVALID;
    Timer* t = static_cast<Timer*>(h);
    if (hipEventSynchronize(t->stop) != hipSuccess) return LP_E_LAUNCH;
    float ms = 0.f;
    if (hipEventElapsedTime(&ms, t->start, t->stop) != hipSuccess) return LP_E_LAUNCH;
    *ns = static_cast<double>(ms) * 1e6;
    return LP_OK;
}

}
```

lanpaint_amd/engine.py:

```python
from __future__ import annotations

import ctypes
import os
import weakref
from collections import OrderedDict
from time import perf_counter

import torch

from . import _cabi
from ._cabi import (LP_FL_ES, LP_FL_ES_GATED, LP_FL_ES_CLOSE, LP_FL_CFG_FUSED, LP_FL_FLOW, LP_FL_MASK_BITS, LP_FL_MASK_U8, LP_FL_XIN_BF16,
                    LP_FL_XIN_F16, LP_FL_PER_ELEMENT, LP_FL_WRITE_X0S, LP_FL_X0_BF16, LP_FL_X0_F16, LP_FL_X0S_GIVEN, LP_PH_EMIT,
                    LP_PH_POST_FIRST, LP_PH_POST_STEADY, LP_PH_PRE_HALF, LP_PH_REPLACE, LP_REPLACE_FLOW, LP_REPLACE_KNOWN,
                    LP_REPLACE_VE)
from ._util import _as_f32c, _noise_scaling_kind, aten_randn_policy, raw_stream, tensor_version
from .buffers import _CallState, _Workspace
from .earlystop import HostStopper, StopOptions
from .masks import _compact_mask, pack_indicator, pack_mask, refresh_packed_mask
from .types import FusedCFGHeads


class EngineCore:

    def __init__(self, Model, NSteps, Friction, Lambda, Beta, StepSize, IS_FLUX=False, IS_FLOW=False,
                 EarlyStopThreshold=0.0, EarlyStopPatience=1, EarlyStopHook=None, MinStepFrac=0.0,
                 *, rng=None, philox_seed=None, graph=None, model_dtype=None, early_stop_group=None):
        self.n_steps = NSteps
        self.chara_lamb = Lambda
        self.IS_FLUX = IS_FLUX
        self.IS_FLOW = IS_FLOW
        self.step_size = StepSize
        self.inner_model = Model
        self.friction = Friction
        self.chara_beta = Beta
        self.min_step_frac = MinStepFrac
        self.img_dim_size = None
        self.early_stop_threshold = EarlyStopThreshold
        self.early_stop_patience = EarlyStopPatience
        self.early_stop_hook = EarlyStopHook

        self.rng = rng if rng is not None else os.environ.get("LANPAINT_AMD_RNG", "torch")
        if not callable(self.rng) and self.rng not in ("torch", "torch-eager", "philox"):
            raise ValueError(f"rng must be 'torch', 'torch-eager', 'philox' or a callable, got {self.rng!r}")
        self._torch_consumed = 0
        self._graph_blocked = False
        self.philox_seed = philox_seed
        self._philox_offset = 0
        if graph is None:
            graph = {"1": True, "0": False}.get(os.environ.get("LANPAINT_AMD_GRAPH", "auto"), "auto")
        self.graph = "auto" if graph == "auto" else bool(graph)
        self._auto = None
        if model_dtype not in (None, torch.float32, torch.bfloat16, torch.float16):
            raise ValueError(f"model_dtype must be None, float32, bfloat16 or float16, got {model_dtype}")
        self.model_dtype = None if model_dtype == torch.float32 else model_dtype
        self._graphs = OrderedDict()
        self._static_ws = {}
        self._last_cap = None
        self._es_close = False
        self._rng_counters = {}
        self._capturing = None
        self._cap_offset = 0
        self._lib = _cabi.load()
        self._ws = None
        self._desc = _cabi.LpStepDesc()
        self._fdesc = _cabi.LpFinalDesc()
        self._hyper = _cabi.LpHyper()
        self._noise_check = None
        self.assume_static_noise = False
        self.auto_pack_mask = os.environ.get("LANPAINT_AMD_AUTO_PACK", "1") != "0"
        self._mask_seen = None
        self._noise_regenerated = False
        self._iterations_run = 0
        self.last_inner_steps = 0
        self.early_stop_group = early_stop_group
        self._ds = None
        self._es_opts = None
        self._es_pending = None

    @property
    def iterations_run(self):
        self._es_resolve()
        return self._iterations_run

    @iterations_run.setter
    def iterations_run(self, v):
        self._iterations_run = v

    def _indicator_pack(self, indicator, shape):
        c = getattr(self, "_av_pack", None)
        if c is None or c[0] is not indicator or c[1] != tuple(shape):
            c = self._av_pack = (indicator, tuple(shape), pack_indicator(indicator, shape))
        return c[2]

    def _auto_pack(self, latent_mask, x):
        if not self.auto_pack_mask or self.graph is True or not latent_mask.is_cuda or latent_mask.dtype != torch.float32 \
                or not latent_mask.is_contiguous() or latent_mask.shape != x.shape or latent_mask.numel() == 0 \
                or getattr(latent_mask, "_lp_u8", None) is not None:
            return
        ver = (tensor_version(latent_mask), latent_mask.data_ptr())
        if ver[0] == -1:
            return
        seen = self._mask_seen
        if seen is None or seen[0]() is not latent_mask or seen[1] != ver:
            self._mask_seen = (weakref.ref(latent_mask), ver, False)
            return
        if seen[2]:
            return
        try:
            pack_mask(latent_mask, check=True)
            latent_mask._lp_auto = True
        except ValueError:
            self._mask_seen = (seen[0], seen[1], True)
        except Exception:
            self.auto_pack_mask = False

    def rng_position(self, device):
        if self.rng == "philox":
            st = self._rng_counters.get(device)
            return (int(st[0].item()) if st is not None else 0, int(self._philox_offset))
        gen = self._generator(device)
        return (int(gen.get_offset()), int(gen.initial_seed()))

    def _es_options(self, model_options):
        o = StopOptions.parse(model_options, self.early_stop_threshold, self.early_stop_patience, self.early_stop_hook)
        if o is None:
            return None
        return {"threshold": o.threshold, "patience_eff": o.patience_eff, "distance_fn": o.distance_fn, "trace": o.trace,
                "tags": o.tags, "device": not callable(o.distance_fn) and self.early_stop_group is None, "parsed": o}

    def add_none_dims(self, array):
        while array.ndim < self.img_dim_size:
            array = array.unsqueeze(array.ndim)
        return array

    def remove_none_dims(self, array):
        return array[(slice(None),) + (0,) * (self.img_dim_size - 1)]

    def unpack_model_output(self, output):
        if isinstance(output, FusedCFGHeads):
            return output.materialize()
        if isinstance(output, (tuple, list)):
            if len(output) >= 2:
                return output[0], output[1]
            if len(output) == 1:
                return output[0], output[0]
            raise ValueError("Model output is empty")
        return output, output

    def sigma_x(self, abt):
        return abt ** 0

    def sigma_y(self, abt):
        return self.chara_beta * abt ** 0

    def prepare_step_size(self, current_times, step_size, sigma_x, sigma_y):
        sigma, abt, _flow_t = current_times
        sigma, abt = self.add_none_dims(sigma), self.add_none_dims(abt)
        dtx, dty = 2 * step_size * sigma_x, 2 * step_size * sigma_y
        gam_x = self.friction ** 2 * self.step_size * sigma_x / 0.1 * sigma ** 0 / 2.0
        gam_y = self.friction ** 2 * self.step_size * sigma_y / 0.1 * sigma ** 0 / 2.0
        a_t_x = 1 / (1 - abt) * dtx / 2
        a_t_y = (1 + self.chara_lamb) / (1 - abt) * dty / 2
        a_x, a_y = a_t_x / (dtx / 2), a_t_y / (dty / 2)
        d = (2 * abt ** 0) ** 0.5
        return sigma, abt, dtx / 2, dty / 2, gam_x / (dtx / 2), gam_y / (dty / 2), a_x, a_y, d, d

    def score_model(self, x_t, y, mask, abt, sigma, tflow, model_options, seed):
        lamb = self.chara_lamb
        if self.IS_FLUX or self.IS_FLOW:
            x = x_t / (abt ** 0.5 + (1 - abt) ** 0.5)
            t = self.remove_none_dims(tflow)
        else:
            x = x_t * (1 + sigma ** 2) ** 0.5
            t = self.remove_none_dims(sigma)
        x_0, x_0_big = self.unpack_model_output(self.inner_model(x, t, model_options=model_options, seed=seed))
        corr = getattr(self, "audio_correction", None)
        if corr is not None:
            x_0 = x + corr * (x_0 - x)
            x_0_big = x + corr * (x_0_big - x)
        score_x = -(x_t - x_0)
        score_y = -(1 + lamb) * (x_t - y) + lamb * (x_t - x_0_big)
        return score_x * (1 - mask) + score_y * mask

    def _overridden(self, name):
        return name in self.__dict__ or getattr(type(self), name) is not self._OWN_METHODS[self._OWN_NAMES.index(name)]

    def _stream(self, device):
        return raw_stream(device)

    def _noise_is_zero(self, noise):
        c = self._noise_check
        ver = (tensor_version(noise), noise.data_ptr())
        stale = ver[0] == -1 and not self.assume_static_noise
        if c is None or c[0]() is not noise or c[1] != ver or stale:
            self._noise_check = c = (weakref.ref(noise), ver, bool(torch.mean(torch.abs(noise)) < 1e-8))
        return c[2]

    def _draw(self, like):
        if self.rng == "philox":
            return None
        xi = self.rng(like) if callable(self.rng) else torch.randn_like(like)
        return _as_f32c(xi)

    @staticmethod
    def _generator(device):
        torch.cuda.init()
        return torch.cuda.default_generators[device.index if device.index is not None else torch.cuda.current_device()]

    _policy_cache = {}

    @classmethod
    def _randn_policy(cls, device, numel):
        key = (device.index, numel)
        hit = cls._policy_cache.get(key)
# ... 207 lines not shown
        corr = self.audio_correction
        if per_el:
            st.base_flags = base_flags = base_flags | LP_FL_PER_ELEMENT
            abt_el = _as_f32c(self.add_none_dims(abt).expand(shape))
            ve_el = _as_f32c(self.add_none_dims(VE_Sigma).expand(shape))
            rs_el = _as_f32c(self.add_none_dims(replace_sigma).expand(shape))
            keep += [abt_el, ve_el, rs_el]
            d.abt_el, d.ve_el, d.rsig_el = abt_el.data_ptr(), ve_el.data_ptr(), rs_el.data_ptr()
            d.coef = None
        elif av is not None:
            st.base_flags = base_flags = base_flags | _cabi.LP_FL_AV
            tv = ws.av_times
            _cabi.check(lib.lp_coeffs(ctypes.byref(hyp), tv[0].data_ptr(), 1, tv[1].data_ptr(), 1, tv[2].data_ptr(), 1, None, 0,
                                      tv[3].data_ptr(), 1, 2 * rows, ws.coef_av.data_ptr(), stream), "lp_coeffs")
            d.coef, d.coef_out = ws.coef_av.data_ptr(), None
            d.av_bits, d.av_frac = av[0].data_ptr(), float(av[1])
            keep.append(av[0])
        else:
            flat = lambda t: _as_f32c(t if t.ndim == 1 else t.reshape(-1))
            ve_r, abt_r, rs_r, tm_r = flat(VE_Sigma), flat(abt), flat(replace_sigma), flat(t_model)
            keep += [ve_r, abt_r, rs_r, tm_r]
            d.t_ve, d.t_abt, d.t_rsig, d.t_model = ve_r.data_ptr(), abt_r.data_ptr(), rs_r.data_ptr(), tm_r.data_ptr()
            d.t_ve_stride, d.t_abt_stride = ve_r.numel() > 1, abt_r.numel() > 1
            d.t_rsig_stride, d.t_model_stride = rs_r.numel() > 1, tm_r.numel() > 1
            d.coef = d.coef_out = ws.coef.data_ptr()
        if corr is not None:
            corr_el = _as_f32c(corr if corr.shape == shape else corr.expand(shape))
            if ws.static_io:
                if getattr(ws, "corr", None) is None:
                    ws.corr = torch.empty_like(ws.x_t)
                ws.corr.copy_(corr_el)
                corr_el = ws.corr
            keep.append(corr_el)
            d.corr_el = corr_el.data_ptr()
        if ws.static_io and not per_el:
            n_t, n_s = (rows if t_model.numel() > 1 else 1), (rows if sigma.numel() > 1 else 1)
            table = ws.coef if av is None else ws.coef_av.view(rows, 2 * _cabi.LP_COEF_STRIDE)
            st.t_model, st.sigma_model = table[:n_t, _cabi.LP_C_TMODEL], table[:n_s, _cabi.LP_C_RSIGMA]
        else:
            st.t_model, st.sigma_model = t_model, sigma

        ms = self.inner_model.inner_model.model_sampling
        d.noise_scale = 1.0
        d.known = None
        d.noise = nz.data_ptr()
        if replace_sigma.numel() == 1 and av is None:
            kind, ns = _noise_scaling_kind(ms)
            if kind == "callback":
                known = _as_f32c(ms.noise_scaling(self.add_none_dims(replace_sigma), nz, y))
                keep.append(known)
                d.replace_kind, d.known = LP_REPLACE_KNOWN, known.data_ptr()
            elif kind == "ve":
                d.replace_kind = LP_REPLACE_VE
            else:
                d.replace_kind, d.noise_scale = LP_REPLACE_FLOW, ns
        else:
            d.replace_kind, d.noise_scale = LP_REPLACE_FLOW, float(getattr(ms, "noise_scale", 1.0))

        st.compat = self._overridden("langevin_dynamics") or self._overridden("score_model") or \
            self._overridden("prepare_step_size")
        if n_steps > 0 and float(self.step_size) <= 0.0 and not st.compat:
            n_steps = 0
        st.n_steps = n_steps

        if ws.static_io:
            st.x_final, st.x_in = ws.x_final, ws.x_in
        else:
            st.x_final = torch.empty_like(xc)
            st.x_in = st.x_final if self.model_dtype is None else torch.empty_like(xc, dtype=self.model_dtype)
        st.xin_flag = 0 if self.model_dtype is None else (LP_FL_XIN_BF16 if self.model_dtype == torch.bfloat16 else LP_FL_XIN_F16)

        d.x = xc.data_ptr()
        d.xi_post = d.xi_pre = None
        d.rng_offset_ptr = None
        d.rng_seed = int(self.philox_seed if self.philox_seed is not None else (seed or 0)) & 0xFFFFFFFFFFFFFFFF
        d.rng_state_out = None
        if ws.static_io and self.rng == "torch" and not per_el:
            gen = self._generator(xc.device)
            d.rng_state_out = self._rng_state(xc.device).data_ptr()
            d.rng_state_val[0], d.rng_state_val[1] = gen.get_offset(), gen.initial_seed()
        d.flags = base_flags | self._emit(st, n_steps == 0)
        d.phases = LP_PH_REPLACE | LP_PH_EMIT | (0 if (per_el or av is not None) else _cabi.LP_PH_COEFFS)
        st.out = None
        if ws.static_io and not per_el:
            st.out = out if out is not None else torch.empty_like(xc)
            d.io_table_out, d.io_valid = self._rng_state(xc.device).data_ptr() + 16, 1
            d.io_table_val[0], d.io_table_val[1] = xc.data_ptr(), st.out.data_ptr()
        st.es = None
        es = self._es_opts
        d.es, d.es_reset = None, 0
        if es is not None and es["device"] and not per_el and not st.compat and (corr is None or av is not None) and n_steps > 0:
            ds = ds if ds is not None else self._device_stop(xc, n_steps)
            ring = ds.ring_for(latent_mask if latent_mask.shape == shape else m, m)
            ring_bits = ds.ring_bits() if (ring is not None and m_flag == LP_FL_MASK_BITS) else None
            st.es = dict(es, ds=ds, seq=ds.next_seq(), ring=ring, ring_flag=_cabi.LP_FL_ES_RING_BITS if ring_bits is not None else 0)
            d.es, d.es_reset, d.es_seq_base = ds.state.data_ptr(), 1, st.es["seq"]
            d.es_threshold, d.es_patience_eff, d.es_n_steps = es["threshold"], es["patience_eff"], n_steps
            d.es_host, d.es_partials = ds.mailbox.data_ptr(), ds.partials.data_ptr()
            for k in range(3):
                d.es_x0s[k] = ds.x0s[k].data_ptr()
            d.es_ring = ring_bits.data_ptr() if ring_bits is not None else (ring.data_ptr() if ring is not None else None)
            d.es_xte = ds.x_te.data_ptr()
        if not defer_launch:
            self._launch_step(stream)
        st.replace_kind_static = d.replace_kind != LP_REPLACE_KNOWN and not per_el and av is None
        st.k0_desc = _cabi.LpStepDesc.from_buffer_copy(d) if ws.static_io else None
        d.io_table_out, d.io_valid = None, 0
        d.es_reset = 0
        return st

    def _emit(self, st, final):
        d = self._desc
        if final:
            d.x_in = st.x_final.data_ptr()
            return 0
        d.x_in = st.x_in.data_ptr()
        return st.xin_flag

    def _think_and_final_model(self, st, model_options, seed):
        d, ws, shape, base_flags, n_steps, stream = self._desc, st.ws, st.shape, st.base_flags, st.n_steps, st.stream
        d.n_el, d.el_per_row, d.rows = st.n_el, st.n_el // st.rows, st.rows
        stopper = None
        if self._capturing is None and st.es is None:
            stopper = HostStopper.from_options(
                StopOptions.parse(model_options, self.early_stop_threshold, self.early_stop_patience, self.early_stop_hook),
                st.m, st.abt)
            if stopper is not None and self.early_stop_group is not None:
                stopper.sums.reduce_group = self.early_stop_group
        ran = 0
        if st.compat:
            ran = self._loop_compat(ws, shape, st.m, st.y, st.abt, st.current_times, n_steps, model_options, seed, stopper)
            d.phases = LP_PH_EMIT
            d.flags = base_flags | self._emit(st, True)
            self._launch_step(stream)
        elif st.es is not None:
            ran = self._loop_es(st, n_steps, model_options, seed)
        elif stopper is not None:
            ran = self._loop_unfused(st, n_steps, model_options, seed, stopper)
        else:
            auto = self._auto if (self.graph == "auto" and self._capturing is None) else None
            bb_s = 0.0
            for i in range(n_steps):
                last = i == n_steps - 1
                if auto is not None:
                    t_bb = perf_counter()
                    output = self.inner_model(st.x_in, st.t_model, model_options=model_options, seed=seed)
                    bb_s += perf_counter() - t_bb
                else:
                    output = self.inner_model(st.x_in, st.t_model, model_options=model_options, seed=seed)
                alive = self._set_model_output(d, output, base_flags | self._emit(st, last), shape)
                d.phases = (LP_PH_POST_FIRST if i == 0 else LP_PH_POST_STEADY) | (0 if last else LP_PH_PRE_HALF) | LP_PH_EMIT
                self._set_xi(d, ws.x_t, want_pre=not last)
                self._launch_step(stream)
                del alive
            ran = n_steps
            if auto is not None and n_steps > 0:
                auto[1] += 1
                auto[2] = min(auto[2], bb_s / n_steps)
        self._iterations_run += ran
        self.last_inner_steps = ran
        x_model = st.x_final if self.model_dtype is None else st.x_final.to(self.model_dtype)
        return self.inner_model(x_model, st.sigma_model, model_options=model_options, seed=seed)

    def _fill_final_desc(self, f, st, final, out):
        shape = st.shape
        converted = []

        def dense(t):
            t0 = t
            if t.shape != shape:
                t = t.expand(shape)
            if t.dtype not in (torch.float32, torch.bfloat16, torch.float16):
                t = t.float()
            t = t if t.is_contiguous() else t.contiguous()
            if t is not t0:
                converted.append(t)
            return t

        uncond = None
        if isinstance(final, FusedCFGHeads) and final._heads is None and final.cond.dtype == final.uncond.dtype:
            out_model, uncond = dense(final.cond), dense(final.uncond)
            f.cfg_scale = final.scale
        else:
            out_model = dense(self.unpack_model_output(final)[0])
        f.n_el = st.n_el
        f.flags = (LP_FL_X0_BF16 if out_model.dtype == torch.bfloat16 else
                   LP_FL_X0_F16 if out_model.dtype == torch.float16 else 0) | (LP_FL_CFG_FUSED if uncond is not None else 0) \
            | st.m_flag
        f.uncond = uncond.data_ptr() if uncond is not None else None
        f.model_out, f.y = out_model.data_ptr(), st.y.data_ptr()
        f.mask = st.m_c.data_ptr() if st.m_c is not None else st.m.data_ptr()
        f.x_src, f.x_dst, f.out = st.x_final.data_ptr(), st.xc.data_ptr(), out.data_ptr()
        f.rng_bump_ptr, f.rng_bump, f.io_table = None, 0, None
        self._final_alive = (out_model, uncond)
        return not converted

    def _epilogue(self, st, final, rng_bump=None, in_graph=False):
        f, xc = self._fdesc, st.xc
        out = st.out if st.out is not None else torch.empty_like(xc)
        if not in_graph:
            self._fill_final_desc(f, st, final, out)
            if rng_bump is not None:
                f.rng_bump_ptr, f.rng_bump = rng_bump[0].data_ptr(), int(rng_bump[1])
            _cabi.check(self._lib.lp_finalize(ctypes.byref(f), st.stream), "lp_finalize")
        if xc is not st.input_x:
            st.input_x.copy_(xc)
        return out if out.dtype == st.input_x.dtype else out.to(st.input_x.dtype)

    def _set_xi(self, d, like, want_pre, want_post=True):
        if self.rng == "philox":
            d.xi_post = d.xi_pre = None
            d.rng_kind = _cabi.LP_RNG_PHILOX
            if self._capturing is not None:
                d.rng_offset, d.rng_offset_ptr = self._cap_offset, self._capturing.data_ptr()
                self._cap_offset += 1
            else:
                d.rng_offset, d.rng_offset_ptr = (1 << 48) + self._philox_offset, None
                self._philox_offset += 1
            self._xi_alive = None
            return
        if self.rng == "torch":
            d.xi_post = d.xi_pre = None
            d.rng_kind = _cabi.LP_RNG_TORCH
            d.rng_bg, d.rng_inc = self._randn_policy(like.device, like.numel())
            used = (int(bool(want_post)) + int(bool(want_pre))) * d.rng_inc
            if self._capturing is not None:
                d.rng_offset, d.rng_offset_ptr = self._cap_offset, self._capturing.data_ptr()
                self._cap_offset += used
            else:
                gen = self._generator(like.device)
                off = gen.get_offset()
                d.rng_seed, d.rng_offset, d.rng_offset_ptr = gen.initial_seed(), off, None
                gen.set_offset(off + used)
                self._torch_consumed += used
            self._xi_alive = None
            return
        xa = self._draw(like) if want_post else None
        xb = self._draw(like) if want_pre else None
        d.xi_post = xa.data_ptr() if xa is not None else None
        d.xi_pre = xb.data_ptr() if xb is not None else None
        self._xi_alive = (xa, xb)
```

Measured before the change: 117,600 think-iterations/s.

## Pass think-step RNG state by value through graph node parameter updates

At replay, each captured think-step kernel node is now bound and updated with the RNG seed and offset passed directly as kernel arguments, instead of reading the offset through a device pointer. This removes the dependent load of the RNG state at kernel start. When a single draw per lane suffices, the kernel can start generating the Philox normal before its other loads. The cost is one graph node parameter update per step on every replay, plus a more complex binding and validation path.

```diff
diff --git a/include/lanpaint_hip.h b/include/lanpaint_hip.h
--- a/include/lanpaint_hip.h
+++ b/include/lanpaint_hip.h
@@ -80,6 +80,8 @@
 #define LP_FL_ES_RING_BITS  (1u << 16)
 #define LP_FL_AV            (1u << 17)
 #define LP_FL_X0S_GIVEN     (1u << 9)
+#define LP_FL_STATE_ARGS       (1u << 30)
+#define LP_FL_STATE_ONE_THREAD (1u << 31)
 
 typedef struct lp_es_state {
     int32_t  stopped;
@@ -229,6 +231,10 @@
     void*                graph_exec;
     const lp_final_desc* final;
     const struct lp_graph_binding* replace_binding;
+    const lp_step_desc*  steps;
+    const struct lp_graph_binding* step_bindings;
+    int32_t              n_steps;
+    int32_t              reserved_steps;
 } lp_call_desc;
 LP_API int lp_replay_call(const lp_call_desc* call, void* stream);
 
@@ -240,6 +246,7 @@
     uint32_t reserved0;
 } lp_graph_binding;
 LP_API int lp_graph_bind_replace(void* graph, const lp_step_desc* captured_replace, lp_graph_binding* out);
+LP_API int lp_graph_bind_steps(void* graph, const lp_step_desc* captured, int32_t n, lp_graph_binding* out);
 LP_API int lp_graph_clone_tail(void* graph, void** tail_graph_out, void** tail_exec_out);
 LP_API int lp_graph_release(void* tail_graph, void* tail_exec);
 LP_API int lp_graph_clone_sigma_root(void* graph, const lp_step_desc* with_sigma, void** graph_out, void** exec_out,
diff --git a/lanpaint_amd/_cabi.py b/lanpaint_amd/_cabi.py
--- a/lanpaint_amd/_cabi.py
+++ b/lanpaint_amd/_cabi.py
@@ -21,6 +21,7 @@
 LP_FL_X0_BF16, LP_FL_X0_F16, LP_FL_XIN_BF16, LP_FL_XIN_F16 = 16, 32, 64, 128
 LP_FL_PER_ELEMENT, LP_FL_X0S_GIVEN, LP_FL_CFG_FUSED, LP_FL_MASK_BITS, LP_FL_NO_REGION_SKIP = 256, 512, 1024, 2048, 4096
 LP_FL_ES, LP_FL_ES_GATED, LP_FL_ES_CLOSE, LP_FL_ES_RING_BITS, LP_FL_AV = 1 << 13, 1 << 14, 1 << 15, 1 << 16, 1 << 17
+LP_FL_STATE_ARGS, LP_FL_STATE_ONE_THREAD = 1 << 30, 1 << 31
 LP_TUNE_VEC1, LP_TUNE_VEC4, LP_TUNE_ES_NO_DECIDE, LP_TUNE_ES_NO_FOLD, LP_TUNE_ES_NO_ATOMICS = 1, 2, 4, 8, 16
 
 
@@ -104,6 +105,8 @@
         ("graph_exec", C.c_void_p),
         ("final", C.POINTER(LpFinalDesc)),
         ("replace_binding", C.POINTER(LpGraphBinding)),
+        ("steps", C.POINTER(LpStepDesc)), ("step_bindings", C.POINTER(LpGraphBinding)),
+        ("n_steps", C.c_int32), ("reserved_steps", C.c_int32),
     ]
 
 
@@ -322,6 +325,7 @@
                                C.c_int32, C.c_void_p]),
     "lp_replay_call": (C.c_int, [C.POINTER(LpCallDesc), C.c_void_p]),
     "lp_graph_bind_replace": (C.c_int, [C.c_void_p, C.POINTER(LpStepDesc), C.POINTER(LpGraphBinding)]),
+    "lp_graph_bind_steps": (C.c_int, [C.c_void_p, C.POINTER(LpStepDesc), C.c_int32, C.POINTER(LpGraphBinding)]),
     "lp_graph_clone_tail": (C.c_int, [C.c_void_p, C.POINTER(C.c_void_p), C.POINTER(C.c_void_p)]),
     "lp_graph_release": (C.c_int, [C.c_void_p, C.c_void_p]),
     "lp_graph_clone_sigma_root": (C.c_int, [C.c_void_p, C.POINTER(LpStepDesc), C.POINTER(C.c_void_p), C.POINTER(C.c_void_p),
diff --git a/lanpaint_amd/buffers.py b/lanpaint_amd/buffers.py
--- a/lanpaint_amd/buffers.py
+++ b/lanpaint_amd/buffers.py
@@ -125,6 +125,8 @@
         self.times_seen = ()
         self.node_table = None
         self.binding = None
+        self.step_descs = None
+        self.step_bindings = None
         self.tail_handles = None
         self.sigma_root = None
 
diff --git a/lanpaint_amd/capture.py b/lanpaint_amd/capture.py
--- a/lanpaint_amd/capture.py
+++ b/lanpaint_amd/capture.py
@@ -343,6 +343,14 @@
         if cap.es is not None and st.es is not None:
             self._es_after_replay(cap, st.es["seq"], x.device)
         return out
+
+    def _bind_steps(self, cap, raw_graph, steps, n_steps):
+        if not steps or len(steps) != n_steps or os.environ.get("LANPAINT_AMD_STEP_STATE_ARGS", "1") == "0":
+            return
+        descs = (_cabi.LpStepDesc * len(steps))(*steps)
+        binds = (_cabi.LpGraphBinding * len(steps))()
+        if self._lib.lp_graph_bind_steps(raw_graph, descs, len(steps), binds) == _cabi.LP_OK:
+            cap.step_descs, cap.step_bindings = descs, binds
 
     def _replay_fast(self, cap, x, sigma, current_times):
         lib, stream = self._lib, self._stream(x.device)
@@ -474,6 +482,7 @@
                                  replace_in_graph=False)
         self._iterations_run = it0
         self._capturing, self._cap_offset = counter, 0
+        self._cap_steps = [] if replace_in_graph and self.rng == "torch" else None
         _gc_hold()
         try:
             f = _cabi.LpFinalDesc()
@@ -490,6 +499,7 @@
                     cap.final_in_graph = True
         finally:
             self._capturing = None
+            cap_steps, self._cap_steps = self._cap_steps, None
             _gc_release()
         cap.launches = self._cap_offset
         self._es_opts = es_user
@@ -516,6 +526,7 @@
                         raw_graph, ctypes.byref(cap.k0_desc), ctypes.byref(b)) == _cabi.LP_OK
                     if ok:
                         cap.binding = b
+                        self._bind_steps(cap, raw_graph, cap_steps, st.n_steps)
                         tg, te = ctypes.c_void_p(), ctypes.c_void_p()
                         if self._lib.lp_graph_clone_tail(raw_graph, ctypes.byref(tg), ctypes.byref(te)) == _cabi.LP_OK:
                             cap.tail_handles = (tg.value, te.value)
@@ -536,6 +547,8 @@
             c.rows, c.coef_table, c.graph_exec = st.rows, cap.ws.coef.data_ptr(), cap.raw_exec
             if cap.binding is not None:
                 c.replace_binding = ctypes.pointer(cap.binding)
+                if cap.step_bindings is not None:
+                    c.steps, c.step_bindings, c.n_steps = cap.step_descs, cap.step_bindings, len(cap.step_descs)
                 if cap.tail_handles is not None:
                     t = cap.tail = _cabi.LpCallDesc()
                     t.rows, t.coef_table, t.graph_exec = st.rows, cap.ws.coef.data_ptr(), cap.tail_handles[1]
diff --git a/lanpaint_amd/csrc/cabi.hip b/lanpaint_amd/csrc/cabi.hip
--- a/lanpaint_amd/csrc/cabi.hip
+++ b/lanpaint_amd/csrc/cabi.hip
@@ -1,10 +1,12 @@
+#include <algorithm>
 #include <cmath>
+#include <vector>
 
 #include "lp_common.h"
 
 namespace lp {
 int step_dispatch(const lp_step_desc* d, hipStream_t stream, void* timer);
-int replace_node_update(const lp_step_desc* d, hipGraphExec_t exec, const lp_graph_binding* b);
+int step_node_update(const lp_step_desc* d, hipGraphExec_t exec, const lp_graph_binding* b, bool replace);
 int timer_create(void** out);
 int timer_destroy(void* h);
 int timer_elapsed_ns(void* h, double* ns);
@@ -192,8 +194,19 @@
     return lp::wmse_dispatch(a, b, mask, ring, n_el, acc, block_scratch, scratch_blocks, as_stream(stream));
 }
 
+static bool bindable_step(const lp_step_desc& d) {
+    return !(d.phases & LP_PH_REPLACE) && !(d.flags & (LP_FL_ES | LP_FL_X0S_GIVEN)) && !d.xi_post && !d.xi_pre &&
+           d.rng_kind == LP_RNG_TORCH && d.rng_offset_ptr != nullptr;
+}
+
 int lp_replay_call(const lp_call_desc* c, void* stream) {
     if (!c || (!c->replace && !c->graph_exec && !c->final)) return LP_E_INVALID;
+    if (c->n_steps < 0) return LP_E_INVALID;
+    if (c->n_steps > 0) {
+        if (!c->steps || !c->step_bindings || !c->graph_exec || !c->replace || !c->replace_binding) return LP_E_INVALID;
+        for (int32_t k = 0; k < c->n_steps; ++k)
+            if (!bindable_step(c->steps[k])) return LP_E_INVALID;
+    }
     hipStream_t s = as_stream(stream);
     int rc = LP_OK;
     if (c->hyper)
@@ -202,11 +215,19 @@
     if (rc != LP_OK) return rc;
     if (c->replace && c->replace_binding) {
         if (!c->graph_exec) return LP_E_INVALID;
-        rc = lp::replace_node_update(c->replace, static_cast<hipGraphExec_t>(c->graph_exec), c->replace_binding);
+        rc = lp::step_node_update(c->replace, static_cast<hipGraphExec_t>(c->graph_exec), c->replace_binding, true);
     } else if (c->replace) {
         rc = lp::step_dispatch(c->replace, s, nullptr);
     }
     if (rc != LP_OK) return rc;
+    for (int32_t k = 0; k < c->n_steps; ++k) {
+        lp_step_desc d = c->steps[k];
+        d.rng_seed = c->replace->rng_state_val[1];
+        d.rng_offset = c->replace->rng_state_val[0] + c->steps[k].rng_offset;
+        d.rng_offset_ptr = nullptr;
+        rc = lp::step_node_update(&d, static_cast<hipGraphExec_t>(c->graph_exec), &c->step_bindings[k], false);
+        if (rc != LP_OK) return rc;
+    }
     if (c->graph_exec && hipGraphLaunch(static_cast<hipGraphExec_t>(c->graph_exec), s) != hipSuccess) return LP_E_LAUNCH;
     return c->final ? lp::finalize_dispatch(c->final, s) : LP_OK;
 }
@@ -235,6 +256,63 @@
     out->grid[0] = p.gridDim.x; out->grid[1] = p.gridDim.y; out->grid[2] = p.gridDim.z;
     out->block[0] = p.blockDim.x; out->block[1] = p.blockDim.y; out->block[2] = p.blockDim.z;
     out->shared_bytes = p.sharedMemBytes; out->reserved0 = 0;
+    return LP_OK;
+}
+
+int lp_graph_bind_steps(void* graph, const lp_step_desc* captured, int32_t n, lp_graph_binding* out) {
+    if (!graph || !captured || !out || n <= 0 || n > 4096) return LP_E_INVALID;
+    std::vector<lp::StepPlan> plans(static_cast<size_t>(n));
+    for (int32_t k = 0; k < n; ++k) {
+        if (!bindable_step(captured[k])) return LP_E_INVALID;
+        const int rc = lp::plan_step(captured[k], &plans[k]);
+        if (rc != LP_OK) return rc;
+    }
+    hipGraph_t g = static_cast<hipGraph_t>(graph);
+    size_t n_root = 0;
+    if (hipGraphGetRootNodes(g, nullptr, &n_root) != hipSuccess || n_root != 1) return LP_E_UNSUPPORTED;
+    hipGraphNode_t root = nullptr;
+    if (hipGraphGetRootNodes(g, &root, &n_root) != hipSuccess || !root) return LP_E_UNSUPPORTED;
+    std::vector<hipGraphNode_t> nodes{root};
+    for (size_t at = 0; at < nodes.size(); ++at) {
+        if (nodes.size() > 65536) return LP_E_UNSUPPORTED;
+        size_t n_dep = 0;
+        if (hipGraphNodeGetDependentNodes(nodes[at], nullptr, &n_dep) != hipSuccess) return LP_E_UNSUPPORTED;
+        if (n_dep == 0) continue;
+        std::vector<hipGraphNode_t> dep(n_dep);
+        if (hipGraphNodeGetDependentNodes(nodes[at], dep.data(), &n_dep) != hipSuccess) return LP_E_UNSUPPORTED;
+        for (size_t j = 0; j < n_dep; ++j)
+            if (dep[j] && std::find(nodes.begin(), nodes.end(), dep[j]) == nodes.end()) nodes.push_back(dep[j]);
+    }
+    std::vector<lp_graph_binding> found(static_cast<size_t>(n));
+    std::vector<int> hits(static_cast<size_t>(n), 0);
+    for (hipGraphNode_t node : nodes) {
+        hipGraphNodeType ty;
+        if (hipGraphNodeGetType(node, &ty) != hipSuccess) return LP_E_UNSUPPORTED;
+        if (ty != hipGraphNodeTypeKernel) continue;
+        hipKernelNodeParams p{};
+        if (hipGraphKernelNodeGetParams(node, &p) != hipSuccess || !p.func) return LP_E_UNSUPPORTED;
+        for (int32_t k = 0; k < n; ++k) {
+            if (!lp::plan_is_node(plans[k], p.func, p.gridDim, p.blockDim) || !p.kernelParams) continue;
+            void* const* kp = p.kernelParams;
+            const lp_step_desc* dn = static_cast<const lp_step_desc*>(kp[8]);
+            const lp_step_desc& c = captured[k];
+            if (!dn || *static_cast<void* const*>(kp[0]) != c.x_t || dn->phases != c.phases || dn->n_el != c.n_el ||
+                dn->rng_offset != c.rng_offset || *static_cast<const void* const*>(kp[5]) != c.rng_offset_ptr)
+                continue;
+            lp_graph_binding& b = found[k];
+            b.node = node; b.func = p.func;
+            b.grid[0] = p.gridDim.x; b.grid[1] = p.gridDim.y; b.grid[2] = p.gridDim.z;
+            b.block[0] = p.blockDim.x; b.block[1] = p.blockDim.y; b.block[2] = p.blockDim.z;
+            b.shared_bytes = p.sharedMemBytes; b.reserved0 = 0;
+            ++hits[k];
+        }
+    }
+    for (int32_t k = 0; k < n; ++k)
+        if (hits[k] != 1) return LP_E_UNSUPPORTED;
+    for (int32_t k = 0; k < n; ++k)
+        for (int32_t j = 0; j < k; ++j)
+            if (found[j].node == found[k].node) return LP_E_UNSUPPORTED;
+    for (int32_t k = 0; k < n; ++k) out[k] = found[k];
     return LP_OK;
 }
 
@@ -352,7 +430,7 @@
                                   ? static_cast<hipGraphExec_t>(c->full_exec_by_count[c->guess]) : nullptr;
         const lp_graph_binding* fb = full ? c->full_binding_by_count[c->guess] : nullptr;
         if (full && fb) {
-            rc = lp::replace_node_update(&d, full, fb);
+            rc = lp::step_node_update(&d, full, fb, true);
             if (rc != LP_OK) return rc;
             if (hipGraphLaunch(full, s) != hipSuccess) return LP_E_LAUNCH;
             *queued_spec = true;
diff --git a/lanpaint_amd/csrc/step_kernel.hip b/lanpaint_amd/csrc/step_kernel.hip
--- a/lanpaint_amd/csrc/step_kernel.hip
+++ b/lanpaint_amd/csrc/step_kernel.hip
@@ -249,8 +249,9 @@
 }
 #define LP_CLK_DECL                                                                                                  \
     uint64_t clk_t[LP_CLK_STAMPS] = {}, clk_r0 = 0;                                                                  \
-    const bool clk_on = d_arg.clk_out && threadIdx.x == 0 && blockIdx.y == 0 && (blockIdx.x == 0 || blockIdx.x == gridDim.x - 1); \
-    if (clk_on) { clk_t[0] = clk_now(); clk_r0 = clk_real(); }
+    asm volatile("s_memtime %0" : "=s"(clk_t[0])::"memory");                                                         \
+    asm volatile("s_memrealtime %0" : "=s"(clk_r0)::"memory");                                                       \
+    const bool clk_on = d_arg.clk_out && threadIdx.x == 0 && blockIdx.y == 0 && (blockIdx.x == 0 || blockIdx.x == gridDim.x - 1);
 #define LP_CLK(k) if (clk_on) clk_t[k] = clk_now();
 #define LP_CLK_LOADS(k) if (clk_on) clk_t[k] = clk_after_loads();
 #define LP_CLK_FLUSH                                                                                                 \
@@ -274,10 +275,10 @@
 
 enum : int { MODE_ROW = 0, MODE_PER_EL = 1, MODE_HARD = 2 };
 
-template <int VEC, int MODE, uint32_t PH, int X0W, int RNG, bool ST = false, int ES = 0>
-__global__ __launch_bounds__(256) __attribute__((amdgpu_waves_per_eu((ES == 2 && VEC == 4 && PH != 0) ? 8 : 1))) void lp_step_kernel(void* a0, void* a1, const void* a2, const void* a3, const void* a4,
-                                                       const void* a5, int32_t a_el_per_row, uint32_t a_flags,
-                                                       const lp_step_desc d_arg) {
+template <int VEC, int MODE, uint32_t PH, int X0W, int RNG, bool ST, int ES, bool BV>
+__device__ __forceinline__ void lp_step_body(void* a0, void* a1, const void* a2, const void* a3, const void* a4,
+                                             const void* a5, int32_t a_el_per_row, uint32_t a_flags,
+                                             const lp_step_desc& d_arg) {
     constexpr bool PER_EL = MODE == MODE_PER_EL;
     constexpr bool HARD = MODE == MODE_HARD;
     constexpr bool SMALL = VEC == 1;
@@ -295,13 +296,20 @@
         d.y = static_cast<const float*>(a4); d.mask = a5;
     } else {
         d.x0 = a2; d.x0_big = a3;
-        if constexpr (SMALL) {
+        if constexpr (BV) {
+            d.rng_seed = reinterpret_cast<uint64_t>(a4); d.rng_offset = reinterpret_cast<uint64_t>(a5);
+            d.rng_offset_ptr = nullptr;
+        } else if constexpr (SMALL) {
             d.coef = static_cast<const float*>(a4); d.rng_offset_ptr = static_cast<const uint64_t*>(a5);
         } else {
             d.y = static_cast<const float*>(a4); d.mask = a5;
         }
     }
-    d.el_per_row = a_el_per_row; d.flags = a_flags;
+    d.el_per_row = a_el_per_row; d.flags = BV ? (a_flags & ~static_cast<uint32_t>(LP_FL_STATE_ARGS | LP_FL_STATE_ONE_THREAD)) : a_flags;
+    static_assert(!BV || (VEC == 1 && PH != 0 && (PH & LP_PH_REPLACE) == 0 && (PH & (LP_PH_POST_FIRST | LP_PH_POST_STEADY)) != 0 &&
+                          RNG == 1 && !ST && ES == 0),
+                  "state by value: the think-step launches at one element per lane, torch stream, no early stop");
+    const bool bv_early = BV && (a_flags & LP_FL_STATE_ONE_THREAD) != 0;
     static_assert(!ES || (!ST && !PER_EL && (PH & LP_PH_REPLACE) == 0), "early stop: think-step launches of the row-table modes");
     constexpr bool es_fold = ES == 2;
     int row = blockIdx.y;
@@ -390,7 +398,7 @@
     const bool flow = fl & LP_FL_FLOW;
     const bool post = ph & kPost;
     constexpr bool HOT = PH != 0 && ES == 0 && RNG == 0;
-    const bool given = HOT ? false : (fl & LP_FL_X0S_GIVEN) != 0;
+    const bool given = (HOT || BV) ? false : (fl & LP_FL_X0S_GIVEN) != 0;
     const int x0dt = X0W == 4 ? static_cast<int>(DT_F32) : x0_dtype(fl), xindt = xin_dtype(fl);
     const int64_t groups = ST ? static_cast<int64_t>(d.rng_bg) : d.el_per_row / VEC;
     const int64_t row_base = static_cast<int64_t>(row) * d.el_per_row;
@@ -471,7 +479,7 @@
         if constexpr (!PER_EL) {
             if constexpr (SMALL && PH != 0) {
                 static_assert(VEC == 1, "load_row_early leaves rc.rscale poisoned: the div_shared paths (VEC == 4) must use load_row");
-                rc = load_row_early(d.coef, row);
+                if constexpr (!BV) rc = load_row_early(d.coef, row);
             } else {
                 int crow = row;
                 if constexpr (PH == 0 && MODE == MODE_ROW && !ST) {
@@ -688,9 +696,17 @@
                 if (!(d.x0_big == d.x0 || given) && need_known && lane_known) load_raw_w<VEC, X0W>(d.x0_big, x0dt, i_kn, x0b_raw);
             }
         }
+        if constexpr (BV) {
+            if (bv_early) {
+                xi_a[0] = torch_normal<true>(static_cast<uint64_t>(i), d.rng_seed, d.rng_offset, 0u, true);
+                asm volatile("" : "+v"(xi_a[0]));
+                __builtin_amdgcn_sched_barrier(0);
+            }
+        }
+        if constexpr (BV) rc = load_row_early(d.coef, row);
         if constexpr (SMALL) load_mask_raw<VEC>(d.mask, mfl, i, m_raw);
         const bool has_corr = d.corr_el != nullptr && !given;
-        const bool host_post = HOT ? false : d.xi_post != nullptr, host_pre = HOT ? false : d.xi_pre != nullptr;
+        const bool host_post = (HOT || BV) ? false : d.xi_post != nullptr, host_pre = (HOT || BV) ? false : d.xi_pre != nullptr;
         const bool need_rng = (post && !host_post) || ((ph & LP_PH_PRE_HALF) && !host_pre);
         if (post) {
             if (!given && need_known && lane_known) load_f32<VEC>(d.y, i_kn, yv);
@@ -764,6 +780,7 @@
             rc.rsigma = rs_f;
         }
 
+        if constexpr (BV) __builtin_amdgcn_sched_barrier(0);
         LP_CLK(1)
         if (need_rng) {
             const bool torch_kind = RNG == 2 ? (d.rng_kind == LP_RNG_TORCH) : (RNG == 1);
@@ -773,8 +790,8 @@
                 if (torch_kind) seed = rng_w1;
             }
             if (torch_kind) {
-                const bool draw_post = post && !host_post, draw_pre = (ph & LP_PH_PRE_HALF) && !host_pre;
-                const uint64_t off_pre = seq + (draw_post ? d.rng_inc : 0u);
+                const bool any_post = post && !host_post, draw_post = any_post && !bv_early, draw_pre = (ph & LP_PH_PRE_HALF) && !host_pre;
+                const uint64_t off_pre = seq + (any_post ? (bv_early ? 4u : d.rng_inc) : 0u);
                 if constexpr (ST) {
                     static_assert(!ST || VEC == 4, "the ATen layout is four elements per lane");
                     __shared__ __attribute__((aligned(16))) float st_xi[2][4][kBlock];
@@ -802,7 +819,7 @@
                         xi_b[0] = q.x; xi_b[1] = q.y; xi_b[2] = q.z; xi_b[3] = q.w;
                     }
                 } else {
-                    const bool small = d.n_el <= static_cast<int64_t>(d.rng_bg);
+                    const bool small = bv_early || d.n_el <= static_cast<int64_t>(d.rng_bg);
 #pragma unroll
                     for (int k = 0; k < VEC; ++k) {
                         const uint64_t li = static_cast<uint64_t>(elem_index(i, k));
@@ -837,6 +854,10 @@
             }
         }
 
+        if constexpr (BV && (PH & LP_PH_PRE_HALF) != 0) {
+            asm volatile("" : "+v"(xi_b[0]));
+            __builtin_amdgcn_sched_barrier(0);
+        }
         if constexpr (ES == 2 && VEC == 4) {
             if (post) {
                 if (es_prev >= 0) load_f32<VEC>(es_prev == 0 ? d.es_x0s[0] : es_prev == 1 ? d.es_x0s[1] : d.es_x0s[2], i, x0p);
@@ -1207,6 +1228,22 @@
     }
 }
 
+template <int VEC, int MODE, uint32_t PH, int X0W, int RNG, bool ST>
+constexpr bool kStateByValue = VEC == 1 && PH != 0 && (PH & LP_PH_REPLACE) == 0 && RNG == 1 && !ST;
+
+template <int VEC, int MODE, uint32_t PH, int X0W, int RNG, bool ST = false, int ES = 0>
+__global__ __launch_bounds__(256) __attribute__((amdgpu_waves_per_eu((ES == 2 && VEC == 4 && PH != 0) ? 8 : 1))) void lp_step_kernel(void* a0, void* a1, const void* a2, const void* a3, const void* a4,
+                                                       const void* a5, int32_t a_el_per_row, uint32_t a_flags,
+                                                       const lp_step_desc d_arg) {
+    if constexpr (ES == 0 && kStateByValue<VEC, MODE, PH, X0W, RNG, ST>) {
+        if (a_flags & LP_FL_STATE_ARGS) {
+            lp_step_body<VEC, MODE, PH, X0W, RNG, ST, ES, true>(a0, a1, a2, a3, a4, a5, a_el_per_row, a_flags, d_arg);
+            return;
+        }
+    }
+    lp_step_body<VEC, MODE, PH, X0W, RNG, ST, ES, false>(a0, a1, a2, a3, a4, a5, a_el_per_row, a_flags, d_arg);
+}
+
 __global__ __launch_bounds__(64) void lp_es_decide_kernel(const lp_step_desc d, int slot) {
     const double* src = es_acc_set(d, d.es_index) + static_cast<size_t>(threadIdx.x) * 8;
     double v[kEsSums];
@@ -1333,6 +1370,7 @@
     if (d.n_el <= 0 || d.rows <= 0 || d.el_per_row <= 0 || d.n_el != d.el_per_row * d.rows) return LP_E_INVALID;
     if (d.rows > 65535 || d.el_per_row > 0x7fffffff) return LP_E_UNSUPPORTED;
     if (!d.mask || !d.x_t) return LP_E_INVALID;
+    if (d.flags & (LP_FL_STATE_ARGS | LP_FL_STATE_ONE_THREAD)) return LP_E_INVALID;
     if ((d.flags & LP_FL_MASK_BITS) && ((d.flags & (LP_FL_MASK_U8 | LP_FL_MASK_DENOISE)) || !aligned(d.mask, 4)))
         return LP_E_INVALID;
     const uint32_t ph = d.phases;
@@ -1421,6 +1459,13 @@
     a->a5 = lead_y ? d.mask : static_cast<const void*>(d.rng_offset_ptr);
     a->el_per_row = static_cast<int32_t>(d.el_per_row);
     a->flags = d.flags;
+    const bool by_value = p.vec == 1 && p.ph_ct != 0 && !rep && p.rng == 1 && !p.st && p.es == 0 && d.rng_offset_ptr == nullptr;
+    if (by_value) {
+        a->a4 = reinterpret_cast<const void*>(static_cast<uintptr_t>(d.rng_seed));
+        a->a5 = reinterpret_cast<const void*>(static_cast<uintptr_t>(d.rng_offset));
+        a->flags |= LP_FL_STATE_ARGS;
+        if (d.n_el <= static_cast<int64_t>(d.rng_bg) && d.rng_inc == 4u) a->flags |= LP_FL_STATE_ONE_THREAD;
+    }
     void* const ptr[9] = {&a->x_t, &a->C, &a->a2, &a->a3, &a->a4, &a->a5, &a->el_per_row, &a->flags, const_cast<lp_step_desc*>(&d)};
     for (int k = 0; k < 9; ++k) a->ptr[k] = ptr[k];
 }
@@ -1488,10 +1533,10 @@
     return rc == LP_OK ? enqueue(p, *dp, stream, timer) : rc;
 }
 
-int replace_node_update(const lp_step_desc* dp, hipGraphExec_t exec, const lp_graph_binding* b) {
+int step_node_update(const lp_step_desc* dp, hipGraphExec_t exec, const lp_graph_binding* b, bool replace) {
     if (!dp || !exec || !b || !b->node || !b->func) return LP_E_INVALID;
     const lp_step_desc& d = *dp;
-    if (!(d.phases & LP_PH_REPLACE) || d.xi_post || d.xi_pre || (d.flags & LP_FL_X0S_GIVEN)) return LP_E_INVALID;
+    if (((d.phases & LP_PH_REPLACE) != 0) != replace || d.xi_post || d.xi_pre || (d.flags & LP_FL_X0S_GIVEN)) return LP_E_INVALID;
     StepPlan p;
     const int rc = plan_step(d, &p);
     if (rc != LP_OK) return rc;
diff --git a/lanpaint_amd/engine.py b/lanpaint_amd/engine.py
--- a/lanpaint_amd/engine.py
+++ b/lanpaint_amd/engine.py
@@ -60,6 +60,7 @@
         self._rng_counters = {}
         self._capturing = None
         self._cap_offset = 0
+        self._cap_steps = None
         self._lib = _cabi.load()
         self._ws = None
         self._desc = _cabi.LpStepDesc()
@@ -573,6 +574,8 @@
                 d.phases = (LP_PH_POST_FIRST if i == 0 else LP_PH_POST_STEADY) | (0 if last else LP_PH_PRE_HALF) | LP_PH_EMIT
                 self._set_xi(d, ws.x_t, want_pre=not last)
                 self._launch_step(stream)
+                if self._cap_steps is not None:
+                    self._cap_steps.append(_cabi.LpStepDesc.from_buffer_copy(d))
                 del alive
             ran = n_steps
             if auto is not None and n_steps > 0:
```

Measured after the change: 120,100 think-iterations/s (median of 5 runs). No clear change (+2.1%).
